# POSTECH-CVLab/SCNeRF

Hardware: AMD Instinct MI355X
Metric: rays/sec (64+128 samples/ray) train-step (higher is better)
Workload: dtype f32 (3 x fp16 MFMA products per product, fp32 accumulate); 1 GPU; configs[1]: 4096 rays x (64 coarse + 128 fine), coarse+fine NeRF (D=8, W=256), fwd+bwd of render_rays per GPU, perturb=1, raw_noise_std=1; precomputed rays of a fixed camera; rays_per_gpu=4096, parallelism=ray-parallel x1, no collective at N = 1

## Files before the change

include/scnerf_hip.h:

```cpp
#ifndef SCNERF_HIP_H
#define SCNERF_HIP_H

#include <stdint.h>

#ifdef __cplusplus
extern "C" {
#endif

#define SCNERF_ABI_VERSION 4

int scnerf_abi_version(void);


int scnerf_searchsorted(const float* a, const float* v, int64_t* out, int nrow, int nrow_a,
                        int nrow_v, int na, int nv, int side_left, void* stream);

int scnerf_sample_pdf(const float* bins, const float* weights, const float* u, int u_row_stride,
                      float* samples, int64_t* inds, float* cdf, int n, int nb, int ns,
                      void* stream);

int scnerf_render_randoms(unsigned long long seed, unsigned long long call, float* t_rand, long long n_t_rand,
                          float* u, long long n_u, float* noise_c, long long n_noise_c, float* noise_f,
                          long long n_noise_f, float raw_noise_std, void* stream);

// ... 18 lines not shown
long long scnerf_camera_bwd_workspace_floats(int n_slots);
int scnerf_camera_rays_bwd(const float* kps, const long long* cam_idx, int single_idx,
                           const float* extrinsic, int n_ext, const float* intr_init,
                           const float* intr_noise, float intr_scale, int multiplicative,
                           const float* extr_init, const float* extr_noise, float extr_scale,
                           int n_cams, const float* grid_o, float scale_o, const float* grid_d,
                           float scale_d, int gh, int gw, int H, int W, const float* g_o,
                           const float* g_d, float* d_intr_noise, float* d_extr_noise, float* d_grid_o,
                           float* d_grid_d, float* d_extrinsic, float* workspace, int n, void* stream);

int scnerf_camera_matrices_fwd(const float* intr_init, const float* intr_noise, float intr_scale, int multiplicative,
                               const float* extr_init, const float* extr_noise, float extr_scale, int n_cams,
                               float* K, float* E, void* stream);
int scnerf_camera_matrices_bwd(const float* intr_init, float intr_scale, int multiplicative, const float* extr_init,
                               const float* extr_noise, float extr_scale, int n_cams, const float* g_K,
                               const float* g_E, float* d_intr_noise, float* d_extr_noise, void* stream);

int scnerf_pinhole_rays(const float* kps, int kps_stride, const float* c2w, float focal, int H, int W,
                        float* rays_o, float* rays_d, int n, void* stream);

int scnerf_ndc_fwd(int H, int W, const float* focal_xy, float near, const float* rays_o,
                   const float* rays_d, float* ndc_o, float* ndc_d, int n, void* stream);
int scnerf_ndc_bwd(int H, int W, const float* focal_xy, float near, const float* rays_o,
                   const float* rays_d, const float* g_ndc_o, const float* g_ndc_d, float* g_rays_o,
                   float* g_rays_d, float* g_focal_xy, int n, void* stream);

int scnerf_pack_rays_fwd(int H, int W, const float* focal_xy, float ndc_near, const float* rays_o, const float* rays_d,
                         float near, float far, int cols, float* ray_batch, int n, void* stream);
int scnerf_pack_rays_bwd(int H, int W, const float* focal_xy, float ndc_near, const float* rays_o, const float* rays_d,
                         int cols, const float* g_ray_batch, float* g_rays_o, float* g_rays_d, float* g_focal_xy, int n,
                         void* stream);

int scnerf_upsample_grid_fwd(const float* grid, float scale, int gh, int gw, int H, int W, float* out,
                             void* stream);
int scnerf_upsample_grid_bwd(const float* g_out, float scale, int gh, int gw, int H, int W,
                             float* d_grid, void* stream);


int scnerf_composite_fwd(const float* raw, const float* z, const float* rays, int ray_stride,
                         const float* noise, int white_bkgd, float* rgb_map, float* disp_map,
                         float* acc_map, float* depth_map, float* weights, int n, int s,
                         void* stream);

int scnerf_composite_bwd(const float* raw, const float* z, const float* rays, int ray_stride,
                         const float* noise, int white_bkgd, const float* g_rgb,
                         const float* g_disp, const float* g_acc, const float* g_depth,
                         const float* g_raw_in, float* d_raw, float* d_rays_d, int n, int s,
                         void* stream);

int scnerf_ray_reduce(const float* d_pts, const float* d_views, const float* z,
                      const float* extra_d, float* d_rays, int ray_stride, int accumulate, int n,
                      int s, void* stream);


int scnerf_gather_f32(const float* src, const int* idx, float* dst, long long n, void* stream);

int scnerf_mlp_layout_info(int pt_dims, int* out, int n);

int scnerf_mlp_fwd(int pt_dims, const float* pts, const float* viewdirs, int vd_stride, int samples_per_ray,
                   const float* wpacked, float* raw, float* save, long long n_samples,
                   void* stream);

long long scnerf_mlp_save_floats(int pt_dims, long long n_samples);
long long scnerf_mlp_grad_floats(long long n_samples);

int scnerf_coarse_stage_fwd(const float* rays, int ray_stride, const float* t_vals, const float* t_rand, int lindisp,
                            const float* wpacked, float* save, const float* noise, int white_bkgd, float* z,
                            float* pts, float* raw, float* rgb_map, float* disp_map, float* acc_map,
                            float* depth_map, float* weights, int n_rays, int n_samples, void* stream);

int scnerf_mlp_bwd(int pt_dims, const float* d_raw, const float* pts, const float* viewdirs, int vd_stride,
                   int samples_per_ray, const float* wpacked_bwd, const float* save,
                   float* grads, float* d_pts, float* d_views, long long n_samples, void* stream);

long long scnerf_wgrad_workspace_floats(int n_load, int k_load, int n_chunks);
int scnerf_wgrad(const float* dz, int lda, int n_load, int n_out, int dz_tiled, const float* x,
                 int ldb, int k_load, int k_out, int x_tiled, long long n_samples, int n_chunks,
                 float* workspace, float* dW, int ldo, int col0, float* db, void* stream);

int scnerf_vecmat(const float* x_tiled256, const float* vec, int vec_stride, long long n_samples,
                  int n_chunks, float* workspace, float* dv, float* dvsum, void* stream);

int scnerf_nerf_param_count(int pt_dims);
int scnerf_wgrad_arithmetic(int mode);
long long scnerf_nerf_wgrad_workspace_floats(int n_chunks);
long long scnerf_wgrad_chunk_samples(long long n_samples, int n_chunks);
int scnerf_wgrad256_chunks(int n_chunks);
int scnerf_nerf_wgrad_h3(int pt_dims, const float* save, const float* grads, const float* d_raw,
                         long long n_samples, int n_chunks, float* workspace, float* flat_grad,
                         int accumulate, const float* amax_x, const float* amax_z, const float* scales,
                         void* ev_before, void* ev_after, void* stream);
int scnerf_wgrad256_half(const float* dz_tiled, const float* x_tiled, long long n_samples, int n_chunks,
                         float* workspace, float* dW, float* db, const float* amax_dz, const float* amax_x,
                         void* stream);
int scnerf_wgrad_half_narrow(const float* dz_tiled, int n_load, const float* x, int k_load, int k_out, int x_tiled,
                             long long n_samples, int n_chunks, float* workspace, float* dW, float* db,
                             const float* amax_dz, const float* amax_x, int n_coarse, long long coarse_chunk,
                             void* stream);
int scnerf_nerf_wgrad(int pt_dims, const float* save, const float* grads, const float* d_raw,
                      long long n_samples, int n_chunks, float* workspace, float* flat_grad,
                      int accumulate, void* stream);

long long scnerf_h3_scale_floats(void);
int scnerf_h3_pack(const float* flat_params, const int* jobs, const int* idx_fwd, const unsigned char* meta_fwd,
                   long long frags_fwd, const int* idx_bwd, const unsigned char* meta_bwd, long long frags_bwd,
                   short* stream_fwd, short* stream_bwd, float* scales, void* stream);
int scnerf_mlp_fwd_h3(int pt_dims, const float* pts, const float* viewdirs, int vd_stride, int samples_per_ray,
                      const float* wpacked, const short* stream_fwd, const float* scales, float* raw, float* save,
                      long long n_samples, float* chunk_amax, int n_chunks, long long chunk_samples, void* stream);
int scnerf_mlp_bwd_h3(int pt_dims, const float* d_raw, const float* pts, const float* viewdirs, int vd_stride,
                      int samples_per_ray, const float* wpacked_bwd, const short* stream_bwd, const float* scales,
                      const float* save, float* grads, float* d_pts, float* d_views, long long n_samples,
                      float* chunk_amax, int n_chunks, long long chunk_samples, void* stream);
int scnerf_coarse_stage_fwd_h3(const float* rays, int ray_stride, const float* t_vals, const float* t_rand,
                               int lindisp, const float* wpacked, const short* stream_fwd, const float* scales,
                               float* save, const float* noise, int white_bkgd, float* z, float* pts, float* raw,
                               float* rgb_map, float* disp_map, float* acc_map, float* depth_map, float* weights,
                               int n_rays, int n_samples, float* chunk_amax, int n_chunks, long long chunk_samples,
                               void* stream);
int scnerf_fine_stage_fwd_h3(const float* rays, int ray_stride, const float* z_c, const float* w_c, const float* u,
                             int u_row_stride, const float* wpacked, const short* stream_fwd, const float* scales,
                             float* save, const float* noise, int white_bkgd, float* z_f, float* pts_f, float* z_samples,
                             float* z_std, long long* inds, float* cdf, float* raw, float* rgb_map, float* disp_map,
                             float* acc_map, float* depth_map, float* weights, int n_rays, int n_coarse, int n_importance,
                             float* chunk_amax, int n_chunks, long long chunk_samples, void* stream);

int scnerf_mlp_fwd_h3_guarded(int pt_dims, const float* pts, const float* viewdirs, int vd_stride, int samples_per_ray,
                              const float* wpacked, const short* stream_fwd, const float* scales, float* raw, float* save,
                              long long n_samples, float* chunk_amax, int n_chunks, long long chunk_samples, int* guard_flags,
                              int* guard_any, float* guard_report, void* stream);
int scnerf_coarse_stage_fwd_h3_guarded(const float* rays, int ray_stride, const float* t_vals, const float* t_rand,
                                       int lindisp, const float* wpacked, const short* stream_fwd, const float* scales,
                                       float* save, const float* noise, int white_bkgd, float* z, float* pts, float* raw,
                                       float* rgb_map, float* disp_map, float* acc_map, float* depth_map, float* weights,
                                       int n_rays, int n_samples, float* chunk_amax, int n_chunks, long long chunk_samples,
                                       int* guard_flags, int* guard_any, float* guard_report, void* stream);
int scnerf_fine_stage_fwd_h3_guarded(const float* rays, int ray_stride, const float* z_c, const float* w_c, const float* u,
                                     int u_row_stride, const float* wpacked, const short* stream_fwd, const float* scales,
                                     float* save, const float* noise, int white_bkgd, float* z_f, float* pts_f,
                                     float* z_samples, float* z_std, long long* inds, float* cdf, float* raw, float* rgb_map,
                                     float* disp_map, float* acc_map, float* depth_map, float* weights, int n_rays,
                                     int n_coarse, int n_importance, float* chunk_amax, int n_chunks,
                                     long long chunk_samples, int* guard_flags, int* guard_any, float* guard_report,
                                     void* stream);
int scnerf_mlp_bwd_h3_guarded(int pt_dims, const float* d_raw, const float* pts, const float* viewdirs, int vd_stride,
                              int samples_per_ray, const float* wpacked_bwd, const short* stream_bwd, const float* scales,
                              const float* save, float* grads, float* d_pts, float* d_views, long long n_samples,
                              float* chunk_amax, int n_chunks, long long chunk_samples, int* guard_flags, int* guard_any,
                              float* guard_report, void* stream);
int scnerf_mlp_fwd_h3_lean(int pt_dims, const float* pts, const float* viewdirs, int vd_stride, int samples_per_ray,
                           const float* wpacked, const short* stream_fwd, const float* scales, float* raw, float* save,
                           long long n_samples, float* chunk_amax, int n_chunks, long long chunk_samples, int* guard_flags,
                           int* guard_any, float* guard_report, int lean, void* stream);
int scnerf_coarse_stage_fwd_h3_lean(const float* rays, int ray_stride, const float* t_vals, const float* t_rand,
                                    int lindisp, const float* wpacked, const short* stream_fwd, const float* scales,
                                    float* save, const float* noise, int white_bkgd, float* z, float* pts, float* raw,
                                    float* rgb_map, float* disp_map, float* acc_map, float* depth_map, float* weights,
                                    int n_rays, int n_samples, float* chunk_amax, int n_chunks, long long chunk_samples,
                                    int* guard_flags, int* guard_any, float* guard_report, int lean, void* stream);
int scnerf_fine_stage_fwd_h3_lean(const float* rays, int ray_stride, const float* z_c, const float* w_c, const float* u,
                                  int u_row_stride, const float* wpacked, const short* stream_fwd, const float* scales,
                                  float* save, const float* noise, int white_bkgd, float* z_f, float* pts_f,
                                  float* z_samples, float* z_std, long long* inds, float* cdf, float* raw, float* rgb_map,
                                  float* disp_map, float* acc_map, float* depth_map, float* weights, int n_rays,
                                  int n_coarse, int n_importance, float* chunk_amax, int n_chunks,
                                  long long chunk_samples, int* guard_flags, int* guard_any, float* guard_report, int lean,
                                  void* stream);
int scnerf_mlp_bwd_h3_lean(int pt_dims, const float* d_raw, const float* pts, const float* viewdirs, int vd_stride,
                           int samples_per_ray, const float* wpacked_bwd, const short* stream_bwd, const float* scales,
                           const float* save, float* grads, float* d_pts, float* d_views, long long n_samples,
                           float* chunk_amax, int n_chunks, long long chunk_samples, int* guard_flags, int* guard_any,
                           float* guard_report, int lean, void* stream);
int scnerf_nerf_wgrad_h3_lean(int pt_dims, const float* save, const float* grads, const float* d_raw,
                              long long n_samples, int n_chunks, float* workspace, float* flat_grad,
                              int accumulate, const float* amax_x, const float* amax_z, const float* scales,
                              const float* flat_params, void* ev_before, void* ev_after, void* stream);
int scnerf_wgrad_lean_finish(const float* M, const float* s, const float* flat_params, float* flat_grad, int accumulate,
                             void* stream);
int scnerf_wgrad_lean_finish_pd(int pt_dims, const float* M, const float* s, const float* flat_params, float* flat_grad,
                                int accumulate, void* stream);
int scnerf_mlp_fwd_gated(int pt_dims, const float* pts, const float* viewdirs, int vd_stride, int samples_per_ray,
                         const float* wpacked, float* raw, float* save, long long n_samples, const int* flags,
                         int max_workgroups, void* stream);
int scnerf_coarse_stage_fwd_gated(const float* rays, int ray_stride, const float* t_vals, const float* t_rand,
                                  int lindisp, const float* wpacked, float* save, const float* noise, int white_bkgd,
                                  float* z, float* pts, float* raw, float* rgb_map, float* disp_map, float* acc_map,
                                  float* depth_map, float* weights, int n_rays, int n_samples, const int* flags,
                                  int max_workgroups, void* stream);
int scnerf_mlp_bwd_gated(int pt_dims, const float* d_raw, const float* pts, const float* viewdirs, int vd_stride,
                         int samples_per_ray, const float* wpacked_bwd, const float* save, float* grads, float* d_pts,
                         float* d_views, long long n_samples, const int* flags, int max_workgroups, void* stream);

int scnerf_mlp_fwd_h3_fast(int pt_dims, const float* pts, const float* viewdirs, int vd_stride, int samples_per_ray,
                           const float* wpacked, const short* stream_fwd, const float* scales, float* raw,
                           long long n_samples, float* chunk_amax, int n_chunks, long long chunk_samples, void* stream);
int scnerf_coarse_stage_fwd_h3_fast(const float* rays, int ray_stride, const float* t_vals, const float* t_rand,
                                    int lindisp, const float* wpacked, const short* stream_fwd, const float* scales,
                                    const float* noise, int white_bkgd, float* z, float* pts, float* raw,
                                    float* rgb_map, float* disp_map, float* acc_map, float* depth_map, float* weights,
                                    int n_rays, int n_samples, float* chunk_amax, int n_chunks, long long chunk_samples,
                                    void* stream);


int scnerf_prd_loss_fwd(const float* kps0, const float* kps1, const float* rays0_o, const float* rays0_d,
                        const float* rays1_o, const float* rays1_d, const float* K, const float* E2,
                        float eps, float threshold, int negate_fx, int eval_mode, int m, float* sums6,
                        float* loss, float* n_match, void* stream);

int scnerf_prd_loss_bwd(const float* kps0, const float* kps1, const float* rays0_o, const float* rays0_d,
                        const float* rays1_o, const float* rays1_d, const float* K, const float* E2,
                        float eps, float threshold, int negate_fx, int m, const float* sums6,
                        const float* g_loss, float* g_rays0_o, float* g_rays0_d, float* g_rays1_o,
                        float* g_rays1_d, float* g_K, float* g_E2, float* workspace36, void* stream);

int scnerf_embed_fwd(const float* x, long long n, int d, const float* freqs, int n_freqs, int include_input,
                     float* out, void* stream);
int scnerf_embed_bwd(const float* x, const float* g_out, long long n, int d, const float* freqs, int n_freqs,
                     int include_input, float* g_x, void* stream);

int scnerf_prd_filter(const float* kps0, const float* kps1, const float* rays0_o, const float* rays0_d,
                      const float* rays1_o, const float* rays1_d, const float* K, const float* E2,
                      float eps, float threshold, int negate_fx, int m, unsigned char* keep, void* stream);


int scnerf_npp_intersect_fwd(const float* ray_o, const float* ray_d, float* far, int* outside_flag, int n,
                             void* stream);
int scnerf_npp_intersect_bwd(const float* ray_o, const float* ray_d, const float* g_far, float* g_ray_o,
                             float* g_ray_d, int n, void* stream);

int scnerf_npp_perturb_fwd(const float* z, const float* t_rand, float* out, int n, int s, void* stream);
int scnerf_npp_perturb_bwd(const float* g_out, const float* t_rand, float* g_z, int n, int s, void* stream);

int scnerf_npp_sample_pdf(const float* bins, const float* weights, const float* u, float* samples,
                          int* below_above, float* t, float* cdf, int n, int m, int ns, void* stream);
int scnerf_npp_sample_pdf_bwd(const float* g_samples, const int* below_above, const float* t, float* g_bins,
                              int n, int m, int ns, void* stream);

int scnerf_npp_points_fwd(const float* ray_o, const float* ray_d, const float* fg_z, const float* bg_z,
                          float* fg_pts, float* bg_pts, float* viewdirs, float* bg_depth_real, int n, int sf,
                          int sb, void* stream);
int scnerf_npp_points_bwd(const float* ray_o, const float* ray_d, const float* fg_z, const float* bg_z,
                          const float* d_fg_pts, const float* d_bg_pts, const float* d_views_fg,
                          const float* d_views_bg, const float* d_norm, const float* g_fg_z_in,
                          float* g_ray_o, float* g_ray_d, float* g_fg_z, int n, int sf, int sb, void* stream);

int scnerf_npp_composite_fwd(const float* raw_fg, const float* raw_bg, const float* fg_z, const float* fg_z_max,
                             const float* bg_z, const float* ray_d, float* rgb, float* fg_weights,
                             float* bg_weights, float* fg_rgb, float* fg_depth, float* bg_rgb, float* bg_depth,
                             float* bg_lambda, int n, int sf, int sb, void* stream);
int scnerf_npp_composite_bwd(const float* raw_fg, const float* raw_bg, const float* fg_z, const float* fg_z_max,
                             const float* bg_z, const float* ray_d, const float* g_rgb, const float* g_fg_weights,
                             const float* g_bg_weights, const float* g_fg_rgb, const float* g_fg_depth,
                             const float* g_bg_rgb, const float* g_bg_depth, const float* g_bg_lambda,
                             float* d_raw_fg, float* d_raw_bg, float* d_fg_z, float* d_fg_z_max, float* d_norm,
                             int n, int sf, int sb, void* stream);

int scnerf_npp_fg_lambda(const float* raw_fg, const float* fg_z, const float* fg_z_max, const float* ray_d,
                         float* bg_lambda, int n, int sf, void* stream);
int scnerf_npp_composite_fwd_skip(const float* raw_fg, const float* raw_bg_live, const float* fg_z,
                                  const float* fg_z_max, const float* bg_z, const float* ray_d, const int* slot_of,
                                  float* rgb, float* fg_weights, float* bg_weights, float* fg_rgb, float* fg_depth,
                                  float* bg_rgb, float* bg_depth, float* bg_lambda, int n, int n_live, int sf, int sb,
                                  void* stream);

int scnerf_npp_camera_rays_fwd(const long long* select, const float* dist2, int camera_idx,
                               const float* extrinsic, const float* intr_init, const float* intr_noise,
                               float intr_scale, int multiplicative, const float* extr_init,
                               const float* extr_noise, float extr_scale, int n_cams, const float* grid_o,
                               float scale_o, const float* grid_d, float scale_d, int gh, int gw, int H, int W,
                               float* rays_o, float* rays_d, int n, void* stream);
int scnerf_npp_camera_rays_bwd(const long long* select, const float* dist2, int camera_idx,
                               const float* extrinsic, const float* intr_init, const float* intr_noise,
                               float intr_scale, int multiplicative, const float* extr_init,
                               const float* extr_noise, float extr_scale, int n_cams, const float* grid_o,
                               float scale_o, const float* grid_d, float scale_d, int gh, int gw, int H, int W,
                               const float* g_o, const float* g_d, float* d_intr_noise, float* d_extr_noise,
                               float* d_grid_o, float* d_grid_d, float* d_extrinsic, float* d_dist2,
                               float* workspace, int n, void* stream);


int scnerf_adam_step(float* param, const float* grad, float* exp_avg, float* exp_avg_sq,
                     long long n, double lr, double beta1, double beta2, double eps,
                     double weight_decay, long long step, void* stream);
int scnerf_adam_step_range(float* param, const float* grad, float* exp_avg, float* exp_avg_sq,
                           long long n, double lr, double beta1, double beta2, double eps,
                           double weight_decay, long long decay_lo, long long decay_hi, long long step, void* stream);


long long scnerf_image_metrics_workspace_floats(int n, int c, int h, int w, int win);

int scnerf_image_metrics(const float* x, long long x_stride_n, long long x_stride_c, long long x_stride_h,
                         long long x_stride_w, const float* y, long long y_stride_n, long long y_stride_c,
                         long long y_stride_h, long long y_stride_w, int n, int c, int h, int w, const float* taps,
                         int win, float c1, float c2, float value_range, int clip_x, float* ssim_out, float* mse_out,
                         float* map_out, float* workspace, void* stream);


int scnerf_ray_batch(int mode, unsigned long long seed, unsigned long long step, const void* images, int image_u8,
                     int channels, int n_images, long long H, long long W, const int64_t* image_ids, int n_sel,
                     int image_pos, long long win_x0, long long win_y0, long long win_w, long long win_h, long long n,
                     int rank, int world, int white_bkgd, int64_t* coords, int64_t* select_inds, int64_t* image_idx,
                     float* target, void* stream);


int scnerf_ray_compact(const float* acc, float tau, int* live_idx, int* slot_of, int* n_live_dev, int* n_live_host,
                       long long n, void* stream);
// ... 73 lines not shown
```

scnerf_amd/_capi.py:

```python
from __future__ import annotations

import ctypes
import os
from ctypes import c_int, c_longlong, c_void_p, c_float, c_double

D = c_double

F = c_float

_HERE = os.path.dirname(os.path.abspath(__file__))
LIB_PATH = os.environ.get("SCNERF_HIP_LIB") or os.path.join(_HERE, "libscnerf_hip.so")

P = c_void_p
I = c_int
LL = c_longlong

PROTOTYPES = {
    "scnerf_abi_version": [],
    "scnerf_searchsorted": [P, P, P, I, I, I, I, I, I, P],
    "scnerf_sample_pdf": [P, P, P, I, P, P, P, I, I, I, P],
    "scnerf_render_randoms": [ctypes.c_ulonglong, ctypes.c_ulonglong, P, LL, P, LL, P, LL, P, LL, F, P],
    "scnerf_coarse_sample": [P, I, P, P, P, P, I, I, I, P],
    "scnerf_fine_sample": [P, I, P, P, P, I, P, P, P, P, P, P, I, I, I, P],
    "scnerf_camera_rays_fwd": [P, P, I, P, I, P, P, F, I, P, P, F, I, P, F, P, F, I, I, I, I, P, P, I, P],
    "scnerf_camera_rays_bwd": [P, P, I, P, I, P, P, F, I, P, P, F, I, P, F, P, F, I, I, I, I, P, P, P, P, P, P, P, P, I, P],
    "scnerf_camera_matrices_fwd": [P, P, F, I, P, P, F, I, P, P, P],
    "scnerf_camera_matrices_bwd": [P, F, I, P, P, F, I, P, P, P, P, P],
    "scnerf_pinhole_rays": [P, I, P, F, I, I, P, P, I, P],
    "scnerf_ndc_fwd": [I, I, P, F, P, P, P, P, I, P],
    "scnerf_ndc_bwd": [I, I, P, F, P, P, P, P, P, P, P, I, P],
    "scnerf_pack_rays_fwd": [I, I, P, F, P, P, F, F, I, P, I, P],
    "scnerf_pack_rays_bwd": [I, I, P, F, P, P, I, P, P, P, P, I, P],
    "scnerf_upsample_grid_fwd": [P, F, I, I, I, I, P, P],
    "scnerf_upsample_grid_bwd": [P, F, I, I, I, I, P, P],
    "scnerf_prd_loss_fwd": [P, P, P, P, P, P, P, P, F, F, I, I, I, P, P, P, P],
    "scnerf_prd_loss_bwd": [P, P, P, P, P, P, P, P, F, F, I, I, P, P, P, P, P, P, P, P, P, P],
    "scnerf_embed_fwd": [P, LL, I, P, I, I, P, P],
    "scnerf_embed_bwd": [P, P, LL, I, P, I, I, P, P],
    "scnerf_prd_filter": [P, P, P, P, P, P, P, P, F, F, I, I, P, P],
    "scnerf_npp_intersect_fwd": [P, P, P, P, I, P],
    "scnerf_npp_intersect_bwd": [P, P, P, P, P, I, P],
    "scnerf_npp_perturb_fwd": [P, P, P, I, I, P],
    "scnerf_npp_perturb_bwd": [P, P, P, I, I, P],
    "scnerf_npp_sample_pdf": [P, P, P, P, P, P, P, I, I, I, P],
    "scnerf_npp_sample_pdf_bwd": [P, P, P, P, I, I, I, P],
    "scnerf_npp_points_fwd": [P, P, P, P, P, P, P, P, I, I, I, P],
    "scnerf_npp_points_bwd": [P, P, P, P, P, P, P, P, P, P, P, P, P, I, I, I, P],
    "scnerf_npp_composite_fwd": [P, P, P, P, P, P, P, P, P, P, P, P, P, P, I, I, I, P],
    "scnerf_npp_composite_bwd": [P, P, P, P, P, P, P, P, P, P, P, P, P, P, P, P, P, P, P, I, I, I, P],
    "scnerf_npp_fg_lambda": [P, P, P, P, P, I, I, P],
    "scnerf_npp_composite_fwd_skip": [P, P, P, P, P, P, P, P, P, P, P, P, P, P, P, I, I, I, I, P],
    "scnerf_npp_camera_rays_fwd": [P, P, I, P, P, P, F, I, P, P, F, I, P, F, P, F, I, I, I, I, P, P, I, P],
    "scnerf_npp_camera_rays_bwd": [P, P, I, P, P, P, F, I, P, P, F, I, P, F, P, F, I, I, I, I, P, P, P, P, P, P, P,
                                   P, P, I, P],
    "scnerf_adam_step": [P, P, P, P, LL, D, D, D, D, D, LL, P],
    "scnerf_adam_step_range": [P, P, P, P, LL, D, D, D, D, D, LL, LL, LL, P],
    "scnerf_composite_fwd": [P, P, P, I, P, I, P, P, P, P, P, I, I, P],
    "scnerf_composite_bwd": [P, P, P, I, P, I, P, P, P, P, P, P, P, I, I, P],
    "scnerf_ray_reduce": [P, P, P, P, P, I, I, I, I, P],
    "scnerf_gather_f32": [P, P, P, LL, P],
    "scnerf_mlp_layout_info": [I, P, I],
    "scnerf_mlp_fwd": [I, P, P, I, I, P, P, P, LL, P],
    "scnerf_coarse_stage_fwd": [P, I, P, P, I, P, P, P, I, P, P, P, P, P, P, P, P, I, I, P],
    "scnerf_mlp_bwd": [I, P, P, P, I, I, P, P, P, P, P, LL, P],
    "scnerf_nerf_param_count": [I],
    "scnerf_nerf_wgrad": [I, P, P, P, LL, I, P, P, I, P],
    "scnerf_wgrad": [P, I, I, I, I, P, I, I, I, I, LL, I, P, P, I, I, P, P],
    "scnerf_vecmat": [P, P, I, LL, I, P, P, P, P],
    "scnerf_wgrad_arithmetic": [I],
    "scnerf_wgrad256_chunks": [I],
    "scnerf_h3_pack": [P, P, P, P, LL, P, P, LL, P, P, P, P],
    "scnerf_mlp_fwd_h3": [I, P, P, I, I, P, P, P, P, P, LL, P, I, LL, P],
    "scnerf_mlp_bwd_h3": [I, P, P, P, I, I, P, P, P, P, P, P, P, LL, P, I, LL, P],
    "scnerf_coarse_stage_fwd_h3": [P, I, P, P, I, P, P, P, P, P, I, P, P, P, P, P, P, P, P, I, I, P, I, LL, P],
    "scnerf_fine_stage_fwd_h3": [P, I, P, P, P, I, P, P, P, P, P, I, P, P, P, P, P, P, P, P, P, P, P, P, I, I, I, P, I, LL, P],
    "scnerf_mlp_fwd_h3_guarded": [I, P, P, I, I, P, P, P, P, P, LL, P, I, LL, P, P, P, P],
    "scnerf_mlp_bwd_h3_guarded": [I, P, P, P, I, I, P, P, P, P, P, P, P, LL, P, I, LL, P, P, P, P],
    "scnerf_coarse_stage_fwd_h3_guarded": [P, I, P, P, I, P, P, P, P, P, I, P, P, P, P, P, P, P, P, I, I, P, I, LL,
                                           P, P, P, P],
    "scnerf_fine_stage_fwd_h3_guarded": [P, I, P, P, P, I, P, P, P, P, P, I, P, P, P, P, P, P, P, P, P, P, P, P, I, I, I, P,
                                         I, LL, P, P, P, P],
    "scnerf_mlp_fwd_h3_fast": [I, P, P, I, I, P, P, P, P, LL, P, I, LL, P],
    "scnerf_coarse_stage_fwd_h3_fast": [P, I, P, P, I, P, P, P, P, I, P, P, P, P, P, P, P, P, I, I, P, I, LL, P],
    "scnerf_mlp_fwd_gated": [I, P, P, I, I, P, P, P, LL, P, I, P],
    "scnerf_coarse_stage_fwd_gated": [P, I, P, P, I, P, P, P, I, P, P, P, P, P, P, P, P, I, I, P, I, P],
    "scnerf_mlp_bwd_gated": [I, P, P, P, I, I, P, P, P, P, P, LL, P, I, P],
    "scnerf_nerf_wgrad_h3": [I, P, P, P, LL, I, P, P, I, P, P, P, P, P, P],
    "scnerf_wgrad256_half": [P, P, LL, I, P, P, P, P, P, P],
    "scnerf_wgrad_half_narrow": [P, I, P, I, I, I, LL, I, P, P, P, P, P, I, LL, P],
    "scnerf_mlp_fwd_h3_lean": [I, P, P, I, I, P, P, P, P, P, LL, P, I, LL, P, P, P, I, P],
    "scnerf_mlp_bwd_h3_lean": [I, P, P, P, I, I, P, P, P, P, P, P, P, LL, P, I, LL, P, P, P, I, P],
    "scnerf_coarse_stage_fwd_h3_lean": [P, I, P, P, I, P, P, P, P, P, I, P, P, P, P, P, P, P, P, I, I, P, I, LL,
                                        P, P, P, I, P],
    "scnerf_fine_stage_fwd_h3_lean": [P, I, P, P, P, I, P, P, P, P, P, I, P, P, P, P, P, P, P, P, P, P, P, P, I, I, I, P,
                                      I, LL, P, P, P, I, P],
    "scnerf_nerf_wgrad_h3_lean": [I, P, P, P, LL, I, P, P, I, P, P, P, P, P, P, P],
    "scnerf_wgrad_lean_finish": [P, P, P, P, I, P],
    "scnerf_wgrad_lean_finish_pd": [I, P, P, P, P, I, P],
    "scnerf_image_metrics": [P, LL, LL, LL, LL, P, LL, LL, LL, LL, I, I, I, I, P, I, F, F, F, I, P, P, P, P, P],
    "scnerf_ray_batch": [I, ctypes.c_ulonglong, ctypes.c_ulonglong, P, I, I, I, LL, LL, P, I, I, LL, LL, LL, LL, LL, I, I, I,
                         P, P, P, P, P],
    "scnerf_ray_compact": [P, F, P, P, P, P, LL, P],
    "scnerf_ray_rows_gather": [P, P, P, LL, I, LL, P],
    "scnerf_ray_expand": [P, LL, LL, I, I] + [P] * 8 + [P] * 4 + [P] * 8 + [P],
    "scnerf_live_compact": [P, LL, P, P, P, P, P, P, P],
    "scnerf_live_gather": [P, LL, LL, P, P, I, P, I, I, P, P, P, P],
    "scnerf_live_remap_maxima": [P, LL, P, I, LL, P, I, LL, I, P],
    "scnerf_live_scatter_rows": [P, P, P, LL, I, LL, P],
    "scnerf_mlp_bwd_h3_masks": [I, P, P, P, I, I, P, P, P, P, P, P, P, LL, P, I, LL, P, P, P, I, P],
    "scnerf_nerf_wgrad_h3_live": [I, P, LL, I, P, P, P, P, LL, I, P, P, I, P, P, P, P, P, P, P],
    "scnerf_occ_compact": [P, LL, P, I, I, P, I, F, F, F, F, F, F, P, P, P, P, P, P, P, P],
    "scnerf_occ_expand_raw": [P, P, P, LL, LL, P],
    "scnerf_occ_probe_points": [LL, LL, I, I, F, F, F, F, F, F, F, F, F, P, P],
    "scnerf_occ_accumulate": [P, F, LL, LL, I, I, P, P],
    "scnerf_occ_dilate": [P, P, I, P],
    "scnerf_occ_compact4": [P, LL, P, I, I, P, I, F, F, F, F, F, F, P, P, P, P, P, P, P, P],
    "scnerf_occ_probe_points_inverted": [LL, LL, I, I, F, F, F, F, F, F, F, F, F, P, P],
    "scnerf_seg_compact": [P, LL, I, I, I, P, P, I, P, I, F, F, F, F, F, F, P, P, P, P, P, P, P, P],
    "scnerf_seg_expand_raw": [P, P, P, LL, I, I, I, LL, P],
    "scnerf_seg_transmittance": [P, P, P, I, LL, I, I, I, I, I, D, P, P, P, P],
}


SIZE_FUNCS = {"scnerf_mlp_save_floats": [I, LL], "scnerf_mlp_grad_floats": [LL],
              "scnerf_wgrad_workspace_floats": [I, I, I],
              "scnerf_nerf_wgrad_workspace_floats": [I],
              "scnerf_h3_scale_floats": [],
              "scnerf_wgrad_chunk_samples": [LL, I],
              "scnerf_camera_bwd_workspace_floats": [I],
              "scnerf_live_compact_workspace_ints": [LL],
              "scnerf_occ_compact_workspace_ints": [LL],
              "scnerf_occ_compact4_workspace_ints": [LL],
              "scnerf_seg_compact_workspace_ints": [LL],
              "scnerf_image_metrics_workspace_floats": [I, I, I, I, I]}


def bind(lib: ctypes.CDLL) -> ctypes.CDLL:
    for name, args in PROTOTYPES.items():
        fn = getattr(lib, name)
        fn.argtypes = args
        fn.restype = c_int
    for name, args in SIZE_FUNCS.items():
        fn = getattr(lib, name)
        fn.argtypes = args
        fn.restype = c_longlong
    return lib


_lib = None


class ScnerfLibraryError(RuntimeError):
    pass


def load() -> ctypes.CDLL:
    global _lib
    if _lib is None:
        import torch
        if not os.path.isfile(LIB_PATH):
            raise ScnerfLibraryError(
                "libscnerf_hip.so is not built (%s). Run `python -m scnerf_amd.csrc.build` "
                "(or __graft_entry__.build()); scnerf_amd has no CPU fallback." % LIB_PATH)
        _lib = bind(ctypes.CDLL(LIB_PATH))
        if _lib.scnerf_abi_version() != 4:
            raise ScnerfLibraryError("ABI version mismatch")
    return _lib


def on_device(t) -> bool:
    return bool(t.is_cuda)


def current_stream():
    import torch
    return torch.cuda.current_stream().cuda_stream


def check(status: int, what: str):
    if status != 0:
        raise RuntimeError("%s failed with status %d" % (what, status))
```

scnerf_amd/csrc/mlp_fwd_h3.hip:

```cpp
#include <scn_wave.h>

#include "launch.h"
#include "mlp_fwd_h3_api.h"
#include "mlp_h3.h"
#include "scnerf_hip.h"

namespace {

using namespace scn;
using namespace scn::h3;

constexpr int kScaleBlocks = 16, kScaleCols = 512;
constexpr int kScalePartial = 4 + kScaleCols;

__global__ __launch_bounds__(256) void h3_scale_partial_kernel(const float* __restrict__ params, const int* __restrict__ jobs,
                                                               float* __restrict__ partial, float* __restrict__ table) {
    float* red = dynamic_lds<float>();
    float* cols_w = red + 16;
    const int l = blockIdx.x, blk = blockIdx.y, tid = threadIdx.x, lane = lane_id(), wave = wave_id();
    const float* wt = params + jobs[4 * l];
    const int rows = jobs[4 * l + 1], cols = jobs[4 * l + 2];
    const float* bs = params + jobs[4 * l + 3];
    const int per = (rows + kScaleBlocks - 1) / kScaleBlocks;
    const int r0 = blk * per, r1 = min(rows, r0 + per);
    if (l == kLayerRgb && blk == 0 && tid == 0) table[kLayerRgb * kScaleStride + kPoison] = 0.f;
    float mx = 0.f, rowsum = 0.f, bmax = 0.f, bad = 0.f;
    float colp[kScaleCols / 64];
#pragma unroll
    for (int k = 0; k < kScaleCols / 64; ++k) colp[k] = 0.f;
    for (int r = r0 + wave; r < r1; r += 4) {
        float s = 0.f;
#pragma unroll
        for (int k = 0; k < kScaleCols / 64; ++k) {
            const int c = lane + 64 * k;
            const float a = c < cols ? fabsf(wt[(long)r * cols + c]) : 0.f;
            s += a;
            mx = fmaxf(mx, a);
            colp[k] += a;
        }
        for (int o = 32; o > 0; o >>= 1) s += shfl_xor(s, o);
        rowsum = fmaxf(rowsum, s);
        bmax = fmaxf(bmax, fabsf(bs[r]));
        if (!(s < __builtin_huge_valf()) || !(fabsf(bs[r]) < __builtin_huge_valf())) bad = 1.f;
    }
    for (int o = 32; o > 0; o >>= 1) mx = fmaxf(mx, shfl_xor(mx, o));
#pragma unroll
    for (int k = 0; k < kScaleCols / 64; ++k) cols_w[wave * kScaleCols + lane + 64 * k] = colp[k];
    if (lane == 0) { red[wave * 4] = mx; red[wave * 4 + 1] = rowsum; red[wave * 4 + 2] = bmax; red[wave * 4 + 3] = bad; }
    block_sync();
    float* out = partial + ((long)l * kScaleBlocks + blk) * kScalePartial;
    if (tid < 4) out[tid] = fmaxf(fmaxf(red[tid], red[4 + tid]), fmaxf(red[8 + tid], red[12 + tid]));
    for (int c = tid; c < kScaleCols; c += 256)
        out[4 + c] = ((cols_w[c] + cols_w[kScaleCols + c]) + cols_w[2 * kScaleCols + c]) + cols_w[3 * kScaleCols + c];
}

__global__ __launch_bounds__(256) void h3_scale_finish_kernel(const float* __restrict__ partial, const int* __restrict__ jobs,
                                                              float* __restrict__ table) {
    float* red = dynamic_lds<float>();
    const int l = blockIdx.x, tid = threadIdx.x;
    const int cols = jobs[4 * l + 2];
    const float* p = partial + (long)l * kScaleBlocks * kScalePartial;
    float colsum = 0.f;
    for (int c = tid; c < cols; c += 256) {
        float s = 0.f;
        for (int b = 0; b < kScaleBlocks; ++b) s += p[b * kScalePartial + 4 + c];
        colsum = fmaxf(colsum, s);
    }
    red[tid] = colsum;
    block_sync();
    for (int s = 128; s > 0; s >>= 1) {
        if (tid < s) red[tid] = fmaxf(red[tid], red[tid + s]);
        block_sync();
    }
    if (tid == 0) {
        float mx = 0.f, rowsum = 0.f, bmax = 0.f, bad = 0.f;
        for (int b = 0; b < kScaleBlocks; ++b) {
            mx = fmaxf(mx, p[b * kScalePartial]);
            rowsum = fmaxf(rowsum, p[b * kScalePartial + 1]);
            bmax = fmaxf(bmax, p[b * kScalePartial + 2]);
            bad = fmaxf(bad, p[b * kScalePartial + 3]);
        }
        if (bad > 0.f) table[kLayerRgb * kScaleStride + kPoison] = __builtin_nanf("");
        const float sw = scn::h3::scale_for(mx);
        float* t = table + l * kScaleStride;
        t[kSw] = sw;
        t[kSwInv] = scn::h3::inv_pow2(sw);
        t[kBoundA] = rowsum * 1.0001f;
        t[kBoundB] = bmax;
        t[kBoundAT] = red[0] * 1.0001f;
        t[5] = mx; t[6] = 0.f;
        if (l != kLayerRgb) t[kPoison] = 0.f;
    }
}

__global__ __launch_bounds__(256) void h3_pack_kernel(const float* __restrict__ params, const int* __restrict__ idx,
                                                      const unsigned char* __restrict__ meta, const float* __restrict__ table,
                                                      short* __restrict__ out, long n) {
    const long i = (long)blockIdx.x * blockDim.x + threadIdx.x;
    if (i >= n) return;
    const int j = idx[i];
    const unsigned mt = meta[i >> 9];
    const float x = j >= 0 ? params[j] * table[(mt >> 1) * kScaleStride + kSw] : 0.f;
    const unsigned hb = f16_bits(x);
    out[i] = (short)((mt & 1u) ? f16_bits(x - f16_value(hb)) : hb);
}

}

extern "C" long long scnerf_h3_scale_floats(void) {
    return (long long)kScaleLayers * kScaleStride + (long long)kScaleLayers * kScaleBlocks * kScalePartial;
}

extern "C" int scnerf_h3_pack(const float* flat_params, const int* jobs, const int* idx_fwd, const unsigned char* meta_fwd,
                              long long frags_fwd, const int* idx_bwd, const unsigned char* meta_bwd, long long frags_bwd,
                              short* stream_fwd, short* stream_bwd, float* scales, void* stream) {
    SCN_RETURN_IF(!flat_params || !jobs || !scales, SCN_EINVAL);
    SCN_RETURN_IF((frags_fwd > 0 && (!idx_fwd || !meta_fwd || !stream_fwd)) || (frags_bwd > 0 && (!idx_bwd || !meta_bwd || !stream_bwd)), SCN_EINVAL);
    SCN_RETURN_IF(frags_fwd < 0 || frags_bwd < 0, SCN_EINVAL);
    hipStream_t st = (hipStream_t)stream;
    float* partial = scales + kScaleLayers * kScaleStride;
    hipLaunchKernelGGL(h3_scale_partial_kernel, dim3(kScaleLayers, kScaleBlocks), dim3(256), (16 + 4 * kScaleCols) * 4, st,
                       flat_params, jobs, partial, scales);
    hipLaunchKernelGGL(h3_scale_finish_kernel, dim3(kScaleLayers), dim3(256), 1024, st, partial, jobs, scales);
    if (frags_fwd > 0)
        hipLaunchKernelGGL(h3_pack_kernel, dim3(scn_ceil_div(frags_fwd * 512, 256)), dim3(256), 0, st, flat_params, idx_fwd,
                           meta_fwd, scales, stream_fwd, (long)(frags_fwd * 512));
    if (frags_bwd > 0)
        hipLaunchKernelGGL(h3_pack_kernel, dim3(scn_ceil_div(frags_bwd * 512, 256)), dim3(256), 0, st, flat_params, idx_bwd,
                           meta_bwd, scales, stream_bwd, (long)(frags_bwd * 512));
    return scn_launch_status();
}

extern "C" int scnerf_mlp_fwd_h3_lean(int pt_dims, const float* pts, const float* viewdirs, int vd_stride,
                                      int samples_per_ray, const float* wpacked, const short* stream_fwd,
                                      const float* scales, float* raw, float* save, long long n_samples, float* chunk_amax,
                                      int n_chunks, long long chunk_samples, int* guard_flags, int* guard_any,
                                      float* guard_report, int lean, void* stream) {
    SCN_RETURN_IF(!pts || !viewdirs || !wpacked || !stream_fwd || !scales || !raw, SCN_EINVAL);
    SCN_RETURN_IF(samples_per_ray < 1 || vd_stride < 3 || n_samples < 0 || (pt_dims != 3 && pt_dims != 4), SCN_EINVAL);
    SCN_RETURN_IF(n_samples >= (1LL << 31), SCN_ENOSUP);
    SCN_RETURN_IF(chunk_amax && (n_chunks < 1 || chunk_samples < 32 || chunk_samples % 32), SCN_EINVAL);
    SCN_RETURN_IF(!guard_flags != !guard_any || (guard_report && !guard_flags), SCN_EINVAL);
    if (n_samples == 0) return 0;
    hipStream_t st = (hipStream_t)stream;
    const scn::h3f::ChunkMaxima cm{chunk_amax, n_chunks, lean != 0, (long)chunk_samples, {guard_flags, guard_any, guard_report}};
    return pt_dims == 3 ? scn::h3f::fwd_h3_pd3(pts, viewdirs, vd_stride, samples_per_ray, wpacked, stream_fwd, scales, raw, save, n_samples, cm, st)
                        : scn::h3f::fwd_h3_pd4(pts, viewdirs, vd_stride, samples_per_ray, wpacked, stream_fwd, scales, raw, save, n_samples, cm, st);
}

extern "C" int scnerf_mlp_fwd_h3_guarded(int pt_dims, const float* pts, const float* viewdirs, int vd_stride,
                                         int samples_per_ray, const float* wpacked, const short* stream_fwd,
                                         const float* scales, float* raw, float* save, long long n_samples, float* chunk_amax,
                                         int n_chunks, long long chunk_samples, int* guard_flags, int* guard_any,
                                         float* guard_report, void* stream) {
    return scnerf_mlp_fwd_h3_lean(pt_dims, pts, viewdirs, vd_stride, samples_per_ray, wpacked, stream_fwd, scales, raw, save,
                                  n_samples, chunk_amax, n_chunks, chunk_samples, guard_flags, guard_any, guard_report, 0, stream);
}

extern "C" int scnerf_mlp_fwd_h3(int pt_dims, const float* pts, const float* viewdirs, int vd_stride, int samples_per_ray,
                                 const float* wpacked, const short* stream_fwd, const float* scales, float* raw, float* save,
                                 long long n_samples, float* chunk_amax, int n_chunks, long long chunk_samples, void* stream) {
    return scnerf_mlp_fwd_h3_guarded(pt_dims, pts, viewdirs, vd_stride, samples_per_ray, wpacked, stream_fwd, scales, raw, save,
                                     n_samples, chunk_amax, n_chunks, chunk_samples, nullptr, nullptr, nullptr, stream);
}

extern "C" int scnerf_coarse_stage_fwd_h3_lean(const float* rays, int ray_stride, const float* t_vals, const float* t_rand,
                                               int lindisp, const float* wpacked, const short* stream_fwd,
                                               const float* scales, float* save, const float* noise, int white_bkgd, float* z,
                                               float* pts, float* raw, float* rgb_map, float* disp_map, float* acc_map,
                                               float* depth_map, float* weights, int n_rays, int n_samples,
                                               float* chunk_amax, int n_chunks, long long chunk_samples, int* guard_flags,
                                               int* guard_any, float* guard_report, int lean, void* stream) {
    SCN_RETURN_IF(!rays || !t_vals || !wpacked || !stream_fwd || !scales || !z || !pts || !raw || !rgb_map || !disp_map || !acc_map, SCN_EINVAL);
    SCN_RETURN_IF(n_rays < 0 || ray_stride < 11, SCN_EINVAL);
    SCN_RETURN_IF(n_samples != scn::h3f::kCoarseSamples || n_rays >= (1 << 25), SCN_ENOSUP);
    SCN_RETURN_IF(chunk_amax && (n_chunks < 1 || chunk_samples < 32 || chunk_samples % 32), SCN_EINVAL);
    SCN_RETURN_IF(!guard_flags != !guard_any || (guard_report && !guard_flags), SCN_EINVAL);
    if (n_rays == 0) return 0;
    const scn::h3f::CoarseStage cs{rays, ray_stride, n_rays, t_vals, t_rand, lindisp, z, pts, noise, white_bkgd,
                                   rgb_map, disp_map, acc_map, depth_map, weights};
    const scn::h3f::ChunkMaxima cm{chunk_amax, n_chunks, lean != 0, (long)chunk_samples, {guard_flags, guard_any, guard_report}};
    return scn::h3f::fwd_h3_coarse(cs, rays, ray_stride, wpacked, stream_fwd, scales, raw, save, cm, (hipStream_t)stream);
}

extern "C" int scnerf_coarse_stage_fwd_h3_guarded(const float* rays, int ray_stride, const float* t_vals, const float* t_rand,
                                                  int lindisp, const float* wpacked, const short* stream_fwd,
                                                  const float* scales, float* save, const float* noise, int white_bkgd, float* z,
                                                  float* pts, float* raw, float* rgb_map, float* disp_map, float* acc_map,
                                                  float* depth_map, float* weights, int n_rays, int n_samples,
                                                  float* chunk_amax, int n_chunks, long long chunk_samples, int* guard_flags,
                                                  int* guard_any, float* guard_report, void* stream) {
    return scnerf_coarse_stage_fwd_h3_lean(rays, ray_stride, t_vals, t_rand, lindisp, wpacked, stream_fwd, scales, save, noise,
                                           white_bkgd, z, pts, raw, rgb_map, disp_map, acc_map, depth_map, weights, n_rays,
                                           n_samples, chunk_amax, n_chunks, chunk_samples, guard_flags, guard_any, guard_report,
                                           0, stream);
}

extern "C" int scnerf_coarse_stage_fwd_h3(const float* rays, int ray_stride, const float* t_vals, const float* t_rand,
                                          int lindisp, const float* wpacked, const short* stream_fwd, const float* scales,
                                          float* save, const float* noise, int white_bkgd, float* z, float* pts, float* raw,
                                          float* rgb_map, float* disp_map, float* acc_map, float* depth_map, float* weights,
                                          int n_rays, int n_samples, float* chunk_amax, int n_chunks, long long chunk_samples,
                                          void* stream) {
    return scnerf_coarse_stage_fwd_h3_guarded(rays, ray_stride, t_vals, t_rand, lindisp, wpacked, stream_fwd, scales, save, noise,
                                              white_bkgd, z, pts, raw, rgb_map, disp_map, acc_map, depth_map, weights, n_rays,
                                              n_samples, chunk_amax, n_chunks, chunk_samples, nullptr, nullptr, nullptr, stream);
}

extern "C" int scnerf_mlp_fwd_h3_fast(int pt_dims, const float* pts, const float* viewdirs, int vd_stride, int samples_per_ray,
                                      const float* wpacked, const short* stream_fwd, const float* scales, float* raw,
                                      long long n_samples, float* chunk_amax, int n_chunks, long long chunk_samples,
                                      void* stream) {
    SCN_RETURN_IF(!pts || !viewdirs || !wpacked || !stream_fwd || !scales || !raw, SCN_EINVAL);
    SCN_RETURN_IF(samples_per_ray < 1 || vd_stride < 3 || n_samples < 0 || (pt_dims != 3 && pt_dims != 4), SCN_EINVAL);
    SCN_RETURN_IF(n_samples >= (1LL << 31), SCN_ENOSUP);
    SCN_RETURN_IF(chunk_amax && (n_chunks < 1 || chunk_samples < 32 || chunk_samples % 32), SCN_EINVAL);
    if (n_samples == 0) return 0;
    hipStream_t st = (hipStream_t)stream;
    return pt_dims == 3 ? scn::h3f::fwd_h3_pd3_fast(pts, viewdirs, vd_stride, samples_per_ray, wpacked, stream_fwd, scales, raw, n_samples, st)
                        : scn::h3f::fwd_h3_pd4_fast(pts, viewdirs, vd_stride, samples_per_ray, wpacked, stream_fwd, scales, raw, n_samples, st);
}

extern "C" int scnerf_coarse_stage_fwd_h3_fast(const float* rays, int ray_stride, const float* t_vals, const float* t_rand,
                                               int lindisp, const float* wpacked, const short* stream_fwd, const float* scales,
                                               const float* noise, int white_bkgd, float* z, float* pts, float* raw,
                                               float* rgb_map, float* disp_map, float* acc_map, float* depth_map, float* weights,
                                               int n_rays, int n_samples, float* chunk_amax, int n_chunks,
                                               long long chunk_samples, void* stream) {
    SCN_RETURN_IF(!rays || !t_vals || !wpacked || !stream_fwd || !scales || !z || !pts || !raw || !rgb_map || !disp_map || !acc_map, SCN_EINVAL);
    SCN_RETURN_IF(n_rays < 0 || ray_stride < 11, SCN_EINVAL);
    SCN_RETURN_IF(n_samples != scn::h3f::kCoarseSamples || n_rays >= (1 << 25), SCN_ENOSUP);
    SCN_RETURN_IF(chunk_amax && (n_chunks < 1 || chunk_samples < 32 || chunk_samples % 32), SCN_EINVAL);
    if (n_rays == 0) return 0;
    const scn::h3f::CoarseStage cs{rays, ray_stride, n_rays, t_vals, t_rand, lindisp, z, pts, noise, white_bkgd,
                                   rgb_map, disp_map, acc_map, depth_map, weights};
    return scn::h3f::fwd_h3_coarse_fast(cs, rays, ray_stride, wpacked, stream_fwd, scales, raw, (hipStream_t)stream);
}

extern "C" int scnerf_fine_stage_fwd_h3_lean(const float* rays, int ray_stride, const float* z_c, const float* w_c,
                                             const float* u, int u_row_stride, const float* wpacked, const short* stream_fwd,
                                             const float* scales, float* save, const float* noise, int white_bkgd, float* z_f,
                                             float* pts_f, float* z_samples, float* z_std, long long* inds, float* cdf,
                                             float* raw, float* rgb_map, float* disp_map, float* acc_map, float* depth_map,
                                             float* weights, int n_rays, int n_coarse, int n_importance, float* chunk_amax,
                                             int n_chunks, long long chunk_samples, int* guard_flags, int* guard_any,
                                             float* guard_report, int lean, void* stream) {
    SCN_RETURN_IF(!rays || !z_c || !w_c || !u || !wpacked || !stream_fwd || !scales, SCN_EINVAL);
    SCN_RETURN_IF(!z_f || !pts_f || !z_samples || !z_std || !raw || !rgb_map || !disp_map || !acc_map, SCN_EINVAL);
    SCN_RETURN_IF(n_rays < 0 || ray_stride < 11 || (u_row_stride != 0 && u_row_stride != n_importance), SCN_EINVAL);
    SCN_RETURN_IF(n_coarse != scn::h3f::kCoarseSamples || (n_importance != 64 && n_importance != 128 && n_importance != 192), SCN_ENOSUP);
    SCN_RETURN_IF((long long)n_rays * (n_coarse + n_importance) >= (1LL << 31), SCN_ENOSUP);
    SCN_RETURN_IF(chunk_amax && (n_chunks < 1 || chunk_samples < 32 || chunk_samples % 32), SCN_EINVAL);
    SCN_RETURN_IF(!guard_flags != !guard_any || (guard_report && !guard_flags), SCN_EINVAL);
    if (n_rays == 0) return 0;
    const int tot = n_coarse + n_importance;
    const int rays_per_block = tot == 192 ? 2 : 1, tiles = tot * rays_per_block / 128;
    const scn::h3f::FineStage fs{rays, ray_stride, n_rays, z_c, w_c, u, u_row_stride, n_importance, z_f, pts_f, z_samples, z_std,
                                 reinterpret_cast<int64_t*>(inds), cdf, noise, white_bkgd, rgb_map, disp_map, acc_map,
                                 depth_map, weights, rays_per_block, tiles};
    const scn::h3f::ChunkMaxima cm{chunk_amax, n_chunks, lean != 0, (long)chunk_samples, {guard_flags, guard_any, guard_report}};
    return save ? scn::h3f::fwd_h3_fine_train(fs, wpacked, stream_fwd, scales, raw, save, cm, (hipStream_t)stream)
                : scn::h3f::fwd_h3_fine_infer(fs, wpacked, stream_fwd, scales, raw, cm, (hipStream_t)stream);
}

extern "C" int scnerf_fine_stage_fwd_h3_guarded(const float* rays, int ray_stride, const float* z_c, const float* w_c,
                                                const float* u, int u_row_stride, const float* wpacked, const short* stream_fwd,
                                                const float* scales, float* save, const float* noise, int white_bkgd, float* z_f,
                                                float* pts_f, float* z_samples, float* z_std, long long* inds, float* cdf,
                                                float* raw, float* rgb_map, float* disp_map, float* acc_map, float* depth_map,
                                                float* weights, int n_rays, int n_coarse, int n_importance, float* chunk_amax,
                                                int n_chunks, long long chunk_samples, int* guard_flags, int* guard_any,
                                                float* guard_report, void* stream) {
    return scnerf_fine_stage_fwd_h3_lean(rays, ray_stride, z_c, w_c, u, u_row_stride, wpacked, stream_fwd, scales, save, noise,
                                         white_bkgd, z_f, pts_f, z_samples, z_std, inds, cdf, raw, rgb_map, disp_map, acc_map,
                                         depth_map, weights, n_rays, n_coarse, n_importance, chunk_amax, n_chunks, chunk_samples,
                                         guard_flags, guard_any, guard_report, 0, stream);
}

extern "C" int scnerf_fine_stage_fwd_h3(const float* rays, int ray_stride, const float* z_c, const float* w_c, const float* u,
                                        int u_row_stride, const float* wpacked, const short* stream_fwd, const float* scales,
                                        float* save, const float* noise, int white_bkgd, float* z_f, float* pts_f,
                                        float* z_samples, float* z_std, long long* inds, float* cdf, float* raw, float* rgb_map,
                                        float* disp_map, float* acc_map, float* depth_map, float* weights, int n_rays,
                                        int n_coarse, int n_importance, float* chunk_amax, int n_chunks,
                                        long long chunk_samples, void* stream) {
    return scnerf_fine_stage_fwd_h3_guarded(rays, ray_stride, z_c, w_c, u, u_row_stride, wpacked, stream_fwd, scales, save, noise,
                                            white_bkgd, z_f, pts_f, z_samples, z_std, inds, cdf, raw, rgb_map, disp_map, acc_map,
                                            depth_map, weights, n_rays, n_coarse, n_importance, chunk_amax, n_chunks,
                                            chunk_samples, nullptr, nullptr, nullptr, stream);
}
```

scnerf_amd/csrc/mlp_fwd_h3_api.h:

```cpp
#pragma once
#include <cstdint>

#include <hip/hip_runtime.h>

#include "resident_guard.h"

namespace scn {
namespace h3f {

struct ChunkMaxima { float* amax; int n_chunks; int lean; long chunk; ResidentGuard guard; };

struct CoarseStage {
    const float* rays; int ray_stride; int n_rays;
    const float* t_vals; const float* t_rand; int lindisp;
    float* z; float* pts;
    const float* noise; int white_bkgd;
    float* rgb; float* disp; float* acc; float* depth; float* weights;
};
constexpr int kCoarseSamples = 64;

struct FineStage {
    const float* rays; int ray_stride; int n_rays;
    const float* z_c; const float* w_c;
    const float* u; int u_row_stride; int n_importance;
    float* z_f; float* pts_f; float* z_samples; float* z_std; int64_t* inds; float* cdf;
    const float* noise; int white_bkgd;
    float* rgb; float* disp; float* acc; float* depth; float* weights;
    int rays_per_block, tiles;
};

int fwd_h3_pd3(const float* pts, const float* viewdirs, int vd_stride, int samples_per_ray, const float* wpacked,
               const short* stream_fwd, const float* scales, float* raw, float* save, long long n_samples, ChunkMaxima cm,
               hipStream_t st);
int fwd_h3_pd4(const float* pts, const float* viewdirs, int vd_stride, int samples_per_ray, const float* wpacked,
               const short* stream_fwd, const float* scales, float* raw, float* save, long long n_samples, ChunkMaxima cm,
               hipStream_t st);
int fwd_h3_coarse(const CoarseStage& cs, const float* rays, int ray_stride, const float* wpacked, const short* stream_fwd,
                  const float* scales, float* raw, float* save, ChunkMaxima cm, hipStream_t st);
int fwd_h3_pd3_fast(const float* pts, const float* viewdirs, int vd_stride, int samples_per_ray, const float* wpacked,
                    const short* stream_fwd, const float* scales, float* raw, long long n_samples, hipStream_t st);
int fwd_h3_pd4_fast(const float* pts, const float* viewdirs, int vd_stride, int samples_per_ray, const float* wpacked,
                    const short* stream_fwd, const float* scales, float* raw, long long n_samples, hipStream_t st);
int fwd_h3_coarse_fast(const CoarseStage& cs, const float* rays, int ray_stride, const float* wpacked, const short* stream_fwd,
                       const float* scales, float* raw, hipStream_t st);
int fwd_h3_fine_train(const FineStage& fs, const float* wpacked, const short* stream_fwd, const float* scales, float* raw,
                      float* save, ChunkMaxima cm, hipStream_t st);
int fwd_h3_fine_infer(const FineStage& fs, const float* wpacked, const short* stream_fwd, const float* scales, float* raw,
                      ChunkMaxima cm, hipStream_t st);

}
}
```

scnerf_amd/csrc/mlp_fwd_h3_kernel.h:

```cpp
#pragma once
#include <scn_wave.h>

#include "launch.h"
#include "mlp_fwd_h3_api.h"
#include "mlp_h3.h"
#include "ray_sample.h"
#include "ray_stage.h"

namespace scn {
namespace h3f {

using namespace scn::mlp;
using namespace scn::h3;


template <int PD, int L, int NS, int LD>
struct PeInverse {
    unsigned off[LD];
    constexpr PeInverse() : off() {
        for (int c = 0; c < LD; ++c) off[c] = 0xffffffffu;
        for (int s = 0; s < NS; ++s)
            for (int h = 0; h < 2; ++h) {
                const int c = pe_col(L, s, h, PD);
                if (c >= 0) off[c] = (unsigned)((s / 4) * (kThreads * 16) + h * 512 + (s % 4) * 4);
            }
    }
};
template <int PD, int L, int NS, int LD>
__device__ __forceinline__ void store_pe_tile(const char* slots, float* __restrict__ section, long wave_tile, int wave, int lane) {
    if (lab::kNoPeStore) return;
    wave_lds_handoff();
    static constexpr PeInverse<PD, L, NS, LD> inverse{};
    constexpr int LPR = LD / 4;
    unsigned o[4];
#pragma unroll
    for (int i = 0; i < 4; ++i) o[i] = inverse.off[4 * (lane % LPR) + i];
    const global_bytes_rw block = uniform_global_rw(section + wave_tile * (32L * LD));
#pragma unroll
    for (int k = 0; k < LD / 8; ++k) {
        const int m = k * (64 / LPR) + lane / LPR;
        const char* row = slots + (wave * 64 + m) * 16;
        f32x4 v;
#pragma unroll
        for (int i = 0; i < 4; ++i) v[i] = o[i] == 0xffffffffu ? 0.f : *reinterpret_cast<const float*>(row + o[i]);
        store_stream_at(uniform_global_rw(block + k * 1024), pinned_here((unsigned)lane * 16u), v);
    }
}

struct NoDensity {};
struct Density {
    float sg;
    const float* alpha;
    f32x4 wq;
};
template <bool ON> struct MaskBits { unsigned bits0, bits1, words[4]; };
template <> struct MaskBits<false> {};
struct NoWindow {};
struct Window { unsigned window; };

template <bool TRAIN, int KIND, int PRODUCTS = 3>
struct FwdEpi : std::conditional_t<KIND == 1, Density, NoDensity>, MaskBits<TRAIN && KIND != 2>,
                std::conditional_t<TRAIN && KIND == 2, Window, NoWindow> {
    float os, s_next, am;
    const float* bias;
    global_bytes_rw save;
    unsigned lane16;
    f32x4 bq;
    float v[4];
    unsigned hp;

    __device__ __forceinline__ void prime() {}

    template <int P, int PIECE, int SUB, int NS>
    __device__ __forceinline__ void sub(f32x16 (&acc)[2], u32x4 (&oh)[NS], u32x4 (&ol)[NS]) {
        constexpr int x = PIECE >> 2, q = PIECE & 3, T = 2 * P + x;
        constexpr int sl = 2 * T + (q >> 1), c0 = 2 * (q & 1);
        static_assert(sl < NS, "operand buffer too small for this tile");
        if constexpr (lab::kNoEpilogue) {
            if constexpr (SUB == 1) {
                oh[sl][c0] = __float_as_uint(acc[x][4 * q]) & 0x3bff3bffu; oh[sl][c0 + 1] = __float_as_uint(acc[x][4 * q + 1]) & 0x3bff3bffu;
                if constexpr (PRODUCTS == 3) {
                    ol[sl][c0] = __float_as_uint(acc[x][4 * q + 2]) & 0x3bff3bffu; ol[sl][c0 + 1] = __float_as_uint(acc[x][4 * q + 3]) & 0x3bff3bffu;
                }
            }
        } else if constexpr (SUB == 0) {
            bq = *reinterpret_cast<const f32x4*>(bias + (4 * T + q) * 8);
            if constexpr (KIND == 1) this->wq = *reinterpret_cast<const f32x4*>(this->alpha + (4 * T + q) * 8);
            if constexpr (TRAIN && KIND != 2 && PIECE == 0) { this->bits0 = 0u; this->bits1 = 0u; }
        } else if constexpr (SUB <= 4) {
            constexpr int e = SUB - 1;
            const float z = __builtin_fmaf(acc[x][4 * q + e], os, bq[e]);
            v[e] = KIND == 2 ? z : relu_raw(z);
            if constexpr (TRAIN && KIND != 2) {
                if constexpr (x == 0) this->bits0 = shift_in_positive(this->bits0, v[e]);
                else this->bits1 = shift_in_positive(this->bits1, v[e]);
            }
        } else if constexpr (SUB == 5) {
            if constexpr (KIND == 2) { am = max3_abs(am, v[0], v[1]); am = max3_abs(am, v[2], v[3]); }
            else { am = max3(am, v[0], v[1]); am = max3(am, v[2], v[3]); }
        } else if constexpr (SUB == 6) {
            hp = pack_f16_scaled(v[0], v[1], s_next);
        } else if constexpr (SUB == 7) {
            oh[sl][c0] = hp;
            if constexpr (PRODUCTS == 3) ol[sl][c0] = pack_f16(residual_f16<0>(v[0], s_next, hp), residual_f16<1>(v[1], s_next, hp));
        } else if constexpr (SUB == 8) {
            hp = pack_f16_scaled(v[2], v[3], s_next);
        } else if constexpr (SUB == 9) {
            oh[sl][c0 + 1] = hp;
            if constexpr (PRODUCTS == 3) ol[sl][c0 + 1] = pack_f16(residual_f16<0>(v[2], s_next, hp), residual_f16<1>(v[3], s_next, hp));
        } else if constexpr (SUB == 10) {
            if constexpr (TRAIN && !lab::kNoStore) {
                if constexpr (KIND == 2)
                    store_written_through_window(uniform_global_rw(save + (4 * T + q) * 1024), pinned_here(lane16), f32x4{v[0], v[1], v[2], v[3]}, this->window);
                else
                    store_written_through_at(uniform_global_rw(save + (4 * T + q) * 1024), pinned_here(lane16), f32x4{v[0], v[1], v[2], v[3]});
            }
        } else {
            if constexpr (KIND == 1) {
#pragma unroll
                for (int e = 0; e < 4; ++e) this->sg = __builtin_fmaf(this->wq[e], v[e], this->sg);
            }
            if constexpr (TRAIN && KIND != 2 && PIECE == 7) this->words[P] = (this->bits0 << 16) | this->bits1;
        }
    }
};



constexpr int kTabFeat = 8 * 256, kTabViews = kTabFeat + 256, kTabRgb = kTabViews + 128, kTabAlpha = kTabRgb + 32,
              kTabAlphaB = kTabAlpha + 256;

enum : int { kPoints = 0, kCoarse = 1, kFine = 2 };
constexpr int kFineMaxSamples = 384;

template <int PD, int STAGE = kPoints>
__host__ __device__ constexpr unsigned fwd_lds_bytes() {
    return (unsigned)(kStreamLds + kTableFloats * 4 + Var<PD>::kES * kThreads * 4 + (STAGE == kFine ? kFineMaxSamples * 20 : 0));
}

struct FwdKernelArgs {
    const float* pts; const float* viewdirs; int vd_stride; int samples_per_ray; const float* wpk; const short* wh3;
    const float* sc; float* raw; float* save; long P; CoarseStage cs; FineStage fs; ChunkMaxima cm;
};
static_assert(sizeof(FwdKernelArgs) == 72 + sizeof(CoarseStage) + sizeof(FineStage) + sizeof(ChunkMaxima), "argument block layout");

template <int PD, bool TRAIN, int STAGE, int PRODUCTS = 3>
__global__ __launch_bounds__(kThreads, 1) void mlp_fwd_h3_kernel(
    const float* __restrict__ pts, const float* __restrict__ viewdirs, int vd_stride, int samples_per_ray,
    const float* __restrict__ wpk, const short* __restrict__ wh3, const float* __restrict__ sc,
    float* __restrict__ raw, float* __restrict__ save_arg, long P, CoarseStage cs, FineStage fs, ChunkMaxima cm) {
    using V = Var<PD>;
    constexpr int ES = V::kES, NE = ES / 8;
    constexpr bool COARSE = STAGE == kCoarse, FINE = STAGE == kFine, ONE = PRODUCTS == 1;
    static_assert(!ONE || (!TRAIN && !FINE), "one product: forward-only, sample-list forward and coarse stage");
    claim_whole_register_file();
    auto low_of = [](const u32x4& lo, const u32x4& hi) { if constexpr (ONE) return hi; else return lo; };
    float* const save = TRAIN ? save_arg : nullptr;
    const long Ppad_kernel = padded_samples(P);

    Wave w;
    w.lds = dynamic_lds<char>();
    float* const tables = reinterpret_cast<float*>(w.lds + kStreamLds);
    float* const zbuf = reinterpret_cast<float*>(w.lds + kStreamLds + kTableFloats * 4 + ES * kThreads * 4);
    f32x4* const rawbuf = reinterpret_cast<f32x4*>(zbuf + kFineMaxSamples);
    for (int i = threadIdx.x; i < V::kFwdTotal - V::kFwdBias; i += kThreads) tables[i] = wpk[V::kFwdBias + i];
    const int tiles = FINE ? uniform(fs.tiles) : 1;
    if constexpr (FINE) {
        static_assert(PD == 3, "the fine stage samples 3-D points");
        const int wv = uniform(wave_id());
        const int slot = wv % fs.rays_per_block;
        long ray = (long)blockIdx.x * fs.rays_per_block + slot;
        const bool mine = wv < fs.rays_per_block && ray < fs.n_rays;
        if (ray >= fs.n_rays) ray = fs.n_rays - 1;
        const int tot = kCoarseSamples + fs.n_importance;
        float* scratch = reinterpret_cast<float*>(w.lds + kStreamLds + kTableFloats * 4) + wv * ray::fine_sample_lds_floats(kCoarseSamples, fs.n_importance);
        const float* sorted = ray::fine_sample_ray(
            fs.rays + ray * fs.ray_stride, fs.z_c + ray * kCoarseSamples, fs.w_c + ray * kCoarseSamples,
            fs.u + ray * fs.u_row_stride, kCoarseSamples, fs.n_importance, scratch, lane_id(), mine, fs.z_f + ray * tot,
            fs.pts_f + ray * tot * 3, fs.z_samples + ray * fs.n_importance, fs.z_std + ray,
            fs.inds ? fs.inds + ray * fs.n_importance : nullptr, fs.cdf ? fs.cdf + ray * (kCoarseSamples - 1) : nullptr);
        if (wv < fs.rays_per_block)
            for (int e = lane_id(); e < tot; e += kWave) zbuf[slot * tot + e] = sorted[e];
        block_sync();
    }
    static_for<FINE ? 3 : 1>([&](auto tile_tag) __attribute__((always_inline)) {
    constexpr int tile = decltype(tile_tag)::value;
    if (tile < tiles && (!FINE || ((long)blockIdx.x * tiles + tile) * kSamplesPerBlock < P)) {
    if (tile > 0) block_sync();
    const long Ppad = FINE ? fresh_uniform(Ppad_kernel) : Ppad_kernel;
    const unsigned tid = FINE ? pinned_here(threadIdx.x) : threadIdx.x;
    w.tid16 = tid * 16u;
    f32x4* const park = reinterpret_cast<f32x4*>(w.lds + kStreamLds + kTableFloats * 4) + tid;
    const long wave_tile = ((long)blockIdx.x * tiles + tile) * 4 + uniform(wave_id());
    struct Lane { int lane, m, h; long p, pc; bool live; };
    auto lane_now = [&]() {
        Lane L;
        L.lane = (int)pinned_here((unsigned)lane_id());
        L.m = L.lane & 31;
        L.h = L.lane >> 5;
        L.p = wave_tile * kSamplesPerWave + L.m;
        L.live = L.p < P;
        L.pc = L.live ? L.p : P - 1;
        return L;
    };
    const Lane L0 = lane_now();
    const int lane = L0.lane, m = L0.m, h = (int)(pinned_here((unsigned)lane_id()) >> 5);
    const long p = L0.p, pc = L0.pc;
    const bool live = L0.live;
    (void)m;

    w.lane16 = (unsigned)lane * 16u;
    stream_prime(w.ws, wh3, w.lds, w.tid16);

    float px, py, pz, pw = 0.f;
    auto coarse_depth_at = [&](long q) {
        const float* r = cs.rays + (q >> 6) * cs.ray_stride;
        return ray::coarse_z(r[6], r[7], cs.t_vals, (int)(q & 63), kCoarseSamples, cs.lindisp, cs.t_rand != nullptr,
                             cs.t_rand ? cs.t_rand[q] : 0.f);
    };
    if constexpr (COARSE) {
        static_assert(PD == 3, "the coarse stage samples 3-D points");
        const float* r = cs.rays + (pc >> 6) * cs.ray_stride;
        const float z = coarse_depth_at(pc);
        px = r[0] + r[3] * z;
        py = r[1] + r[4] * z;
        pz = r[2] + r[5] * z;
        if (live && h == 0) {
            cs.z[p] = z;
            cs.pts[p * 3 + 0] = px; cs.pts[p * 3 + 1] = py; cs.pts[p * 3 + 2] = pz;
        }
    } else if constexpr (FINE) {
        const FwdKernelArgs mirror{pts, viewdirs, vd_stride, samples_per_ray, wpk, wh3, sc, raw, save_arg, P, cs, fs, cm};
        const auto* late = late_args(mirror);
        const float* r = late->fs.rays + (long)((unsigned)pc / (unsigned)samples_per_ray) * late->fs.ray_stride;
        const float z = zbuf[(int)(pc - (long)blockIdx.x * tiles * kSamplesPerBlock)];
        px = r[0] + r[3] * z;
        py = r[1] + r[4] * z;
        pz = r[2] + r[5] * z;
    } else {
        px = pts[pc * PD + 0]; py = pts[pc * PD + 1]; pz = pts[pc * PD + 2];
        if constexpr (PD == 4) pw = pts[pc * PD + (PD - 1)];
    }
    const float m_e = fmaxf(fmaxf(1.f, fabsf(px)), fmaxf(fmaxf(fabsf(py), fabsf(pz)), fabsf(pw)));
    u32x4 eh[NE], el[NE];
    {
        float e[ES];
        if constexpr (lab::kNoPe) {
#pragma unroll
            for (int i = 0; i < ES; ++i) e[i] = px * (float)i + py;
        } else {
            pe_slots<PD, 10, ES>(px, py, pz, pw, h, e);
        }
#pragma unroll
        for (int g = 0; g < ES / 4; ++g) park[g * kThreads] = f32x4{e[4 * g], e[4 * g + 1], e[4 * g + 2], e[4 * g + 3]};
        if (save) store_pe_tile<PD, 10, ES, V::kEW>(w.lds + kStreamLds + kTableFloats * 4, save + (long)kSaveEpts * Ppad, wave_tile,
                                                    uniform(wave_id()), lane);
        const float s_e = scale_for(m_e);
#pragma unroll
        for (int u = 0; u < NE; ++u) {
            if constexpr (ONE) cut8_high(e + 8 * u, s_e, eh[u]);
            else cut8(e + 8 * u, s_e, eh[u], el[u]);
        }
    }
    block_sync();
    ring_prime(w);

    u32x4 bh[2][16], bl[2][16];
    f32x16 acc[2][2];
    const float* const tab_h = tables + 4 * h;
    auto section = [&](int offset, int width) {
        return uniform_global_rw(save + (long)offset * Ppad + wave_tile * (32L * width));
    };
    auto mask_block = [&](int sect) {
        unsigned* base = reinterpret_cast<unsigned*>(save + (long)V::kSavePerSample * Ppad);
        return uniform_global_rw(base + ((long)sect * (Ppad / 32) + wave_tile) * 256);
    };
    auto scale_of = [&](int layer, int what) { return sc[layer * kScaleStride + what]; };
    auto amax_of = [&](float a) { return fmaxf(a, shfl_xor(a, 32)); };
    const int chunk_of_tile = (TRAIN && cm.amax) ? uniform((int)((unsigned)(wave_tile * kSamplesPerWave) / (unsigned)cm.chunk)) : 0;
    auto note_chunk_max = [&](int job, float v) __attribute__((always_inline)) {
        if constexpr (TRAIN) {
            if (cm.amax == nullptr) return;
            v = fmaxf(v, shfl_xor(v, 16)); v = fmaxf(v, shfl_xor(v, 8)); v = fmaxf(v, shfl_xor(v, 4));
            v = fmaxf(v, shfl_xor(v, 2)); v = fmaxf(v, shfl_xor(v, 1));
            if (lane_id() == 0) atomic_max_nonneg(cm.amax + (long)job * cm.n_chunks + chunk_of_tile, v);
        }
    };

    auto guard = [&](int guard_layer, float am, float s) __attribute__((always_inline)) {
        if constexpr (!ONE) {
            const FwdKernelArgs mirror{pts, viewdirs, vd_stride, samples_per_ray, wpk, wh3, sc, raw, save_arg, P, cs, fs, cm};
            const auto* late = late_args(mirror);
            const ResidentGuard g{late->cm.guard.flags, late->cm.guard.any, late->cm.guard.report};
            guard_check(g, guard_layer, am, s, lane_now().live, wave_tile);
        }
    };

    using Relu = FwdEpi<TRAIN, 0, PRODUCTS>;
    auto make_relu = [&](int l, float s_in) {
        Relu e;
        e.os = inv_pow2(s_in) * scale_of(l, kSwInv);
        e.s_next = 1.f;
        e.am = 0.f;
        e.bias = tab_h + 256 * l;
        e.save = TRAIN ? section(kSaveAct + 256 * l, 256) : nullptr;
        e.lane16 = w.lane16;
        e.prime();
        return e;
    };
    auto store_mask = [&](auto& epi, int sect) {
        if constexpr (TRAIN) store_at(mask_block(sect), w.lane16, u32x4{epi.words[0], epi.words[1], epi.words[2], epi.words[3]});
    };

    Relu prev = make_relu(0, scale_for(m_e));
    prev.s_next = scale_for(__builtin_fmaf(scale_of(0, kBoundA), m_e, scale_of(0, kBoundB)));
    {
        auto operand = [&](auto s_tag, u32x4& xh, u32x4& xl) {
            constexpr int s = decltype(s_tag)::value;
            xh = eh[s]; xl = low_of(el[s], xh);
        };
        static_for<4>([&](auto p_tag) {
            constexpr int PP = decltype(p_tag)::value;
            tile_pair<NE * PP, NE, PRODUCTS>(w, acc[PP & 1], operand, NoFill{});
            if constexpr (PP < 3) epi_all<Relu, PP>(prev, acc[PP & 1], bh[0], bl[0]);
        });
    }

    auto trunk_layer = [&](auto x_tag, auto nef_tag, auto u0_tag, auto& pend, auto& cur, int pend_mask_sect, int layer,
                           float am_floor, float bound_floor) __attribute__((always_inline)) {
        constexpr int X = decltype(x_tag)::value, NEF = decltype(nef_tag)::value, U0 = decltype(u0_tag)::value;
        constexpr int NK = NEF + 16;
        auto operand = [&](auto s_tag, u32x4& xh, u32x4& xl) {
            constexpr int s = decltype(s_tag)::value;
            if constexpr (s < NEF) { xh = eh[s]; xl = low_of(el[s], xh); }
            else { xh = bh[X][s - NEF]; xl = low_of(bl[X][s - NEF], xh); }
        };
        using Pend = std::remove_reference_t<decltype(pend)>;
        using Cur = std::remove_reference_t<decltype(cur)>;
        tile_pair<U0, NK, PRODUCTS>(w, acc[0], operand, [&](auto sg_tag) {
            epi_slot<Pend, 3, decltype(sg_tag)::value, NEF >= 4 ? 12 : 9>(pend, acc[1], bh[X], bl[X]);
        });
        if constexpr (std::is_base_of_v<MaskBits<true>, Pend>) store_mask(pend, pend_mask_sect);
        const float am_in = amax_of(pend.am);
        note_chunk_max(layer == kLayerFeat ? 7 : layer - 1, am_in);
        guard(layer == kLayerFeat ? 7 : layer - 1, am_in, pend.s_next);
        const float am = fmaxf(am_in, am_floor);
        cur.s_next = scale_for(fmaxf(__builtin_fmaf(scale_of(layer, kBoundA), am, scale_of(layer, kBoundB)), bound_floor));
        tile_pair<U0 + NK, NK, PRODUCTS>(w, acc[1], operand, [&](auto sg_tag) {
            epi_slot<Cur, 0, decltype(sg_tag)::value, 12>(cur, acc[0], bh[X ^ 1], bl[X ^ 1]);
        });
        tile_pair<U0 + 2 * NK, NK, PRODUCTS>(w, acc[0], operand, [&](auto sg_tag) {
            epi_slot<Cur, 1, decltype(sg_tag)::value, 12>(cur, acc[1], bh[X ^ 1], bl[X ^ 1]);
        });
        tile_pair<U0 + 3 * NK, NK, PRODUCTS>(w, acc[1], operand, [&](auto sg_tag) {
            epi_slot<Cur, 2, decltype(sg_tag)::value, 12>(cur, acc[0], bh[X ^ 1], bl[X ^ 1]);
        });
    };

#pragma unroll 1
    for (int it = 0; it < 3; ++it) {
        const int l = 2 * it + 1;
        Relu cur = make_relu(l, prev.s_next);
        if (it < 2) {
            trunk_layer(I<0>{}, I<0>{}, I<0>{}, prev, cur, l - 1, l, 0.f, 0.f);
        } else {
            float e[ES];
#pragma unroll
            for (int g = 0; g < ES / 4; ++g) {
                const f32x4 v = park[g * kThreads];
                e[4 * g] = v[0]; e[4 * g + 1] = v[1]; e[4 * g + 2] = v[2]; e[4 * g + 3] = v[3];
            }
#pragma unroll
            for (int u = 0; u < NE; ++u) {
                if constexpr (ONE) cut8_high(e + 8 * u, prev.s_next, eh[u]);
                else cut8(e + 8 * u, prev.s_next, eh[u], el[u]);
            }
            trunk_layer(I<0>{}, I<NE>{}, I<0>{}, prev, cur, l - 1, l, m_e, 0.f);
        }
        prev = cur;
        Relu cur2 = make_relu(l + 1, prev.s_next);
        trunk_layer(I<1>{}, I<0>{}, I<0>{}, prev, cur2, l, l + 1, 0.f, l + 1 == 4 ? m_e : 0.f);
        prev = cur2;
    }

    float vx, vy, vz;
    {
        const Lane L = lane_now();
        const long ray = (long)((unsigned)L.pc / (unsigned)samples_per_ray);
        vx = viewdirs[ray * vd_stride + 0]; vy = viewdirs[ray * vd_stride + 1]; vz = viewdirs[ray * vd_stride + 2];
    }
    const float m_ev = fmaxf(fmaxf(1.f, fabsf(vx)), fmaxf(fabsf(vy), fabsf(vz)));
    FwdEpi<TRAIN, 1, PRODUCTS> epi7;
    {
        const Relu t = make_relu(7, prev.s_next);
        epi7.os = t.os; epi7.s_next = 1.f; epi7.am = 0.f; epi7.sg = 0.f; epi7.bias = t.bias;
        epi7.alpha = tab_h + kTabAlpha; epi7.save = t.save; epi7.lane16 = t.lane16;
        epi7.prime();
    }
    trunk_layer(I<0>{}, I<0>{}, I<0>{}, prev, epi7, 6, 7, 0.f, 0.f);
    FwdEpi<TRAIN, 2, PRODUCTS> epif;
    epif.os = inv_pow2(epi7.s_next) * scale_of(kLayerFeat, kSwInv);
    epif.s_next = 1.f; epif.am = 0.f;
    epif.bias = tab_h + kTabFeat;
    epif.save = TRAIN ? section(kSaveFeat, 256) : nullptr;
    epif.lane16 = w.lane16;
    if constexpr (TRAIN) {
        const FwdKernelArgs mirror{pts, viewdirs, vd_stride, samples_per_ray, wpk, wh3, sc, raw, save_arg, P, cs, fs, cm};
        epif.window = late_args(mirror)->cm.lean ? kStoreWindowShut : kStoreWindowOpen;
    }
    epif.prime();
    trunk_layer(I<1>{}, I<0>{}, I<0>{}, epi7, epif, 7, kLayerFeat, 0.f, m_ev);

    u32x4 vh[2], vl[2];
    {
        float ev[16];
        pe_slots<3, 4, 16>(vx, vy, vz, 0.f, h, ev);
        if (save) {
            f32x4* const vpark = reinterpret_cast<f32x4*>(w.lds + kStreamLds + kTableFloats * 4) + pinned_here(threadIdx.x);
#pragma unroll
            for (int g = 0; g < 4; ++g) vpark[g * kThreads] = f32x4{ev[4 * g], ev[4 * g + 1], ev[4 * g + 2], ev[4 * g + 3]};
            store_pe_tile<3, 4, 16, 32>(w.lds + kStreamLds + kTableFloats * 4, save + (long)kSaveEviews * Ppad, wave_tile,
                                        uniform(wave_id()), (int)pinned_here((unsigned)lane_id()));
        }
        if constexpr (ONE) {
            cut8_high(ev, epif.s_next, vh[0]);
            cut8_high(ev + 8, epif.s_next, vh[1]);
        } else {
            cut8(ev, epif.s_next, vh[0], vl[0]);
            cut8(ev + 8, epif.s_next, vh[1], vl[1]);
        }
    }
    Relu epiv;
    epiv.os = inv_pow2(epif.s_next) * scale_of(kLayerViews, kSwInv);
    epiv.s_next = 1.f; epiv.am = 0.f;
    epiv.bias = tab_h + kTabViews;
    epiv.save = TRAIN ? section(kSaveHv, 128) : nullptr;
    epiv.lane16 = w.lane16;
    epiv.prime();
    if constexpr (TRAIN) { epiv.words[2] = 0u; epiv.words[3] = 0u; }
    {
        auto operand = [&](auto s_tag, u32x4& xh, u32x4& xl) {
            constexpr int s = decltype(s_tag)::value;
            if constexpr (s < 16) { xh = bh[0][s]; xl = low_of(bl[0][s], xh); }
            else { xh = vh[s - 16]; xl = low_of(vl[s - 16], xh); }
        };
        tile_pair<0, 18, PRODUCTS>(w, acc[0], operand, [&](auto sg_tag) {
            epi_slot<FwdEpi<TRAIN, 2, PRODUCTS>, 3, decltype(sg_tag)::value, 9>(epif, acc[1], bh[0], bl[0]);
        });
        const float am_f = amax_of(epif.am);
        guard(kLayerFeat, am_f, epif.s_next);
        const float am = fmaxf(am_f, m_ev);
        epiv.s_next = scale_for(__builtin_fmaf(scale_of(kLayerViews, kBoundA), am, scale_of(kLayerViews, kBoundB)));
        tile_pair<18, 18, PRODUCTS>(w, acc[1], operand, [&](auto sg_tag) {
            epi_slot<Relu, 0, decltype(sg_tag)::value, 12>(epiv, acc[0], bh[1], bl[1]);
        });
        epi_all<Relu, 1>(epiv, acc[1], bh[1], bl[1]);
        store_mask(epiv, 8);
        guard(kLayerViews, amax_of(epiv.am), epiv.s_next);
    }

    f32x16 accc[2];
    tile_single<36, 4, PRODUCTS>(w, accc, [&](auto s_tag, u32x4& xh, u32x4& xl) {
        constexpr int s = decltype(s_tag)::value;
        xh = bh[1][s]; xl = low_of(bl[1][s], xh);
    }, NoFill{});
    const float os_rgb = __builtin_fmaf(inv_pow2(epiv.s_next), scale_of(kLayerRgb, kSwInv), scale_of(kLayerRgb, kPoison));
    const float sigma = epi7.sg + shfl_xor(epi7.sg, 32) + tables[kTabAlphaB];
    const f32x4 brgb = *reinterpret_cast<const f32x4*>(tables + kTabRgb);
    const f32x4 o = {__builtin_fmaf(accc[0][0] + accc[1][0], os_rgb, brgb[0]), __builtin_fmaf(accc[0][1] + accc[1][1], os_rgb, brgb[1]),
                     __builtin_fmaf(accc[0][2] + accc[1][2], os_rgb, brgb[2]), sigma};
    const Lane LE = lane_now();
    if (LE.live && LE.h == 0) *reinterpret_cast<f32x4*>(raw + LE.p * 4) = o;
    if constexpr (FINE) {
        if (LE.h == 0) rawbuf[tile * kSamplesPerBlock + wave_id() * kSamplesPerWave + LE.m] = o;
    }
    if constexpr (COARSE) {
        float* sraw = reinterpret_cast<float*>(w.lds + kStreamLds + kTableFloats * 4);
        float* sz = sraw + kSamplesPerBlock * 4;
        const int local = wave_id() * kSamplesPerWave + LE.m;
        if (LE.h == 0) {
            *reinterpret_cast<f32x4*>(sraw + local * 4) = o;
            sz[local] = coarse_depth_at(LE.pc);
        }
        block_sync();
        if (wave_id() < kSamplesPerBlock / kCoarseSamples) {
            const int slot = wave_id();
            long ray = (long)blockIdx.x * (kSamplesPerBlock / kCoarseSamples) + slot;
            const bool ray_live = ray < cs.n_rays;
            if (!ray_live) ray = cs.n_rays - 1;
            const float norm = ray::ray_norm(cs.rays + ray * cs.ray_stride + 3);
            auto fetch = [&](int i, f32x4* rw, float* zi) {
                *rw = *reinterpret_cast<const f32x4*>(sraw + (slot * kCoarseSamples + i) * 4);
                *zi = sz[slot * kCoarseSamples + i];
            };
            ray::composite_ray(fetch, kCoarseSamples, norm, cs.noise ? cs.noise + ray * kCoarseSamples : nullptr,
                               cs.white_bkgd, ray_live, LE.lane, cs.rgb + ray * 3, cs.disp + ray, cs.acc + ray,
                               cs.depth ? cs.depth + ray : nullptr, cs.weights ? cs.weights + ray * kCoarseSamples : nullptr);
        }
    }
    }});
    if constexpr (FINE) {
        block_sync();
        const FwdKernelArgs mirror{pts, viewdirs, vd_stride, samples_per_ray, wpk, wh3, sc, raw, save_arg, P, cs, fs, cm};
        const auto* late = late_args(mirror);
        const int rays_per_block = late->fs.rays_per_block;
        if (wave_id() < rays_per_block) {
            const int slot = wave_id(), tot = kCoarseSamples + late->fs.n_importance;
            const int n_rays = late->fs.n_rays;
            long ray = (long)blockIdx.x * rays_per_block + slot;
            const bool ray_live = ray < n_rays;
            if (!ray_live) ray = n_rays - 1;
            const float norm = ray::ray_norm(late->fs.rays + ray * late->fs.ray_stride + 3);
            auto fetch = [&](int i, f32x4* rw, float* zi) {
                *rw = rawbuf[slot * tot + i];
                *zi = zbuf[slot * tot + i];
            };
            const float* noise = late->fs.noise;
            float* depth = late->fs.depth;
            float* weights = late->fs.weights;
            ray::composite_ray(fetch, tot, norm, noise ? noise + ray * tot : nullptr, late->fs.white_bkgd, ray_live, lane_id(),
                               late->fs.rgb + ray * 3, late->fs.disp + ray, late->fs.acc + ray, depth ? depth + ray : nullptr,
                               weights ? weights + ray * tot : nullptr);
        }
    }
}


template <int PD, bool TRAIN, int PRODUCTS = 3>
inline int launch_fwd_h3(const float* pts, const float* viewdirs, int vd_stride, int samples_per_ray, const float* wpacked,
                         const short* wh3, const float* scales, float* raw, float* save, long long n_samples, ChunkMaxima cm,
                         hipStream_t st) {
    constexpr unsigned lds = fwd_lds_bytes<PD>();
    SCN_LDS_OPT_IN((mlp_fwd_h3_kernel<PD, TRAIN, kPoints, PRODUCTS>), lds);
    hipLaunchKernelGGL((mlp_fwd_h3_kernel<PD, TRAIN, kPoints, PRODUCTS>), dim3(scn_ceil_div(n_samples, kSamplesPerBlock)), dim3(kThreads),
                       lds, st, pts, viewdirs, vd_stride, samples_per_ray, wpacked, wh3, scales, raw, save, (long)n_samples,
                       CoarseStage{}, FineStage{}, cm);
    return scn_launch_status();
}


template <bool TRAIN, int PRODUCTS = 3>
inline int launch_coarse_h3(const CoarseStage& cs, const float* rays, int ray_stride, const float* wpacked, const short* stream_fwd,
                            const float* scales, float* raw, float* save, ChunkMaxima cm, hipStream_t st) {
    constexpr unsigned lds = fwd_lds_bytes<3>();
    const long P = (long)cs.n_rays * kCoarseSamples;
    SCN_LDS_OPT_IN((mlp_fwd_h3_kernel<3, TRAIN, kCoarse, PRODUCTS>), lds);
    hipLaunchKernelGGL((mlp_fwd_h3_kernel<3, TRAIN, kCoarse, PRODUCTS>), dim3(scn_ceil_div(P, kSamplesPerBlock)), dim3(kThreads), lds, st,
                       (const float*)nullptr, rays + 8, ray_stride, kCoarseSamples, wpacked, stream_fwd, scales, raw, save, P, cs,
                       FineStage{}, cm);
    return scn_launch_status();
}


template <bool TRAIN>
inline int launch_fine_h3(const FineStage& fs, const float* wpacked, const short* stream_fwd, const float* scales, float* raw,
                          float* save, ChunkMaxima cm, hipStream_t st) {
    constexpr unsigned lds = fwd_lds_bytes<3, kFine>();
    const int tot = kCoarseSamples + fs.n_importance;
    const long P = (long)fs.n_rays * tot;
    SCN_LDS_OPT_IN((mlp_fwd_h3_kernel<3, TRAIN, kFine>), lds);
    hipLaunchKernelGGL((mlp_fwd_h3_kernel<3, TRAIN, kFine>), dim3(scn_ceil_div(fs.n_rays, fs.rays_per_block)), dim3(kThreads), lds,
                       st, (const float*)nullptr, fs.rays + 8, fs.ray_stride, tot, wpacked, stream_fwd, scales, raw, save, P,
                       CoarseStage{}, fs, cm);
    return scn_launch_status();
}

}
}
```

scnerf_amd/csrc/mlp_h3.h:

```cpp
#pragma once
#include <type_traits>
#include <utility>

#include <scn_lab.h>
#include <scn_wave.h>

#include "mlp_common.h"
#include "resident_guard.h"

namespace scn {
namespace h3 {

using namespace scn::mlp;

constexpr int kChunkBytes = 32768;
constexpr int kStreamLds = 3 * kChunkBytes;
constexpr int kTableFloats = 2816;
constexpr int kScaleStride = 8;
enum : int { kSw = 0, kSwInv = 1, kBoundA = 2, kBoundB = 3, kBoundAT = 4, kPoison = 7 };
enum : int { kLayerFeat = 8, kLayerViews = 9, kLayerRgb = 10, kLayerAlpha = 11, kScaleLayers = 12 };

typedef unsigned u32x4 __attribute__((ext_vector_type(4)));
template <int N> using I = std::integral_constant<int, N>;

template <class F, int... Is>
__device__ __forceinline__ void static_for_impl(F&& f, std::integer_sequence<int, Is...>) {
    (f(I<Is>{}), ...);
}
template <int N, class F>
__device__ __forceinline__ void static_for(F&& f) {
    static_for_impl(f, std::make_integer_sequence<int, N>{});
}

__device__ __forceinline__ float scale_for(float bound) {
    const unsigned e = (__float_as_uint(bound) >> 23) & 0xffu;
    return __uint_as_float((266u - (e < 13u ? 13u : e)) << 23);
}
__device__ __forceinline__ float inv_pow2(float s) { return __uint_as_float(0x7f000000u - __float_as_uint(s)); }

constexpr unsigned kStoreWindowOpen = 0x7fffffffu, kStoreWindowShut = 0u;
#if defined(SCNERF_SIMT_EMU_BUILD)
inline void store_written_through_window(global_bytes_rw base, unsigned lane_off, f32x4 v, unsigned window) {
    if (window != kStoreWindowShut) store_written_through_at(base, lane_off, v);
}
#else
__device__ __forceinline__ void store_written_through_window(global_bytes_rw base, unsigned lane_off, f32x4 v, unsigned window) {
    const __amdgpu_buffer_rsrc_t rsrc = __builtin_amdgcn_make_buffer_rsrc((void*)base, 0, (int)window, 0x00020000);
    __builtin_amdgcn_raw_buffer_store_b128(__builtin_bit_cast(scn_u32x4, v), rsrc, (int)lane_off, 0, 1 | 2 | 16);
}
#endif

__device__ __forceinline__ void guard_check(const ResidentGuard& g, int guard_layer, float am, float s, bool live, long wave_tile) {
    if (g.flags == nullptr) return;
    const int m = (int)((__float_as_uint(am) >> 23) & 0xffu) + (int)((__float_as_uint(s) >> 23) & 0xffu) - 254;
    const bool on = live && lane_id() < 32 && am > 0.f;
    const unsigned long long under = ballot(on && m < kGuardLo), over = ballot(on && m >= kGuardHi);
    if ((under | over) != 0ull && lane_id() == 0) {
        g.flags[wave_tile >> 2] = 1;
        *g.any = 1;
        if (g.report) {
            float* counts = g.report + kGuardLayers * kGuardSlots + 2 * guard_layer;
            if (under) atomic_add(counts, (float)popcount64(under));
            if (over) atomic_add(counts + 1, (float)popcount64(over));
        }
    }
    if (g.report) {
        float v = on ? (float)(kGuardBias - m) : 0.f;
        v = fmaxf(v, shfl_xor(v, 16)); v = fmaxf(v, shfl_xor(v, 8)); v = fmaxf(v, shfl_xor(v, 4));
        v = fmaxf(v, shfl_xor(v, 2)); v = fmaxf(v, shfl_xor(v, 1));
        if (lane_id() == 0 && v > 0.f)
            atomic_max_nonneg(g.report + guard_layer * kGuardSlots + (int)(wave_tile & (kGuardSlots - 1)), v);
    }
}

__device__ __forceinline__ void cut8(const float* x, float s, u32x4& h, u32x4& l) {
#pragma unroll
    for (int c = 0; c < 4; ++c) {
        const unsigned hp = pack_f16_scaled(x[2 * c], x[2 * c + 1], s);
        h[c] = hp;
        l[c] = pack_f16(residual_f16<0>(x[2 * c], s, hp), residual_f16<1>(x[2 * c + 1], s, hp));
    }
}

__device__ __forceinline__ void cut8_high(const float* x, float s, u32x4& h) {
#pragma unroll
    for (int c = 0; c < 4; ++c) h[c] = pack_f16_scaled(x[2 * c], x[2 * c + 1], s);
}

struct Stream {
    global_bytes g;
    unsigned cur;
    f32x4 stage[8];
    __device__ __forceinline__ unsigned next() const { return cur == 2u * kChunkBytes ? 0u : cur + kChunkBytes; }
};

__device__ __forceinline__ void stream_prime(Stream& ws, const void* stream, char* lds, unsigned tid16) {
    ws.g = uniform_global(stream);
#pragma unroll
    for (int i = 0; i < 8; ++i) ws.stage[i] = load_f32x4(ws.g + i * 4096, tid16);
#pragma unroll
    for (int i = 0; i < 8; ++i) *reinterpret_cast<f32x4*>(lds + i * 4096 + tid16) = ws.stage[i];
    ws.g = uniform_global(ws.g + kChunkBytes);
#pragma unroll
    for (int i = 0; i < 8; ++i) ws.stage[i] = load_f32x4(ws.g + i * 4096, tid16);
    ws.g = uniform_global(ws.g + kChunkBytes);
    ws.cur = 0u;
    if constexpr (lab::kNoStream) {
#pragma unroll
        for (int b = 1; b < 3; ++b)
#pragma unroll
            for (int i = 0; i < 8; ++i) *reinterpret_cast<f32x4*>(lds + b * kChunkBytes + i * 4096 + tid16) = ws.stage[i];
    }
}

template <int KAPPA>
__device__ __forceinline__ void stream_slot(Stream& ws, char* lds, unsigned tid16) {
    if constexpr (!lab::kNoStream && KAPPA < 24 && KAPPA % 3 == 0)
        *reinterpret_cast<f32x4*>(lds + ws.next() + (KAPPA / 3) * 4096 + tid16) = ws.stage[KAPPA / 3];
    if constexpr (!lab::kNoBarrier && KAPPA == 30) block_sync();
    constexpr int LOAD_PIECE = lab::kNoStream ? -1
                               : lab::kLateLoads ? ((KAPPA >= 24 && KAPPA % 3 == 0) ? (KAPPA - 24) / 3 : -1)
                                                 : ((KAPPA < 24 && KAPPA % 3 == 1) ? KAPPA / 3 : -1);
    if constexpr (LOAD_PIECE >= 0)
        ws.stage[LOAD_PIECE] = load_f32x4(uniform_global(ws.g + LOAD_PIECE * 4096), pinned_here(tid16));
    if constexpr (KAPPA == 47) {
        ws.cur = ws.next();
        ws.g = uniform_global(ws.g + kChunkBytes);
    }
}

__device__ __forceinline__ s16x8 as_frag(u32x4 v) { return __builtin_bit_cast(s16x8, v); }

struct NoFill {
    template <int S> __device__ __forceinline__ void operator()(I<S>) const {}
};

struct Wave {
    char* lds;
    unsigned tid16, lane16;
    Stream ws;
    s16x8 ring[2][4];
};

__device__ __forceinline__ void ring_prime(Wave& w) {
#pragma unroll
    for (int j = 0; j < 4; ++j) w.ring[0][j] = *reinterpret_cast<const s16x8*>(w.lds + j * 1024 + w.lane16);
}

template <int U, bool PAIR, bool FIRST, int PRODUCTS = 3, class Fill>
__device__ __forceinline__ void unit(Wave& w, u32x4 xhA, u32x4 xlA, u32x4 xhB, u32x4 xlB, f32x16 (&acc)[2], Fill&& fill) {
    static_assert(PRODUCTS == 3 || PRODUCTS == 1, "three fp16 products per product, or the high one alone");
    constexpr int PH = U & 7, RP = U & 1;
    static_for<6>([&](auto j_tag) {
        constexpr int j = decltype(j_tag)::value;
        if constexpr (PRODUCTS == 1) {
            stream_slot<PH * 6 + j>(w.ws, w.lds, w.tid16);
            fill(j_tag);
            if constexpr (j < 3) {
                constexpr int NPH = (PH + 1) & 7;
                const unsigned buf = PH == 7 ? w.ws.next() : w.ws.cur;
                w.ring[RP ^ 1][j] = *reinterpret_cast<const s16x8*>(w.lds + buf + (NPH * 4 + j) * 1024 + w.lane16);
            }
            sched_fence();
            if constexpr (j == 0 || j == 3) {
                constexpr int x = j == 3, fr = PAIR ? x : 2 * x;
                const u32x4 b = (!PAIR && x) ? xhB : xhA;
                if constexpr (FIRST) {
                    const f32x16 zero = {0.f, 0.f, 0.f, 0.f, 0.f, 0.f, 0.f, 0.f, 0.f, 0.f, 0.f, 0.f, 0.f, 0.f, 0.f, 0.f};
                    acc[x] = mfma_32x32x16_f16(w.ring[RP][fr], as_frag(b), zero);
                } else {
                    acc[x] = mfma_32x32x16_f16(w.ring[RP][fr], as_frag(b), acc[x]);
                }
            }
// ... 92 lines not shown
```

scnerf_amd/functional.py:

```python
from __future__ import annotations

from dataclasses import dataclass
from typing import Optional

import torch

from . import mlp_layout as ML
from . import ops

Tensor = torch.Tensor


@dataclass
class RenderConfig:
    n_samples: int
    n_importance: int
    lindisp: bool
    white_bkgd: bool
    track: bool = True


_host_cache = {}


def host_linspace(n: int, device) -> Tensor:
    key = (n, str(device))
    if key not in _host_cache:
        _host_cache[key] = torch.linspace(0.0, 1.0, steps=n, dtype=torch.float32, device="cpu").to(device)
    return _host_cache[key]


def _c(t: Optional[Tensor]) -> Optional[Tensor]:
    if t is None:
        return None
    return t.contiguous().float()


class RenderRaysFunction(torch.autograd.Function):

    @staticmethod
    def forward(ctx, ray_batch, cfg, t_rand, u, noise_c, noise_f, net_c, net_f, *params):
        ctx.set_materialize_grads(False)
        rays = _c(ray_batch)
        if rays.shape[1] < 11:
            raise NotImplementedError("the fused network needs view directions (ray_batch [N, 11])")
        n = rays.shape[0]
        dev = rays.device
        sc, sf = cfg.n_samples, cfg.n_importance
        train = cfg.track and any(ctx.needs_input_grad)
        viewdirs = rays[:, 8:11]

        net_c.require_standard()
        flat_c = net_c.flat_parameters()
        save_c = ops.save_workspace(n * sc, dev) if train else None
        wf_c, pl_c = ops.network_packs(net_c, flat_c, train, n)
        resident = isinstance(pl_c, ops.ResidentWeights)
        mx_c = ops.ChunkMaxima(n * sc, dev) if (train and resident) else None
        lean = ops.lean_decision(("render", "all"), mx_c)
        fast = resident and pl_c.fast
        guards = ops.guard_records(dev, [("coarse", n * sc)] + ([("fine", n * (sc + sf))] if sf > 0 else []), fast=fast) \
            if (resident and n > 0) else {}
        gd_c = guards.get("coarse")
        grid = ops.inference_occupancy() if (not train and n > 0 and noise_c is None and noise_f is None) else None
        stop = ops.inference_early_stop() if (not train and n > 0 and noise_c is None and noise_f is None) else None
        if grid is not None:
            grid.check(net_c, net_f)
            if grid.bits.device != dev:
                raise ValueError("the occupancy grid lives on %s, the rays on %s" % (grid.bits.device, dev))
        if grid is not None or (stop is not None and sf == 0):
            z_c, pts_c = ops.coarse_sample(rays, host_linspace(sc, dev), _c(t_rand), cfg.lindisp)
            raw_c = RenderRaysFunction._stage_network(pts_c, viewdirs, sc, wf_c, pl_c, gd_c, grid,
                                                      stop + (z_c, rays) if (stop is not None and sf == 0) else None).view(n, sc, 4)
            rgb_c, disp_c, acc_c, w_c, depth_c = ops.composite_fwd(raw_c, z_c, rays, None, cfg.white_bkgd)
        elif sc == ops.COARSE_STAGE_SAMPLES and n > 0:
            z_c, pts_c, raw_c, rgb_c, disp_c, acc_c, w_c, depth_c = ops.coarse_stage_fwd(
                rays, host_linspace(sc, dev), _c(t_rand), cfg.lindisp, wf_c, save_c, _c(noise_c), cfg.white_bkgd,
                planes=pl_c, maxima=mx_c, guard=gd_c, lean=lean)
        else:
            z_c, pts_c = ops.coarse_sample(rays, host_linspace(sc, dev), _c(t_rand), cfg.lindisp)
            raw_c = ops.mlp_fwd(pts_c, viewdirs, sc, wf_c, save_c, planes=pl_c, maxima=mx_c, guard=gd_c, lean=lean).view(n, sc, 4)
            rgb_c, disp_c, acc_c, w_c, depth_c = ops.composite_fwd(raw_c, z_c, rays, _c(noise_c), cfg.white_bkgd)

        ctx.cfg, ctx.train, ctx.n = cfg, train, n
        ctx.net_c, ctx.net_f = net_c, net_f
        ctx.n_params_c = len(net_c.ordered_parameters())
        ctx.coarse = (z_c, pts_c, raw_c, _c(noise_c), save_c, mx_c)
        ctx.lean = lean
        ctx.live = {"coarse": ops.live_decision(n * sc, mx_c), "fine": False}
        ctx.flat_c = flat_c.detach().clone() if lean else None
        ctx.flat_f = None
        ctx.pl_c = pl_c
        ctx.guards = guards
        ctx.rays = rays
        ctx.wb_c = ops.pack_weights(flat_c, "bwd") if train else None
        ctx.fine = None
        if sf == 0:
            out = (rgb_c, disp_c, acc_c, depth_c, raw_c, None, None, None, None, None, z_c, None)
            ctx.mark_non_differentiable(z_c)
            return out

        fine_net = net_f if net_f is not None else net_c
        u_dev = _c(u) if u is not None else host_linspace(sf, dev)
        tot = sc + sf
        fine_net.require_standard()
        flat_f = fine_net.flat_parameters()
        save_f = ops.save_workspace(n * tot, dev) if train else None
        wf_f, pl_f = (wf_c, pl_c) if fine_net is net_c else ops.network_packs(fine_net, flat_f, train, n)
        mx_f = ops.ChunkMaxima(n * tot, dev) if (train and resident) else None
        gd_f = guards.get("fine")
        if not train and sf > 0 and ops.inference_skip_empty() is not None and n > 0:
            out = RenderRaysFunction._fine_stage_on_live_rays(
                ops.inference_skip_empty(), rays, z_c, w_c, u_dev, _c(noise_f), cfg.white_bkgd, wf_f, pl_f, gd_f,
                (rgb_c, disp_c, acc_c, depth_c), sc, sf, grid=grid, stop=stop)
            ctx.mark_non_differentiable(*out[5:])
            return out[:5] + (rgb_c, disp_c, acc_c, depth_c) + out[5:]
        if grid is not None or stop is not None:
            z_f, pts_f, z_s, z_std, _, _ = ops.fine_sample(rays, z_c, w_c, u_dev)
            raw_f = RenderRaysFunction._stage_network(pts_f, viewdirs, tot, wf_f, pl_f, gd_f, grid,
                                                      stop + (z_f, rays) if stop is not None else None).view(n, tot, 4)
            rgb_f, disp_f, acc_f, _, depth_f = ops.composite_fwd(raw_f, z_f, rays, None, cfg.white_bkgd, want_weights=False)
        elif ops.fused_fine_stage() and gd_f is None and not fast and resident and sc == ops.COARSE_STAGE_SAMPLES and sf in ops.FINE_STAGE_IMPORTANCE and n > 0:
            z_f, pts_f, z_s, z_std, _, _, raw_f, rgb_f, disp_f, acc_f, depth_f, _ = ops.fine_stage_fwd(
                rays, z_c, w_c, u_dev, wf_f, save_f, _c(noise_f), cfg.white_bkgd, pl_f, maxima=mx_f, lean=lean)
        else:
            z_f, pts_f, z_s, z_std, _, _ = ops.fine_sample(rays, z_c, w_c, u_dev)
            raw_f = ops.mlp_fwd(pts_f, viewdirs, tot, wf_f, save_f, planes=pl_f, maxima=mx_f, guard=gd_f, lean=lean).view(n, tot, 4)
            rgb_f, disp_f, acc_f, _, depth_f = ops.composite_fwd(raw_f, z_f, rays, _c(noise_f), cfg.white_bkgd,
                                                                 want_weights=False)
        ctx.fine = (z_f, pts_f, raw_f, _c(noise_f), save_f, mx_f)
        ctx.live["fine"] = ops.live_decision(n * tot, mx_f)
        ctx.flat_f = (ctx.flat_c if fine_net is net_c else flat_f.detach().clone()) if lean else None
        ctx.pl_f = pl_f
        ctx.wb_f = (ctx.wb_c if fine_net is net_c else ops.pack_weights(flat_f, "bwd")) if train else None
        ctx.mark_non_differentiable(z_std, z_f, z_s)
        return (rgb_f, disp_f, acc_f, depth_f, raw_f, rgb_c, disp_c, acc_c, depth_c, z_std, z_f, z_s)

    @staticmethod
    def _stage_network(pts, viewdirs, samples_per_ray, wf, pl, gd, grid=None, stop=None):
        if stop is None:
            if grid is None:
                return ops.mlp_fwd(pts, viewdirs, samples_per_ray, wf, None, planes=pl, guard=gd)
            _, slot_of, pts_l, vd_l, n_live = ops.occ_compact(pts, viewdirs, samples_per_ray, grid)
            raw_l = ops.mlp_fwd(pts_l, vd_l, 1, wf, None, planes=pl, guard=gd) if n_live > 0 else None
            return ops.occ_expand_raw(raw_l, slot_of, n_live)
        eps, K, z, rays = stop
        S = samples_per_ray
        n = z.shape[0]
        b = ops.segment_bounds(S, K)
        raw = torch.empty((n * S, 4), dtype=torch.float32, device=pts.device)
        state = ops.StopState(n, pts.device)
        ran, n_rays = 0, n
        for k in range(K):
            first, length = b[k], b[k + 1] - b[k]
            opening = k == 0
            _, slot_of, pts_l, vd_l, n_live, n_rays = ops.seg_compact(
                pts, viewdirs, S, first, length, None if opening else state.alive, grid, read=not (opening and grid is None))
            raw_l = None
            if n_live > 0:
                name = "%s/%d" % (gd.name, k) if gd is not None else None
                gd_k = ops.guard_records(pts.device, [(name, n_live)])[name] if gd is not None else None
                raw_l = ops.mlp_fwd(pts_l, vd_l, 1, wf, None, planes=pl, guard=gd_k)
            ops.seg_expand_raw(raw_l, slot_of, raw, S, first, length, n_live)
            ran += n_live
            if k < K - 1:
                ops.seg_transmittance(raw, z, rays, first, length, k, K, eps, state)
        ops.early_stop_count(n, S, ran, n_rays, state.stop_segment)
        return raw

    @staticmethod
    def _fine_stage_on_live_rays(tau, rays, z_c, w_c, u, noise_f, white_bkgd, wf_f, pl_f, gd_f, coarse, sc, sf, grid=None,
                                 stop=None):
        tot = sc + sf
        live_idx, slot_of, n_live = ops.ray_compact(coarse[2], tau)
        live = None
        if n_live > 0:
            rays_l, z_l, w_l = (ops.ray_rows_gather(t, live_idx, n_live) for t in (rays, z_c, w_c))
            u_l = ops.ray_rows_gather(u, live_idx, n_live) if u.dim() == 2 else u
            noise_l = ops.ray_rows_gather(noise_f, live_idx, n_live) if noise_f is not None else None
            z_f, pts_f, z_s, z_std, _, _ = ops.fine_sample(rays_l, z_l, w_l, u_l)
            raw_f = RenderRaysFunction._stage_network(pts_f, rays_l[:, 8:11], tot, wf_f, pl_f, gd_f, grid,
                                                      stop + (z_f, rays_l) if stop is not None else None)
            raw_f = raw_f.view(n_live, tot, 4)
            rgb_f, disp_f, acc_f, _, depth_f = ops.composite_fwd(raw_f, z_f, rays_l, noise_l, white_bkgd, want_weights=False)
            live = (rgb_f, disp_f, acc_f, depth_f, z_std, raw_f, z_f, z_s)
        rgb, disp, acc, depth, z_std, raw, z_vals, z_samples = ops.ray_expand(slot_of, n_live, live, coarse, tot, sf)
        return rgb, disp, acc, depth, raw, z_std, z_vals, z_samples

    @staticmethod
    def _stage_composite_bwd(stage, rays, white_bkgd, g_rgb, g_disp, g_acc, g_depth, g_raw, want, live):
        z, _, raw, noise, _, _ = stage
        d_raw, d_rd = ops.composite_bwd(raw, z, rays, noise, white_bkgd, _c(g_rgb), _c(g_disp), _c(g_acc),
                                        _c(g_depth), _c(g_raw), want_d_rays_d=want)
        return d_raw, d_rd, ops.live_compact(d_raw) if live else None

    @staticmethod
    def _stage_dgrad(stage, first, rays, spr, wbk, d_rays, accumulate, planes=None, guard=None, lean=False, flat_params=None,
                     guard_fwd=None):
        z, pts, raw, noise, save, maxima = stage
        d_raw, d_rd, L = first
        want = d_rays is not None
        P = z.shape[0] * spr
        if L is not None and L.n > 0 and ops.live_guard_tripped(guard_fwd):
            L = None
        if L is not None and L.n > ops.LIVE_MAX_SHARE * P:
            L = None
        if L is not None and L.n > 0:
            masks, pts_l, vd_l = ops.live_gather(L, save, pts, rays[:, 8:11], spr)
            maxima_l = ops.live_maxima(L, maxima)
            guard_l = ops.live_guard_record(guard, L.n) if guard is not None else None
            grads, d_pts, d_views = ops.mlp_bwd_live(L, masks, pts_l, vd_l, wbk, planes, maxima_l, input_grad=want, lean=lean,
                                                     guard=guard_l)
            if guard_l is not None and guard_l.rerun and ops.live_guard_tripped(guard_l):
                L = None
            else:
                if guard_l is not None:
                    ops.live_guard_keep(guard_l)
                maxima = maxima_l
                if want:
                    d_pts, d_views = ops.live_scatter_rows(L, d_pts), ops.live_scatter_rows(L, d_views)
        if L is None:
            grads, d_pts, d_views = ops.mlp_bwd(d_raw, pts, rays[:, 8:11], spr, wbk, save, planes=planes, maxima=maxima,
                                                input_grad=want, guard=guard, lean=lean)
        elif L.n == 0:
            grads = maxima = None
            d_pts, d_views = (torch.zeros((P, 3), dtype=torch.float32, device=rays.device) for _ in range(2)) if want else (None, None)
        if want:
            ops.ray_reduce(d_pts, d_views, z, d_rd, d_rays, accumulate)
        return save, grads, d_raw, P, maxima, lean, flat_params, L

    @staticmethod
    def _stage_wgrad(pending, into=None):
        save, grads, d_raw, P, maxima, lean, flat_params, L = pending
        if L is not None:
            if L.n == 0:
                return None if into is not None else torch.zeros(ML.N_PARAMS, dtype=torch.float32, device=d_raw.device)
            out = ops.nerf_wgrad_live(L, save, grads, d_raw, maxima, flat_grad=into, accumulate=into is not None, lean=lean,
                                      flat_params=flat_params)
            return None if into is not None else out
        if into is not None:
            ops.nerf_wgrad(save, grads, d_raw, P, flat_grad=into, accumulate=True, maxima=maxima, lean=lean,
                           flat_params=flat_params)
            return None
        return ops.nerf_wgrad(save, grads, d_raw, P, maxima=maxima, lean=lean, flat_params=flat_params)

    @staticmethod
    def backward(ctx, g_rgb, g_disp, g_acc, g_depth, g_raw, g_rgb0, g_disp0, g_acc0, g_depth0, *_unused):
        if not ctx.train:
            raise RuntimeError("render_rays was evaluated without gradient tracking")
        cfg, rays, n = ctx.cfg, ctx.rays, ctx.n
        sc, sf = cfg.n_samples, cfg.n_importance
        d_rays = torch.zeros_like(rays) if ctx.needs_input_grad[0] else None
        fg_c = fg_f = None
        wrote = False
        n_pc = ctx.n_params_c
        need = ctx.needs_input_grad[8:]
        into_c = ctx.net_c.attached_flat_grad() if all(need[:n_pc]) else None
        into_f = into_c if ctx.net_f is None else (ctx.net_f.attached_flat_grad() if all(need[n_pc:]) else None)
        pend_f = pend_c = first_f = first_c = None
        want = d_rays is not None
        if sf > 0:
            if any(g is not None for g in (g_rgb, g_disp, g_acc, g_depth, g_raw)):
                first_f = RenderRaysFunction._stage_composite_bwd(ctx.fine, rays, cfg.white_bkgd, g_rgb, g_disp, g_acc, g_depth,
                                                                  g_raw, want, ctx.live["fine"])
            coarse_g = (g_rgb0, g_disp0, g_acc0, g_depth0, None)
        else:
            coarse_g = (g_rgb, g_disp, g_acc, g_depth, g_raw)
        if any(g is not None for g in coarse_g):
            first_c = RenderRaysFunction._stage_composite_bwd(ctx.coarse, rays, cfg.white_bkgd, *coarse_g, want,
                                                              ctx.live["coarse"])
        compactions = [f[2] for f in (first_f, first_c) if f is not None and f[2] is not None]
        if compactions:
            ops.live_counts(*compactions)
        if first_f is not None:
            pend_f = RenderRaysFunction._stage_dgrad(ctx.fine, first_f, rays, sc + sf, ctx.wb_f, d_rays, wrote,
                                                     planes=ctx.pl_f, guard=ctx.guards.get("fine_bwd"), lean=ctx.lean,
                                                     flat_params=ctx.flat_f, guard_fwd=ctx.guards.get("fine"))
            wrote = True
        if first_c is not None:
            pend_c = RenderRaysFunction._stage_dgrad(ctx.coarse, first_c, rays, sc, ctx.wb_c, d_rays, wrote, planes=ctx.pl_c,
# ... 48 lines not shown
```

scnerf_amd/mlp_layout.py:

```python
from __future__ import annotations

from dataclasses import dataclass
from typing import Dict, List, Tuple

import numpy as np

W = 256
D = 8
SKIP = 4
L_PTS = 10
L_VIEWS = 4
IN_VIEWS = 3 + 6 * L_VIEWS
E_VIEWS_SLOTS = 16


def feat_of(t, r, h):
    return 32 * t + (r & 3) + 8 * (r >> 2) + 4 * h


def row_to_rh(i):
    return (i & 3) + 4 * (i >> 3), (i >> 2) & 1


def pe_col(L: int, s: int, h: int, pd: int = 3) -> int:
# ... 206 lines not shown
                return base + row * ld + col if (col >= 0 and row >= 0) else -1
            return src

        def ident(limit, off=0):
            return lambda t, i: (off + 32 * t + i) if (32 * t + i) < limit else -1

        def pe_rows(L, t_base, off=0, pdim=3):
            def f(t, i):
                r, h = row_to_rh(i)
                c = pe_col(L, 16 * (t - t_base) + r, h, pdim)
                return off + c if c >= 0 else -1
            return f

        for p in self.bwd_parts:
            if p.name == "RGBT":
                s = dense_t("rgb_linear.weight", W // 2, ident(W // 2),
                            lambda st, h: (2 * st + h) if (2 * st + h) < 3 else -1)
            elif p.name == "VTF":
                s = dense_t("views_linears.0.weight", W + IN_VIEWS, ident(W), _feat_step)
            elif p.name == "VTE":
                s = dense_t("views_linears.0.weight", W + IN_VIEWS, pe_rows(L_VIEWS, 0, off=W), _feat_step)
            elif p.name == "FT":
                s = dense_t("feature_linear.weight", W, ident(W), _feat_step)
            elif p.name == "L5TH":
                s = dense_t("pts_linears.5.weight", W + IN, ident(W, off=IN), _feat_step)
            elif p.name == "L5TE":
                s = dense_t("pts_linears.5.weight", W + IN, pe_rows(L_PTS, 0, pdim=pd), _feat_step)
            elif p.name == "L0T":
                s = dense_t("pts_linears.0.weight", IN, pe_rows(L_PTS, 0, pdim=pd), _feat_step)
            else:
                l = int(p.name[1])
                s = dense_t("pts_linears.%d.weight" % l, W, ident(W), _feat_step)
            out.append(_part_index(p, s))
        out.append(lane_vector_table(po["alpha_linear.weight"], W, 8))
        idx = np.concatenate(out)
        assert idx.shape[0] == self.bwd_total
        return idx


_layouts: Dict[int, Layout] = {}


def layout(pd: int = 3) -> Layout:
    if pd not in _layouts:
        _layouts[pd] = Layout(pd)
    return _layouts[pd]


def padded_samples(P: int) -> int:
    return (P + 127) // 128 * 128


def grad_floats(P: int) -> int:
    return GRAD_FLOATS_PER_SAMPLE * padded_samples(P)


def untile(block, width: int, P: int):
    Pp = block.shape[0] // width
    a = block.reshape(Pp // 32, width // 32, 4, 2, 32, 4)
    a = a.transpose(0, 4, 1, 2, 3, 5).reshape(Pp, width)
    return a[:P]


def section_offsets(sections, P):
    Pp = padded_samples(P)
    off, out = 0, {}
    for name, w in sections:
        out[name] = off
        off += w * Pp
    return out, off


_STD = layout(3)
IN_PTS = _STD.in_pts
E_PTS_SLOTS = _STD.e_slots
PARAM_SHAPES = _STD.param_shapes
PARAM_OFFSETS = _STD.param_offsets
N_PARAMS = _STD.n_params
FWD_PARTS, BWD_PARTS = _STD.fwd_parts, _STD.bwd_parts
FWD_STREAM, BWD_STREAM = _STD.fwd_stream, _STD.bwd_stream
FWD_BIAS, FWD_BIAS_F, FWD_BIAS_V, FWD_BIAS_RGB = _STD.fwd_bias, _STD.fwd_bias_f, _STD.fwd_bias_v, _STD.fwd_bias_rgb
FWD_ALPHA_W, FWD_ALPHA_B, FWD_TOTAL = _STD.fwd_alpha_w, _STD.fwd_alpha_b, _STD.fwd_total
BWD_ALPHA_W, BWD_TOTAL = _STD.bwd_alpha_w, _STD.bwd_total
SAVE_SECTIONS = _STD.save_sections
SAVE_FLOATS_PER_SAMPLE = _STD.save_floats_per_sample


def forward_index() -> np.ndarray:
    return _STD.forward_index()


def backward_index() -> np.ndarray:
    return _STD.backward_index()


def save_floats(P: int) -> int:
    return _STD.save_floats(P)


H3_CHUNK_FRAGS = 32
H3_LAYER_FEAT, H3_LAYER_VIEWS, H3_LAYER_RGB, H3_LAYER_ALPHA = 8, 9, 10, 11
H3_SCALE_STRIDE = 8
H3_N_LAYERS = 12


def h3_feature_of(sl, g, e):
    return 32 * (sl >> 1) + 16 * (sl & 1) + 8 * (e >> 2) + 4 * g + (e & 3)


class H3Plan:

    def __init__(self):
        self.idx: List[np.ndarray] = []
        self.meta: List[int] = []
        self.part_units: List[Tuple[str, int]] = []

    def _frag(self, elem, T, slab, plane, layer):
        lane = np.arange(64)
        n, g = lane & 31, lane >> 5
        f = np.full((64, 8), -1, np.int32)
        for e in range(8):
            for ln in range(64):
                f[ln, e] = elem(32 * T + int(n[ln]), slab, int(g[ln]), e)
        self.idx.append(f)
        self.meta.append(plane | (layer << 1))

    def pair_part(self, name, n_tiles, slabs, elem, layer):
        assert n_tiles % 2 == 0
        for P in range(n_tiles // 2):
            for sl in slabs:
                for plane in (0, 1):
                    for T in (2 * P, 2 * P + 1):
                        self._frag(elem, T, sl, plane, layer)
        self.part_units.append((name, (n_tiles // 2) * len(slabs)))

    def single_part(self, name, T, slabs, elem, layer):
        assert len(slabs) % 2 == 0
        for sl in slabs:
            for plane in (0, 1):
                self._frag(elem, T, sl, plane, layer)
        self.part_units.append((name, len(slabs) // 2))

    def finish(self):
        n = len(self.idx)
        pad = (-n) % H3_CHUNK_FRAGS
        total = n + pad + 2 * H3_CHUNK_FRAGS
        idx = np.full((total, 64, 8), -1, np.int32)
        idx[:n] = np.stack(self.idx)
        meta = np.zeros(total, np.uint8)
        meta[:n] = np.array(self.meta, np.uint8)
        return idx.reshape(-1), meta, n


def _h3_forward(lay: "Layout") -> H3Plan:
    po, IN, pd = lay.param_offsets, lay.in_pts, lay.pd
    plan = H3Plan()
    enc = [("e", u) for u in range(lay.e_slots // 8)]
    trunk = [("t", sl) for sl in range(16)]

    def kcol(slab, g, e, L, pdim, off_enc, off_feat):
        kind, s = slab
        if kind == "e":
            c = pe_col(L, 8 * s + e, g, pdim)
            return off_enc + c if c >= 0 else -1
        return off_feat + h3_feature_of(s, g, e)

    def dense(wname, ld, n_valid, L=L_PTS, pdim=pd, off_enc=0, off_feat=0):
        base = po[wname]

        def elem(o, slab, g, e):
            c = kcol(slab, g, e, L, pdim, off_enc, off_feat)
            return base + o * ld + c if (o < n_valid and c >= 0) else -1
        return elem

    plan.pair_part("L0", 8, enc, dense("pts_linears.0.weight", IN, W), 0)
    for l in range(1, 8):
        if l == 5:
            plan.pair_part("L5", 8, enc + trunk, dense("pts_linears.5.weight", W + IN, W, off_feat=IN), 5)
        else:
            plan.pair_part("L%d" % l, 8, trunk, dense("pts_linears.%d.weight" % l, W, W), l)
    plan.pair_part("LF", 8, trunk, dense("feature_linear.weight", W, W), H3_LAYER_FEAT)
    venc = [("e", u) for u in range(E_VIEWS_SLOTS // 8)]
    plan.pair_part("V", 4, trunk + venc,
                   dense("views_linears.0.weight", W + IN_VIEWS, W // 2, L=L_VIEWS, pdim=3, off_enc=W), H3_LAYER_VIEWS)
    plan.single_part("RGB", 0, [("t", sl) for sl in range(8)], dense("rgb_linear.weight", W // 2, 3), H3_LAYER_RGB)
    return plan


def _h3_backward(lay: "Layout") -> H3Plan:
    po, IN, pd = lay.param_offsets, lay.in_pts, lay.pd
    plan = H3Plan()
    trunk = list(range(16))

    def ident(limit, off=0):
        return lambda o: (off + o) if o < limit else -1

    def pe_rows(L, off=0, pdim=3, n_slots=None):
        def f(o):
            t, i = divmod(o, 32)
            r, h = row_to_rh(i)
            s = 16 * t + r
            if n_slots is not None and s >= n_slots:
                return -1
            c = pe_col(L, s, h, pdim)
            return off + c if c >= 0 else -1
        return f

    def dense_t(wname, ld, ocol, n_rows):
        base = po[wname]

        def elem(o, sl, g, e):
            col = ocol(o)
            row = h3_feature_of(sl, g, e)
            return base + row * ld + col if (col >= 0 and row < n_rows) else -1
        return elem

    def rgbt(o, sl, g, e):
        return po["rgb_linear.weight"] + e * (W // 2) + o if (g == 0 and e < 3 and o < W // 2) else -1

    plan.pair_part("RGBT", 4, [0], rgbt, H3_LAYER_RGB)
    hv = list(range(8))
    plan.single_part("VTE", 0, hv, dense_t("views_linears.0.weight", W + IN_VIEWS,
                                            pe_rows(L_VIEWS, off=W, n_slots=E_VIEWS_SLOTS), W // 2), H3_LAYER_VIEWS)
    plan.pair_part("VTF", 8, hv, dense_t("views_linears.0.weight", W + IN_VIEWS, ident(W), W // 2), H3_LAYER_VIEWS)
    plan.pair_part("FT", 8, trunk, dense_t("feature_linear.weight", W, ident(W), W), H3_LAYER_FEAT)
    e_tiles = 2 if pd == 3 else 4
    for l in range(7, 0, -1):
        if l == 5:
            plan.pair_part("L5TE", e_tiles, trunk,
                           dense_t("pts_linears.5.weight", W + IN, pe_rows(L_PTS, pdim=pd, n_slots=lay.e_slots), W), 5)
            plan.pair_part("L5TH", 8, trunk, dense_t("pts_linears.5.weight", W + IN, ident(W, off=IN), W), 5)
        else:
            plan.pair_part("L%dT" % l, 8, trunk, dense_t("pts_linears.%d.weight" % l, W, ident(W), W), l)
    plan.pair_part("L0T", e_tiles, trunk,
                   dense_t("pts_linears.0.weight", IN, pe_rows(L_PTS, pdim=pd, n_slots=lay.e_slots), W), 0)
    return plan


_h3_cache: Dict[Tuple[int, str], tuple] = {}


def h3_plan(pd: int, kind: str):
    key = (pd, kind)
    if key not in _h3_cache:
        plan = _h3_forward(layout(pd)) if kind == "fwd" else _h3_backward(layout(pd))
        idx, meta, n = plan.finish()
        _h3_cache[key] = (idx, meta, n, plan.part_units)
    return _h3_cache[key]


def h3_scale_jobs(pd: int) -> np.ndarray:
    lay = layout(pd)
    po = lay.param_offsets
    names = ["pts_linears.%d" % l for l in range(8)] + ["feature_linear", "views_linears.0", "rgb_linear", "alpha_linear"]
    shapes = dict(lay.param_shapes)
    jobs = []
    for n in names:
        rows, cols = shapes[n + ".weight"]
        jobs.append([po[n + ".weight"], rows, cols, po[n + ".bias"]])
    return np.array(jobs, np.int32)
```

scnerf_amd/ops.py:

```python
from __future__ import annotations

import os
from typing import Optional

import numpy as np
import torch

from . import _capi
from . import mlp_layout as ML

Tensor = torch.Tensor


class _Profile:

    def __init__(self):
        self.enabled = False
        self.records = {}

    def reset(self, enabled=False):
        self.records = {}
        self.enabled = enabled

    class _Region:
# ... 734 lines not shown
    _EARLY_STOP_LAST[0] = stop_segment


RESIDENT_GUARDS = ("off", "fallback", "report", "strict")
_RESIDENT_GUARD = _Switch(RESIDENT_GUARDS, "SCNERF_RESIDENT_GUARD", "off",
                          "resident_guard is one of " + ", ".join(RESIDENT_GUARDS))


def resident_guard(mode: Optional[str] = None) -> str:
    return _RESIDENT_GUARD(mode)


class ResidentRangeError(RuntimeError):
    """A resident pass cut a layer output at a scale outside the range where the arithmetic is fp32 grade."""


GUARD_LAYERS = tuple("layer_%d" % l for l in range(8)) + ("feature", "views")
GUARD_SLOTS, GUARD_BIAS, GUARD_RANGE = 64, 256, (-3, 13)
GUARD_REPORT_FLOATS = len(GUARD_LAYERS) * (GUARD_SLOTS + 2)
_GUARD_LAST = {}


class GuardRecord:
    __slots__ = ("name", "blocks", "flags", "any", "report", "mode")

    def __init__(self, name, blocks, flags, any_, report, mode):
        self.name, self.blocks, self.flags, self.any, self.report, self.mode = name, blocks, flags, any_, report, mode

    @property
    def rerun(self) -> bool:
        return self.mode in ("fallback", "report")

    def args(self):
        return _p(self.flags) if self.blocks else _p(self.any), _p(self.any), _p(self.report)

    def margins(self) -> dict:
        out = {"reran_blocks": int((self.flags != 0).sum()) if self.rerun else 0, "blocks": self.blocks}
        if self.report is not None:
            rep = self.report.cpu()
            nl = len(GUARD_LAYERS)
            best = rep[:nl * GUARD_SLOTS].view(nl, GUARD_SLOTS).max(1)[0]
            counts = rep[nl * GUARD_SLOTS:].view(nl, 2)
            for i, name in enumerate(GUARD_LAYERS):
                out[name] = {"min_log2": GUARD_BIAS - int(best[i]) if best[i] > 0 else None,
                             "under": int(counts[i, 0]), "over": int(counts[i, 1])}
        return out

    def raise_if_tripped(self):
        if int(self.any.item()) == 0:
            return
        m = self.margins()
        lo, hi = GUARD_RANGE
        bad = [(n, m[n]) for n in GUARD_LAYERS if m[n]["under"] or m[n]["over"]]
        raise ResidentRangeError("resident pass %r: %s outside [%d, %d) (%d of %d blocks)" % (
            self.name, ", ".join("%s at min_log2 %s (%d under, %d over)" % (n, r["min_log2"], r["under"], r["over"]) for n, r in bad),
            lo, hi, int((self.flags != 0).sum()), m["blocks"]))


def guard_records(device, passes, fast: bool = False) -> dict:
    mode = _RESIDENT_GUARD.value
    if fast:
        for name, _ in passes:
            _GUARD_LAST.pop(name, None)
            _GUARD_LAST.pop(name + "_bwd", None)
        return {}
    if mode == "off":
        return {}
    rep = GUARD_REPORT_FLOATS if mode in ("report", "strict") else 0
    layout, total = [], 0
    for name, P in passes:
        nb = (int(P) + 127) // 128
        layout.append((name, nb, total))
        total += nb + 2 + 2 * rep
    buf = torch.zeros(total, dtype=torch.float32, device=device)
    ints = buf.view(torch.int32)
    out = {}
    for name, nb, o in layout:
        flags = ints[o:o + nb]
        r = o + nb + 2
        out[name] = GuardRecord(name, nb, flags, ints[o + nb:o + nb + 1], buf[r:r + rep] if rep else None, mode)
        out[name + "_bwd"] = GuardRecord(name + "_bwd", nb, flags, ints[o + nb + 1:o + nb + 2],
                                         buf[r + rep:r + 2 * rep] if rep else None, mode)
    return out


def resident_margins() -> dict:
    return {name: rec.margins() for name, rec in _GUARD_LAST.items()}


def _guard_args(guard: Optional[GuardRecord]):
    return guard.args() if guard is not None else (None, None, None)


def _guard_after(guard: Optional[GuardRecord], rerun):
    if guard is None:
        return
    _GUARD_LAST[guard.name] = guard
    if guard.mode == "strict":
        guard.raise_if_tripped()
    elif guard.rerun and guard.blocks:
        rerun(_p(guard.flags), 0)


def pack_for_arithmetic(flat_params: Tensor, train: bool, pd: int = 3, remap=None):
    if _MLP_ARITHMETIC.value == "resident":
        return pack_resident(flat_params, pd, remap=remap)
    return None


_PACK_CACHE = _Switch((False, True), "SCNERF_PACK_CACHE", parse=lambda preset: preset != "0")
PACK_CACHE_STATS = {"hits": 0, "packs": 0}


def weight_pack_cache(on: Optional[bool] = None) -> bool:
    return _PACK_CACHE(_on_off(on))


def forget_packs(net) -> None:
    if hasattr(net, "_infer_packs"):
        net._infer_packs = None


def inference_packs(net, flat_params: Tensor, pd: int = 3, remap=None):
    def build():
        PACK_CACHE_STATS["packs"] += 1
        planes = pack_for_arithmetic(flat_params, False, pd, remap=remap)
        if isinstance(planes, ResidentWeights):
            planes.fast = _INFERENCE_ARITHMETIC.value == "fast"
        return (pack_weights(flat_params, "fwd", pd=pd, remap=remap), planes)
    if not _PACK_CACHE.value:
        return build()
    key = (flat_params.data_ptr(), flat_params._version, tuple(p._version for p in net.parameters()), _MLP_ARITHMETIC.value,
           _INFERENCE_ARITHMETIC.value, pd, torch.cuda.current_stream(flat_params.device).cuda_stream if flat_params.is_cuda else 0)
    hit = getattr(net, "_infer_packs", None)
    if hit is not None and hit[0] == key:
        PACK_CACHE_STATS["hits"] += 1
        return hit[1]
    packs = build()
    object.__setattr__(net, "_infer_packs", (key, packs))
    return packs


def network_packs(net, flat_params: Tensor, train: bool, n: int, pd: int = 3, remap=None):
    if train or n == 0:
        wpacked = pack_weights(flat_params, "fwd", pd=pd, remap=remap)
        return wpacked, (pack_for_arithmetic(flat_params, train, pd, remap=remap) if n > 0 else None)
    return inference_packs(net, flat_params, pd, remap=remap)


_canon_cache = {}


class ResidentWeights:
    __slots__ = ("fwd", "bwd", "scales", "pd", "fast")

    def __init__(self, fwd, bwd, scales, pd):
        self.fwd, self.bwd, self.scales, self.pd = fwd, bwd, scales, pd
        self.fast = False


class ChunkMaxima:
    __slots__ = ("x", "z", "chunks", "chunk_samples", "scales")

    def __init__(self, P: int, device):
        self.chunks = int(_capi.load().scnerf_wgrad256_chunks(wgrad_chunks(P)))
        self.chunk_samples = int(_capi.load().scnerf_wgrad_chunk_samples(int(P), self.chunks))
        both = torch.zeros((2, 12, self.chunks), dtype=torch.float32, device=device)
        self.x, self.z = both[0], both[1]
        self.scales = None


_h3_tables = {}


def _h3_device_tables(pd: int, device):
    key = (pd, str(device))
    if key not in _h3_tables:
        t = {"jobs": torch.from_numpy(np.ascontiguousarray(ML.h3_scale_jobs(pd))).to(device)}
        for kind in ("fwd", "bwd"):
            idx, meta, _, _ = ML.h3_plan(pd, kind)
            t[kind] = (torch.from_numpy(idx).to(device), torch.from_numpy(meta).to(device), int(meta.shape[0]))
        _h3_tables[key] = t
    return _h3_tables[key]


def pack_resident(flat_params: Tensor, pd: int = 3, out: Optional[ResidentWeights] = None, remap=None) -> ResidentWeights:
    _f(flat_params, "flat_params")
    lay = ML.layout(pd)
    if flat_params.numel() != lay.n_params:
        raise ValueError("expected %d parameters, got %d" % (lay.n_params, flat_params.numel()))
    lib = _capi.load()
    dev = flat_params.device
    if remap is not None:
        key = (remap[0], str(dev))
        if key not in _canon_cache:
            _canon_cache[key] = torch.from_numpy(np.asarray(remap[1], dtype=np.int32)).to(dev)
        idx = _canon_cache[key]
        canon = torch.empty(lay.n_params, dtype=torch.float32, device=dev)
        _capi.check(lib.scnerf_gather_f32(_p(flat_params), _p(idx), _p(canon), idx.numel(), _stream()), "scnerf_gather_f32")
        flat_params = canon
    t = _h3_device_tables(pd, dev)
    if out is None:
        out = ResidentWeights(torch.empty(t["fwd"][2] * 512, dtype=torch.int16, device=dev),
                              torch.empty(t["bwd"][2] * 512, dtype=torch.int16, device=dev),
                              torch.empty(lib.scnerf_h3_scale_floats(), dtype=torch.float32, device=dev), pd)
    st = lib.scnerf_h3_pack(_p(flat_params), _p(t["jobs"]), _p(t["fwd"][0]), _p(t["fwd"][1]), t["fwd"][2],
                            _p(t["bwd"][0]), _p(t["bwd"][1]), t["bwd"][2], _p(out.fwd), _p(out.bwd), _p(out.scales), _stream())
    _capi.check(st, "scnerf_h3_pack")
    return out


def _vd(viewdirs: Tensor):
    if viewdirs.dtype != torch.float32 or not _capi.on_device(viewdirs) or viewdirs.dim() != 2 or viewdirs.shape[1] != 3:
        raise TypeError("viewdirs must be a CUDA fp32 [n,3] tensor")
    if viewdirs.stride(1) != 1:
        raise ValueError("viewdirs rows must be dense")
    return viewdirs.data_ptr(), int(viewdirs.stride(0)) if viewdirs.shape[0] > 1 else 3


def _network_args(pts: Tensor, viewdirs: Tensor, packed: Tensor, kind: str, pd: int, save: Optional[Tensor]):
    name = "wpacked" if kind == "fwd" else "wpacked_bwd"
    _f(pts, "pts"), _f(packed, name)
    if kind == "bwd":
        _f(save, "save")
    vptr, vstride = _vd(viewdirs)
    lay = ML.layout(pd)
    P = pts.numel() // pd
    if packed.numel() != (lay.fwd_total if kind == "fwd" else lay.bwd_total):
        raise ValueError(name + " has the wrong size")
    if kind == "fwd" and save is not None:
        _f(save, "save")
        if save.numel() < lay.save_floats(P):
            raise ValueError("activation workspace too small")
    return vptr, vstride, lay, P


def _ray_outputs(n: int, s: int, device, want_weights: bool = True):
    rgb = torch.empty((n, 3), dtype=torch.float32, device=device)
    disp, acc, depth = (torch.empty((n,), dtype=torch.float32, device=device) for _ in range(3))
    return rgb, disp, acc, depth, torch.empty((n, s), dtype=torch.float32, device=device) if want_weights else None


_MAC_PER_SAMPLE = {3: 593408, 4: 593408 + 2 * 256 * 21}


def mlp_fwd(pts: Tensor, viewdirs: Tensor, samples_per_ray: int, wpacked: Tensor,
            save: Optional[Tensor] = None, pd: int = 3, planes: Optional[Tensor] = None,
            maxima: Optional["ChunkMaxima"] = None, guard: Optional[GuardRecord] = None, lean: bool = False) -> Tensor:
    if isinstance(planes, ResidentWeights):
        if planes.pd != pd:
            raise ValueError("resident weights of another network variant")
        return mlp_fwd_resident(pts, viewdirs, samples_per_ray, wpacked, planes, save, maxima, guard, lean=lean)
    vptr, vstride, _, P = _network_args(pts, viewdirs, wpacked, "fwd", pd, save)
    raw = torch.empty((P, 4), dtype=torch.float32, device=pts.device)
    tag = "" if pd == 3 else "/pd4"
    if planes is not None:
        raise TypeError("planes must be a ResidentWeights or None")
    if lean:
        raise ValueError("the lean workspace belongs to the resident arithmetic")
    with PROFILE.region("mlp_fwd_kernel%s/P=%d/%s" % (tag, P, "train" if save is not None else "infer"),
                        2 * _MAC_PER_SAMPLE[pd] * P):
        st = _capi.load().scnerf_mlp_fwd(pd, _p(pts), vptr, vstride, int(samples_per_ray), _p(wpacked), _p(raw),
                                         _p(save), P, _stream())
    _capi.check(st, "scnerf_mlp_fwd")
    return raw


def mlp_fwd_resident(pts: Tensor, viewdirs: Tensor, samples_per_ray: int, wpacked: Tensor, rw: ResidentWeights,
                     save: Optional[Tensor] = None, maxima: Optional[ChunkMaxima] = None,
                     guard: Optional[GuardRecord] = None, lean: bool = False) -> Tensor:
    pd = rw.pd
    vptr, vstride, _, P = _network_args(pts, viewdirs, wpacked, "fwd", pd, save)
    raw = torch.empty((P, 4), dtype=torch.float32, device=pts.device)
    _check_lean(lean, pd, save, maxima, rw)
    if rw.fast:
        if save is not None or guard is not None:
            raise ValueError("the one-product arithmetic is forward-only and takes no guard record")
        with PROFILE.region("mlp_fwd_h3_kernel%s/P=%d/infer fast" % ("" if pd == 3 else "/pd4", P), 2 * _MAC_PER_SAMPLE[pd] * P):
            st = _capi.load().scnerf_mlp_fwd_h3_fast(pd, _p(pts), vptr, vstride, int(samples_per_ray), _p(wpacked), _p(rw.fwd),
                                                     _p(rw.scales), _p(raw), P, None, 0, 0, _stream())
        _capi.check(st, "scnerf_mlp_fwd_h3_fast")
        return raw
    with PROFILE.region("mlp_fwd_h3_kernel%s/P=%d/%s" % ("" if pd == 3 else "/pd4", P, "train" if save is not None else "infer"),
                        2 * _MAC_PER_SAMPLE[pd] * P):
        mx = maxima if save is not None else None
        st = _capi.load().scnerf_mlp_fwd_h3_lean(
            pd, _p(pts), vptr, vstride, int(samples_per_ray), _p(wpacked), _p(rw.fwd), _p(rw.scales), _p(raw), _p(save), P,
            _p(mx.x) if mx else None, mx.chunks if mx else 0, mx.chunk_samples if mx else 0, *_guard_args(guard), int(lean),
            _stream())
    _capi.check(st, "scnerf_mlp_fwd_h3")

    def rerun(flags, wgs):
        _capi.check(_capi.load().scnerf_mlp_fwd_gated(pd, _p(pts), vptr, vstride, int(samples_per_ray), _p(wpacked), _p(raw),
                                                      _p(save), P, flags, wgs, _stream()), "scnerf_mlp_fwd_gated")
    _guard_after(guard, rerun)
    return raw


def _check_lean(lean, pd, save, maxima, rw):
    if lean and (pd not in (3, 4) or save is None or maxima is None or rw.fast):
        raise ValueError("the lean workspace needs a training pass on three-product packs with chunk maxima")


COARSE_STAGE_SAMPLES = 64


def coarse_stage_fwd(rays: Tensor, t_vals: Tensor, t_rand: Optional[Tensor], lindisp: bool, wpacked: Tensor,
                     save: Optional[Tensor], noise: Optional[Tensor], white_bkgd: bool, planes: Optional[Tensor] = None,
                     maxima: Optional["ChunkMaxima"] = None, guard: Optional[GuardRecord] = None, lean: bool = False):
    _f(rays, "rays"), _f(t_vals, "t_vals"), _f(wpacked, "wpacked")
    for name, t_ in (("t_rand", t_rand), ("noise", noise), ("save", save)):
        if t_ is not None:
            _f(t_, name)
    n, s = rays.shape[0], t_vals.shape[0]
    if s != COARSE_STAGE_SAMPLES or rays.shape[1] < 11:
        raise ValueError("the fused coarse stage takes 64 samples per ray and an 11-column ray batch")
    lay = ML.layout(3)
    if wpacked.numel() != lay.fwd_total:
        raise ValueError("wpacked has the wrong size")
    if save is not None and save.numel() < lay.save_floats(n * s):
        raise ValueError("activation workspace too small")
    dev = rays.device
    z = torch.empty((n, s), dtype=torch.float32, device=dev)
    pts = torch.empty((n, s, 3), dtype=torch.float32, device=dev)
    raw = torch.empty((n, s, 4), dtype=torch.float32, device=dev)
    rgb, disp, acc, depth, w = _ray_outputs(n, s, dev)
    P = n * s
    if isinstance(planes, ResidentWeights):
        if planes.pd != 3:
            raise ValueError("the coarse stage samples 3-D points")
        _check_lean(lean, 3, save, maxima, planes)
        if planes.fast:
            if save is not None or guard is not None:
                raise ValueError("the one-product arithmetic is forward-only and takes no guard record")
            with PROFILE.region("mlp_fwd_h3_kernel<coarse stage>/P=%d/infer fast" % P, 2 * _MAC_PER_SAMPLE[3] * P):
                st = _capi.load().scnerf_coarse_stage_fwd_h3_fast(
                    _p(rays), rays.shape[1], _p(t_vals), _p(t_rand), int(bool(lindisp)), _p(wpacked), _p(planes.fwd),
                    _p(planes.scales), _p(noise), int(bool(white_bkgd)), _p(z), _p(pts), _p(raw), _p(rgb), _p(disp), _p(acc),
                    _p(depth), _p(w), n, s, None, 0, 0, _stream())
            _capi.check(st, "scnerf_coarse_stage_fwd_h3_fast")
            return z, pts, raw, rgb, disp, acc, w, depth
        with PROFILE.region("mlp_fwd_h3_kernel<coarse stage>/P=%d/%s" % (P, "train" if save is not None else "infer"),
                            2 * _MAC_PER_SAMPLE[3] * P):
            st = _capi.load().scnerf_coarse_stage_fwd_h3_lean(
                _p(rays), rays.shape[1], _p(t_vals), _p(t_rand), int(bool(lindisp)), _p(wpacked), _p(planes.fwd),
                _p(planes.scales), _p(save), _p(noise), int(bool(white_bkgd)), _p(z), _p(pts), _p(raw), _p(rgb), _p(disp),
                _p(acc), _p(depth), _p(w), n, s, _p(maxima.x) if (maxima and save is not None) else None,
                maxima.chunks if maxima else 0, maxima.chunk_samples if maxima else 0, *_guard_args(guard), int(lean),
                _stream())
        _capi.check(st, "scnerf_coarse_stage_fwd_h3")

        def rerun(flags, wgs):
            _capi.check(_capi.load().scnerf_coarse_stage_fwd_gated(
                _p(rays), rays.shape[1], _p(t_vals), _p(t_rand), int(bool(lindisp)), _p(wpacked), _p(save), _p(noise),
                int(bool(white_bkgd)), _p(z), _p(pts), _p(raw), _p(rgb), _p(disp), _p(acc), _p(depth), _p(w), n, s, flags, wgs,
                _stream()), "scnerf_coarse_stage_fwd_gated")
        _guard_after(guard, rerun)
        return z, pts, raw, rgb, disp, acc, w, depth
    if planes is not None:
        raise TypeError("planes must be a ResidentWeights or None")
    if lean:
        raise ValueError("the lean workspace belongs to the resident arithmetic")
    with PROFILE.region("mlp_fwd_kernel/P=%d/%s" % (P, "train" if save is not None else "infer"), 2 * _MAC_PER_SAMPLE[3] * P):
        st = _capi.load().scnerf_coarse_stage_fwd(_p(rays), rays.shape[1], _p(t_vals), _p(t_rand), int(bool(lindisp)),
                                                  _p(wpacked), _p(save), _p(noise), int(bool(white_bkgd)), _p(z), _p(pts),
                                                  _p(raw), _p(rgb), _p(disp), _p(acc), _p(depth), _p(w), n, s, _stream())
    _capi.check(st, "scnerf_coarse_stage_fwd")
    return z, pts, raw, rgb, disp, acc, w, depth


FINE_STAGE_IMPORTANCE = (64, 128, 192)
_FUSED_FINE_STAGE = _Switch((False, True), "SCNERF_FUSED_FINE_STAGE", parse=lambda preset: preset not in (None, "", "0"))


def fused_fine_stage(on: Optional[bool] = None) -> bool:
    return _FUSED_FINE_STAGE(_on_off(on))


_LEAN_SCOPES = ("off", "render", "all")


def _lean_scope_from_env(value: Optional[str]) -> str:
    if value is None:
        return "render"
    if value in ("", "0"):
        return "off"
    return "all" if value == "all" else "render"


_LEAN_WORKSPACE = _Switch(_LEAN_SCOPES, "SCNERF_LEAN_WORKSPACE", set_error="lean workspace scope must be one of %s" % (_LEAN_SCOPES,),
                          parse=_lean_scope_from_env)


def lean_workspace_scope(scope: Optional[str] = None) -> str:
    return _LEAN_WORKSPACE(scope)


def lean_workspace(on: Optional[bool] = None) -> bool:
    if on is not None:
        _LEAN_WORKSPACE.value = "render" if on else "off"
    return _LEAN_WORKSPACE.value != "off"


def lean_decision(scopes, *maxima) -> bool:
    return bool(_LEAN_WORKSPACE.value in scopes and all(m is not None for m in maxima) and wgrad_arithmetic() == "half")


def fine_stage_fwd(rays: Tensor, z_c: Tensor, w_c: Tensor, u: Tensor, wpacked: Tensor, save: Optional[Tensor],
                   noise: Optional[Tensor], white_bkgd: bool, planes: "ResidentWeights", maxima: Optional["ChunkMaxima"] = None,
                   want_inds=False, want_cdf=False, want_weights=False, lean: bool = False):
    _f(rays, "rays"), _f(z_c, "z_c"), _f(w_c, "w_c"), _f(u, "u"), _f(wpacked, "wpacked")
    for name, t_ in (("noise", noise), ("save", save)):
        if t_ is not None:
            _f(t_, name)
    if not isinstance(planes, ResidentWeights) or planes.pd != 3:
        raise TypeError("the fused fine stage runs on the resident arithmetic (3-D points)")
    if planes.fast:
        raise ValueError("the fused fine stage has no one-product instantiation: fine_sample, mlp_fwd, composite_fwd")
    n, sc = z_c.shape
    sf = u.shape[-1]
    if sc != COARSE_STAGE_SAMPLES or sf not in FINE_STAGE_IMPORTANCE or rays.shape[1] < 11:
        raise ValueError("the fused fine stage takes 64 coarse samples, N_importance in %s and an 11-column ray batch" % (FINE_STAGE_IMPORTANCE,))
    tot = sc + sf
    stride = sf if u.dim() == 2 else 0
    lay = ML.layout(3)
    if wpacked.numel() != lay.fwd_total:
        raise ValueError("wpacked has the wrong size")
    if save is not None and save.numel() < lay.save_floats(n * tot):
        raise ValueError("activation workspace too small")
    dev = rays.device
    z_f = torch.empty((n, tot), dtype=torch.float32, device=dev)
    pts_f = torch.empty((n, tot, 3), dtype=torch.float32, device=dev)
    z_s = torch.empty((n, sf), dtype=torch.float32, device=dev)
    z_std = torch.empty((n,), dtype=torch.float32, device=dev)
    inds = torch.empty((n, sf), dtype=torch.int64, device=dev) if want_inds else None
    cdf = torch.empty((n, sc - 1), dtype=torch.float32, device=dev) if want_cdf else None
    raw = torch.empty((n, tot, 4), dtype=torch.float32, device=dev)
    rgb, disp, acc, depth, w = _ray_outputs(n, tot, dev, want_weights)
    P = n * tot
    mx = maxima if save is not None else None
    _check_lean(lean, 3, save, maxima, planes)
    with PROFILE.region("mlp_fwd_h3_kernel<fine stage>/P=%d/%s" % (P, "train" if save is not None else "infer"),
                        2 * _MAC_PER_SAMPLE[3] * P):
        st = _capi.load().scnerf_fine_stage_fwd_h3_lean(
            _p(rays), rays.shape[1], _p(z_c), _p(w_c), _p(u), stride, _p(wpacked), _p(planes.fwd), _p(planes.scales), _p(save),
            _p(noise), int(bool(white_bkgd)), _p(z_f), _p(pts_f), _p(z_s), _p(z_std), _p(inds), _p(cdf), _p(raw), _p(rgb),
            _p(disp), _p(acc), _p(depth), _p(w), n, sc, sf, _p(mx.x) if mx else None, mx.chunks if mx else 0,
            mx.chunk_samples if mx else 0, *_guard_args(None), int(lean), _stream())
    _capi.check(st, "scnerf_fine_stage_fwd_h3")
    return z_f, pts_f, z_s, z_std, inds, cdf, raw, rgb, disp, acc, depth, w


def save_workspace(P: int, device, pd: int = 3) -> Tensor:
    return torch.empty(ML.layout(pd).save_floats(P), dtype=torch.float32, device=device)


def mlp_bwd(d_raw: Tensor, pts: Tensor, viewdirs: Tensor, samples_per_ray: int, wpacked_bwd: Tensor,
            save: Tensor, pd: int = 3, planes: Optional[Tensor] = None, maxima: Optional["ChunkMaxima"] = None,
            input_grad: bool = True, guard: Optional[GuardRecord] = None, lean: bool = False):
    if isinstance(planes, ResidentWeights):
        if planes.pd != pd:
            raise ValueError("resident weights of another network variant")
        return mlp_bwd_resident(d_raw, pts, viewdirs, samples_per_ray, wpacked_bwd, planes, save, maxima, input_grad, guard,
                                lean=lean)
    if lean:
        raise ValueError("the lean workspace belongs to the resident arithmetic")
    _f(d_raw, "d_raw")
    vptr, vstride, _, P = _network_args(pts, viewdirs, wpacked_bwd, "bwd", pd, save)
    dev = pts.device
    grads = torch.empty(ML.grad_floats(P), dtype=torch.float32, device=dev)
    d_pts = torch.empty((P, pd), dtype=torch.float32, device=dev)
    d_views = torch.empty((P, 3), dtype=torch.float32, device=dev)
    if planes is not None:
        raise TypeError("planes must be a ResidentWeights or None")
    with PROFILE.region("mlp_bwd_kernel%s/P=%d" % ("" if pd == 3 else "/pd4", P), 2 * _MAC_PER_SAMPLE[pd] * P):
        st = _capi.load().scnerf_mlp_bwd(pd, _p(d_raw), _p(pts), vptr, vstride, int(samples_per_ray),
                                         _p(wpacked_bwd), _p(save), _p(grads), _p(d_pts), _p(d_views), P, _stream())
    _capi.check(st, "scnerf_mlp_bwd")
    return grads, d_pts, d_views


def mlp_bwd_resident(d_raw: Tensor, pts: Tensor, viewdirs: Tensor, samples_per_ray: int, wpacked_bwd: Tensor,
                     rw: ResidentWeights, save: Tensor, maxima: Optional[ChunkMaxima] = None, input_grad: bool = True,
                     guard: Optional[GuardRecord] = None, lean: bool = False):
    _f(d_raw, "d_raw")
    pd = rw.pd
    vptr, vstride, _, P = _network_args(pts, viewdirs, wpacked_bwd, "bwd", pd, save)
    _check_lean(lean, pd, save, maxima, rw)
    dev = pts.device
    grads = torch.empty(ML.grad_floats(P), dtype=torch.float32, device=dev)
    d_pts = torch.empty((P, pd), dtype=torch.float32, device=dev) if input_grad else None
    d_views = torch.empty((P, 3), dtype=torch.float32, device=dev) if input_grad else None
    with PROFILE.region("mlp_bwd_h3_kernel%s/P=%d" % ("" if pd == 3 else "/pd4", P), 2 * _MAC_PER_SAMPLE[pd] * P):
        if maxima is not None:
            maxima.scales = rw.scales
        st = _capi.load().scnerf_mlp_bwd_h3_lean(
            pd, _p(d_raw), _p(pts), vptr, vstride, int(samples_per_ray), _p(wpacked_bwd), _p(rw.bwd), _p(rw.scales), _p(save),
            _p(grads), _p(d_pts), _p(d_views), P, _p(maxima.z) if maxima else None, maxima.chunks if maxima else 0,
            maxima.chunk_samples if maxima else 0, *_guard_args(guard), int(lean), _stream())
    _capi.check(st, "scnerf_mlp_bwd_h3")

    def rerun(flags, wgs):
        dp = d_pts if input_grad else torch.empty((P, pd), dtype=torch.float32, device=dev)
        dv = d_views if input_grad else torch.empty((P, 3), dtype=torch.float32, device=dev)
        _capi.check(_capi.load().scnerf_mlp_bwd_gated(pd, _p(d_raw), _p(pts), vptr, vstride, int(samples_per_ray),
                                                      _p(wpacked_bwd), _p(save), _p(grads), _p(dp), _p(dv), P, flags, wgs,
                                                      _stream()), "scnerf_mlp_bwd_gated")
    _guard_after(guard, rerun)
    return grads, d_pts, d_views


def wgrad_chunks(P: int) -> int:
    return int(max(1, min(256, P // 256)))

# ... 553 lines not shown
```

Before: 403,800 rays/s.

## Fold feature_linear into views layer for lean coarse forward passes

Adds a fold kernel that precomputes W_views[:, :256]·W_feat and the matching folded bias in double precision. It also adds forward kernel variants that skip the feature_linear layer and feed layer 7's output straight into the folded views layer. This removes one 256x256 GEMM per sample in the lean training forward. The cost is a separate folded weight pack, plus extra validation and numeric differences from folding the weights. The path is gated by a SCNERF_FOLD_FEATURE switch that is off by default and by a minimum sample count.

```diff
diff --git a/include/scnerf_hip.h b/include/scnerf_hip.h
--- a/include/scnerf_hip.h
+++ b/include/scnerf_hip.h
@@ -194,6 +194,8 @@
                            const float* wpacked, const short* stream_fwd, const float* scales, float* raw, float* save,
                            long long n_samples, float* chunk_amax, int n_chunks, long long chunk_samples, int* guard_flags,
                            int* guard_any, float* guard_report, int lean, void* stream);
+int scnerf_h3_fold(float* ext_params, long long w_views, long long b_views, long long w_feat, long long b_feat,
+                   long long w_out, long long b_out, float* scales, void* stream);
 int scnerf_coarse_stage_fwd_h3_lean(const float* rays, int ray_stride, const float* t_vals, const float* t_rand,
                                     int lindisp, const float* wpacked, const short* stream_fwd, const float* scales,
                                     float* save, const float* noise, int white_bkgd, float* z, float* pts, float* raw,
diff --git a/scnerf_amd/_capi.py b/scnerf_amd/_capi.py
--- a/scnerf_amd/_capi.py
+++ b/scnerf_amd/_capi.py
@@ -95,6 +95,7 @@
     "scnerf_fine_stage_fwd_h3_lean": [P, I, P, P, P, I, P, P, P, P, P, I, P, P, P, P, P, P, P, P, P, P, P, P, I, I, I, P,
                                       I, LL, P, P, P, I, P],
     "scnerf_nerf_wgrad_h3_lean": [I, P, P, P, LL, I, P, P, I, P, P, P, P, P, P, P],
+    "scnerf_h3_fold": [P, LL, LL, LL, LL, LL, LL, P, P],
     "scnerf_wgrad_lean_finish": [P, P, P, P, I, P],
     "scnerf_wgrad_lean_finish_pd": [I, P, P, P, P, I, P],
     "scnerf_image_metrics": [P, LL, LL, LL, LL, P, LL, LL, LL, LL, I, I, I, I, P, I, F, F, F, I, P, P, P, P, P],
diff --git a/scnerf_amd/csrc/mlp_fwd_h3.hip b/scnerf_amd/csrc/mlp_fwd_h3.hip
--- a/scnerf_amd/csrc/mlp_fwd_h3.hip
+++ b/scnerf_amd/csrc/mlp_fwd_h3.hip
@@ -10,8 +10,6 @@
 using namespace scn;
 using namespace scn::h3;
 
-constexpr int kScaleBlocks = 16, kScaleCols = 512;
-constexpr int kScalePartial = 4 + kScaleCols;
 
 __global__ __launch_bounds__(256) void h3_scale_partial_kernel(const float* __restrict__ params, const int* __restrict__ jobs,
                                                                float* __restrict__ partial, float* __restrict__ table) {
@@ -105,10 +103,47 @@
     out[i] = (short)((mt & 1u) ? f16_bits(x - f16_value(hb)) : hb);
 }
 
-}
-
-extern "C" long long scnerf_h3_scale_floats(void) {
-    return (long long)kScaleLayers * kScaleStride + (long long)kScaleLayers * kScaleBlocks * kScalePartial;
+constexpr int kFoldRows = 128, kFoldCols = 256 + 27, kFoldInner = 256;
+
+__global__ __launch_bounds__(256) void h3_fold_kernel(float* __restrict__ ext, long w_views, long b_views, long w_feat,
+                                                      long b_feat, long w_out, long b_out, float* __restrict__ scales) {
+    const int i = blockIdx.x * blockDim.x + threadIdx.x;
+    if (i >= kFoldRows * (kFoldCols + 1)) return;
+    const float* wv = ext + w_views;
+    if (i < kFoldRows * kFoldCols) {
+        const int o = i / kFoldCols, c = i % kFoldCols;
+        float r = wv[(long)o * kFoldCols + c];
+        if (c < kFoldInner) {
+            const float* wf = ext + w_feat;
+            double s = 0.0;
+            for (int k = 0; k < kFoldInner; ++k) s += (double)wv[(long)o * kFoldCols + k] * (double)wf[(long)k * kFoldInner + c];
+            r = (float)s;
+        }
+        ext[w_out + i] = r;
+    } else {
+        const int o = i - kFoldRows * kFoldCols;
+        const float* bf = ext + b_feat;
+        double s = (double)ext[b_views + o];
+        for (int k = 0; k < kFoldInner; ++k) s += (double)wv[(long)o * kFoldCols + k] * (double)bf[k];
+        const float r = (float)s;
+        ext[b_out + o] = r;
+        scales[kScaleFoldBias + o] = r;
+    }
+}
+
+}
+
+extern "C" long long scnerf_h3_scale_floats(void) { return (long long)kScaleFloats; }
+
+extern "C" int scnerf_h3_fold(float* ext_params, long long w_views, long long b_views, long long w_feat, long long b_feat,
+                              long long w_out, long long b_out, float* scales, void* stream) {
+    SCN_RETURN_IF(!ext_params || !scales, SCN_EINVAL);
+    SCN_RETURN_IF(w_views < 0 || b_views < 0 || w_feat < 0 || b_feat < 0 || w_out < 0 || b_out < 0, SCN_EINVAL);
+    SCN_RETURN_IF(w_out < w_views + (long long)kFoldRows * kFoldCols || w_out < w_feat + (long long)kFoldInner * kFoldInner, SCN_EINVAL);
+    SCN_RETURN_IF(w_out < b_views + kFoldRows || w_out < b_feat + kFoldInner || b_out < w_out + (long long)kFoldRows * kFoldCols, SCN_EINVAL);
+    hipLaunchKernelGGL(h3_fold_kernel, dim3(scn_ceil_div(kFoldRows * (kFoldCols + 1), 256)), dim3(256), 0, (hipStream_t)stream,
+                       ext_params, (long)w_views, (long)b_views, (long)w_feat, (long)b_feat, (long)w_out, (long)b_out, scales);
+    return scn_launch_status();
 }
 
 extern "C" int scnerf_h3_pack(const float* flat_params, const int* jobs, const int* idx_fwd, const unsigned char* meta_fwd,
@@ -141,9 +176,12 @@
     SCN_RETURN_IF(n_samples >= (1LL << 31), SCN_ENOSUP);
     SCN_RETURN_IF(chunk_amax && (n_chunks < 1 || chunk_samples < 32 || chunk_samples % 32), SCN_EINVAL);
     SCN_RETURN_IF(!guard_flags != !guard_any || (guard_report && !guard_flags), SCN_EINVAL);
+    SCN_RETURN_IF(lean < 0 || lean > 3 || ((lean & 2) && (!(lean & 1) || pt_dims != 3 || !save)), SCN_EINVAL);
     if (n_samples == 0) return 0;
     hipStream_t st = (hipStream_t)stream;
-    const scn::h3f::ChunkMaxima cm{chunk_amax, n_chunks, lean != 0, (long)chunk_samples, {guard_flags, guard_any, guard_report}};
+    const scn::h3f::ChunkMaxima cm{chunk_amax, n_chunks, lean & 1, (long)chunk_samples, {guard_flags, guard_any, guard_report}};
+    if (lean & 2)
+        return scn::h3f::fwd_h3_pd3_fold(pts, viewdirs, vd_stride, samples_per_ray, wpacked, stream_fwd, scales, raw, save, n_samples, cm, st);
     return pt_dims == 3 ? scn::h3f::fwd_h3_pd3(pts, viewdirs, vd_stride, samples_per_ray, wpacked, stream_fwd, scales, raw, save, n_samples, cm, st)
                         : scn::h3f::fwd_h3_pd4(pts, viewdirs, vd_stride, samples_per_ray, wpacked, stream_fwd, scales, raw, save, n_samples, cm, st);
 }
@@ -176,10 +214,12 @@
     SCN_RETURN_IF(n_samples != scn::h3f::kCoarseSamples || n_rays >= (1 << 25), SCN_ENOSUP);
     SCN_RETURN_IF(chunk_amax && (n_chunks < 1 || chunk_samples < 32 || chunk_samples % 32), SCN_EINVAL);
     SCN_RETURN_IF(!guard_flags != !guard_any || (guard_report && !guard_flags), SCN_EINVAL);
+    SCN_RETURN_IF(lean < 0 || lean > 3 || ((lean & 2) && (!(lean & 1) || !save)), SCN_EINVAL);
     if (n_rays == 0) return 0;
     const scn::h3f::CoarseStage cs{rays, ray_stride, n_rays, t_vals, t_rand, lindisp, z, pts, noise, white_bkgd,
                                    rgb_map, disp_map, acc_map, depth_map, weights};
-    const scn::h3f::ChunkMaxima cm{chunk_amax, n_chunks, lean != 0, (long)chunk_samples, {guard_flags, guard_any, guard_report}};
+    const scn::h3f::ChunkMaxima cm{chunk_amax, n_chunks, lean & 1, (long)chunk_samples, {guard_flags, guard_any, guard_report}};
+    if (lean & 2) return scn::h3f::fwd_h3_coarse_fold(cs, rays, ray_stride, wpacked, stream_fwd, scales, raw, save, cm, (hipStream_t)stream);
     return scn::h3f::fwd_h3_coarse(cs, rays, ray_stride, wpacked, stream_fwd, scales, raw, save, cm, (hipStream_t)stream);
 }
 
diff --git a/scnerf_amd/csrc/mlp_fwd_h3_api.h b/scnerf_amd/csrc/mlp_fwd_h3_api.h
--- a/scnerf_amd/csrc/mlp_fwd_h3_api.h
+++ b/scnerf_amd/csrc/mlp_fwd_h3_api.h
@@ -37,6 +37,11 @@
                hipStream_t st);
 int fwd_h3_coarse(const CoarseStage& cs, const float* rays, int ray_stride, const float* wpacked, const short* stream_fwd,
                   const float* scales, float* raw, float* save, ChunkMaxima cm, hipStream_t st);
+int fwd_h3_pd3_fold(const float* pts, const float* viewdirs, int vd_stride, int samples_per_ray, const float* wpacked,
+                    const short* stream_fwd, const float* scales, float* raw, float* save, long long n_samples, ChunkMaxima cm,
+                    hipStream_t st);
+int fwd_h3_coarse_fold(const CoarseStage& cs, const float* rays, int ray_stride, const float* wpacked, const short* stream_fwd,
+                       const float* scales, float* raw, float* save, ChunkMaxima cm, hipStream_t st);
 int fwd_h3_pd3_fast(const float* pts, const float* viewdirs, int vd_stride, int samples_per_ray, const float* wpacked,
                     const short* stream_fwd, const float* scales, float* raw, long long n_samples, hipStream_t st);
 int fwd_h3_pd4_fast(const float* pts, const float* viewdirs, int vd_stride, int samples_per_ray, const float* wpacked,
diff --git a/scnerf_amd/csrc/mlp_fwd_h3_coarse_fold.hip b/scnerf_amd/csrc/mlp_fwd_h3_coarse_fold.hip
--- /dev/null
+++ b/scnerf_amd/csrc/mlp_fwd_h3_coarse_fold.hip
@@ -0,0 +1,12 @@
+#include "mlp_fwd_h3_kernel.h"
+
+namespace scn {
+namespace h3f {
+
+int fwd_h3_coarse_fold(const CoarseStage& cs, const float* rays, int ray_stride, const float* wpacked, const short* stream_fwd,
+                       const float* scales, float* raw, float* save, ChunkMaxima cm, hipStream_t st) {
+    return launch_coarse_h3<true, 3, true>(cs, rays, ray_stride, wpacked, stream_fwd, scales, raw, save, cm, st);
+}
+
+}
+}
diff --git a/scnerf_amd/csrc/mlp_fwd_h3_kernel.h b/scnerf_amd/csrc/mlp_fwd_h3_kernel.h
--- a/scnerf_amd/csrc/mlp_fwd_h3_kernel.h
+++ b/scnerf_amd/csrc/mlp_fwd_h3_kernel.h
@@ -144,8 +144,8 @@
 };
 static_assert(sizeof(FwdKernelArgs) == 72 + sizeof(CoarseStage) + sizeof(FineStage) + sizeof(ChunkMaxima), "argument block layout");
 
-template <int PD, bool TRAIN, int STAGE, int PRODUCTS = 3>
-__global__ __launch_bounds__(kThreads, 1) void mlp_fwd_h3_kernel(
+template <int PD, bool TRAIN, int STAGE, int PRODUCTS, bool FOLD>
+__device__ __forceinline__ void mlp_fwd_h3_body(
     const float* __restrict__ pts, const float* __restrict__ viewdirs, int vd_stride, int samples_per_ray,
     const float* __restrict__ wpk, const short* __restrict__ wh3, const float* __restrict__ sc,
     float* __restrict__ raw, float* __restrict__ save_arg, long P, CoarseStage cs, FineStage fs, ChunkMaxima cm) {
@@ -153,6 +153,7 @@
     constexpr int ES = V::kES, NE = ES / 8;
     constexpr bool COARSE = STAGE == kCoarse, FINE = STAGE == kFine, ONE = PRODUCTS == 1;
     static_assert(!ONE || (!TRAIN && !FINE), "one product: forward-only, sample-list forward and coarse stage");
+    static_assert(!FOLD || (TRAIN && PD == 3 && !FINE && !ONE), "folded: the lean training passes of the standard network");
     claim_whole_register_file();
     auto low_of = [](const u32x4& lo, const u32x4& hi) { if constexpr (ONE) return hi; else return lo; };
     float* const save = TRAIN ? save_arg : nullptr;
@@ -163,7 +164,8 @@
     float* const tables = reinterpret_cast<float*>(w.lds + kStreamLds);
     float* const zbuf = reinterpret_cast<float*>(w.lds + kStreamLds + kTableFloats * 4 + ES * kThreads * 4);
     f32x4* const rawbuf = reinterpret_cast<f32x4*>(zbuf + kFineMaxSamples);
-    for (int i = threadIdx.x; i < V::kFwdTotal - V::kFwdBias; i += kThreads) tables[i] = wpk[V::kFwdBias + i];
+    for (int i = threadIdx.x; i < V::kFwdTotal - V::kFwdBias; i += kThreads)
+        tables[i] = (FOLD && i >= kTabViews && i < kTabViews + 128) ? sc[kScaleFoldBias + i - kTabViews] : wpk[V::kFwdBias + i];
     const int tiles = FINE ? uniform(fs.tiles) : 1;
     if constexpr (FINE) {
         static_assert(PD == 3, "the fine stage samples 3-D points");
@@ -397,20 +399,26 @@
         epi7.alpha = tab_h + kTabAlpha; epi7.save = t.save; epi7.lane16 = t.lane16;
         epi7.prime();
     }
-    trunk_layer(I<0>{}, I<0>{}, I<0>{}, prev, epi7, 6, 7, 0.f, 0.f);
-    FwdEpi<TRAIN, 2, PRODUCTS> epif;
-    epif.os = inv_pow2(epi7.s_next) * scale_of(kLayerFeat, kSwInv);
-    epif.s_next = 1.f; epif.am = 0.f;
-    epif.bias = tab_h + kTabFeat;
-    epif.save = TRAIN ? section(kSaveFeat, 256) : nullptr;
-    epif.lane16 = w.lane16;
-    if constexpr (TRAIN) {
-        const FwdKernelArgs mirror{pts, viewdirs, vd_stride, samples_per_ray, wpk, wh3, sc, raw, save_arg, P, cs, fs, cm};
-        epif.window = late_args(mirror)->cm.lean ? kStoreWindowShut : kStoreWindowOpen;
-    }
-    epif.prime();
-    trunk_layer(I<1>{}, I<0>{}, I<0>{}, epi7, epif, 7, kLayerFeat, 0.f, m_ev);
-
+    trunk_layer(I<0>{}, I<0>{}, I<0>{}, prev, epi7, 6, 7, 0.f, FOLD ? m_ev : 0.f);
+    using Feat = FwdEpi<TRAIN, 2, PRODUCTS>;
+    [[maybe_unused]] Feat epif;
+    if constexpr (!FOLD) {
+        epif.os = inv_pow2(epi7.s_next) * scale_of(kLayerFeat, kSwInv);
+        epif.s_next = 1.f; epif.am = 0.f;
+        epif.bias = tab_h + kTabFeat;
+        epif.save = TRAIN ? section(kSaveFeat, 256) : nullptr;
+        epif.lane16 = w.lane16;
+        if constexpr (TRAIN) {
+            const FwdKernelArgs mirror{pts, viewdirs, vd_stride, samples_per_ray, wpk, wh3, sc, raw, save_arg, P, cs, fs, cm};
+            epif.window = late_args(mirror)->cm.lean ? kStoreWindowShut : kStoreWindowOpen;
+        }
+        epif.prime();
+        trunk_layer(I<1>{}, I<0>{}, I<0>{}, epi7, epif, 7, kLayerFeat, 0.f, m_ev);
+    }
+
+    constexpr int XV = FOLD ? 1 : 0;
+    float s_vin;
+    if constexpr (FOLD) s_vin = epi7.s_next; else s_vin = epif.s_next;
     u32x4 vh[2], vl[2];
     {
         float ev[16];
@@ -423,15 +431,15 @@
                                         uniform(wave_id()), (int)pinned_here((unsigned)lane_id()));
         }
         if constexpr (ONE) {
-            cut8_high(ev, epif.s_next, vh[0]);
-            cut8_high(ev + 8, epif.s_next, vh[1]);
+            cut8_high(ev, s_vin, vh[0]);
+            cut8_high(ev + 8, s_vin, vh[1]);
         } else {
-            cut8(ev, epif.s_next, vh[0], vl[0]);
-            cut8(ev + 8, epif.s_next, vh[1], vl[1]);
+            cut8(ev, s_vin, vh[0], vl[0]);
+            cut8(ev + 8, s_vin, vh[1], vl[1]);
         }
     }
     Relu epiv;
-    epiv.os = inv_pow2(epif.s_next) * scale_of(kLayerViews, kSwInv);
+    epiv.os = inv_pow2(s_vin) * scale_of(kLayerViews, kSwInv);
     epiv.s_next = 1.f; epiv.am = 0.f;
     epiv.bias = tab_h + kTabViews;
     epiv.save = TRAIN ? section(kSaveHv, 128) : nullptr;
@@ -441,20 +449,29 @@
     {
         auto operand = [&](auto s_tag, u32x4& xh, u32x4& xl) {
             constexpr int s = decltype(s_tag)::value;
-            if constexpr (s < 16) { xh = bh[0][s]; xl = low_of(bl[0][s], xh); }
+            if constexpr (s < 16) { xh = bh[XV][s]; xl = low_of(bl[XV][s], xh); }
             else { xh = vh[s - 16]; xl = low_of(vl[s - 16], xh); }
         };
         tile_pair<0, 18, PRODUCTS>(w, acc[0], operand, [&](auto sg_tag) {
-            epi_slot<FwdEpi<TRAIN, 2, PRODUCTS>, 3, decltype(sg_tag)::value, 9>(epif, acc[1], bh[0], bl[0]);
+            if constexpr (FOLD) epi_slot<FwdEpi<TRAIN, 1, PRODUCTS>, 3, decltype(sg_tag)::value, 9>(epi7, acc[1], bh[XV], bl[XV]);
+            else epi_slot<Feat, 3, decltype(sg_tag)::value, 9>(epif, acc[1], bh[XV], bl[XV]);
         });
-        const float am_f = amax_of(epif.am);
-        guard(kLayerFeat, am_f, epif.s_next);
-        const float am = fmaxf(am_f, m_ev);
+        float am_in;
+        if constexpr (FOLD) {
+            store_mask(epi7, 7);
+            am_in = amax_of(epi7.am);
+            note_chunk_max(7, am_in);
+            guard(7, am_in, epi7.s_next);
+        } else {
+            am_in = amax_of(epif.am);
+            guard(kLayerFeat, am_in, epif.s_next);
+        }
+        const float am = fmaxf(am_in, m_ev);
         epiv.s_next = scale_for(__builtin_fmaf(scale_of(kLayerViews, kBoundA), am, scale_of(kLayerViews, kBoundB)));
         tile_pair<18, 18, PRODUCTS>(w, acc[1], operand, [&](auto sg_tag) {
-            epi_slot<Relu, 0, decltype(sg_tag)::value, 12>(epiv, acc[0], bh[1], bl[1]);
+            epi_slot<Relu, 0, decltype(sg_tag)::value, 12>(epiv, acc[0], bh[XV ^ 1], bl[XV ^ 1]);
         });
-        epi_all<Relu, 1>(epiv, acc[1], bh[1], bl[1]);
+        epi_all<Relu, 1>(epiv, acc[1], bh[XV ^ 1], bl[XV ^ 1]);
         store_mask(epiv, 8);
         guard(kLayerViews, amax_of(epiv.am), epiv.s_next);
     }
@@ -462,7 +479,7 @@
     f32x16 accc[2];
     tile_single<36, 4, PRODUCTS>(w, accc, [&](auto s_tag, u32x4& xh, u32x4& xl) {
         constexpr int s = decltype(s_tag)::value;
-        xh = bh[1][s]; xl = low_of(bl[1][s], xh);
+        xh = bh[XV ^ 1][s]; xl = low_of(bl[XV ^ 1][s], xh);
     }, NoFill{});
     const float os_rgb = __builtin_fmaf(inv_pow2(epiv.s_next), scale_of(kLayerRgb, kSwInv), scale_of(kLayerRgb, kPoison));
     const float sigma = epi7.sg + shfl_xor(epi7.sg, 32) + tables[kTabAlphaB];
@@ -526,28 +543,60 @@
 }
 
 
-template <int PD, bool TRAIN, int PRODUCTS = 3>
+template <int PD, bool TRAIN, int STAGE, int PRODUCTS = 3>
+__global__ __launch_bounds__(kThreads, 1) void mlp_fwd_h3_kernel(
+    const float* __restrict__ pts, const float* __restrict__ viewdirs, int vd_stride, int samples_per_ray,
+    const float* __restrict__ wpk, const short* __restrict__ wh3, const float* __restrict__ sc,
+    float* __restrict__ raw, float* __restrict__ save_arg, long P, CoarseStage cs, FineStage fs, ChunkMaxima cm) {
+    mlp_fwd_h3_body<PD, TRAIN, STAGE, PRODUCTS, false>(pts, viewdirs, vd_stride, samples_per_ray, wpk, wh3, sc, raw, save_arg, P, cs, fs, cm);
+}
+
+template <int STAGE>
+__global__ __launch_bounds__(kThreads, 1) void mlp_fwd_h3_kernel_fold(
+    const float* __restrict__ pts, const float* __restrict__ viewdirs, int vd_stride, int samples_per_ray,
+    const float* __restrict__ wpk, const short* __restrict__ wh3, const float* __restrict__ sc,
+    float* __restrict__ raw, float* __restrict__ save_arg, long P, CoarseStage cs, FineStage fs, ChunkMaxima cm) {
+    mlp_fwd_h3_body<3, true, STAGE, 3, true>(pts, viewdirs, vd_stride, samples_per_ray, wpk, wh3, sc, raw, save_arg, P, cs, fs, cm);
+}
+
+template <int PD, bool TRAIN, int PRODUCTS = 3, bool FOLD = false>
 inline int launch_fwd_h3(const float* pts, const float* viewdirs, int vd_stride, int samples_per_ray, const float* wpacked,
                          const short* wh3, const float* scales, float* raw, float* save, long long n_samples, ChunkMaxima cm,
                          hipStream_t st) {
     constexpr unsigned lds = fwd_lds_bytes<PD>();
-    SCN_LDS_OPT_IN((mlp_fwd_h3_kernel<PD, TRAIN, kPoints, PRODUCTS>), lds);
-    hipLaunchKernelGGL((mlp_fwd_h3_kernel<PD, TRAIN, kPoints, PRODUCTS>), dim3(scn_ceil_div(n_samples, kSamplesPerBlock)), dim3(kThreads),
-                       lds, st, pts, viewdirs, vd_stride, samples_per_ray, wpacked, wh3, scales, raw, save, (long)n_samples,
-                       CoarseStage{}, FineStage{}, cm);
+    if constexpr (FOLD) {
+        static_assert(PD == 3 && TRAIN && PRODUCTS == 3, "folded: the lean training pass of the standard network");
+        SCN_LDS_OPT_IN((mlp_fwd_h3_kernel_fold<kPoints>), lds);
+        hipLaunchKernelGGL((mlp_fwd_h3_kernel_fold<kPoints>), dim3(scn_ceil_div(n_samples, kSamplesPerBlock)), dim3(kThreads),
+                           lds, st, pts, viewdirs, vd_stride, samples_per_ray, wpacked, wh3, scales, raw, save, (long)n_samples,
+                           CoarseStage{}, FineStage{}, cm);
+    } else {
+        SCN_LDS_OPT_IN((mlp_fwd_h3_kernel<PD, TRAIN, kPoints, PRODUCTS>), lds);
+        hipLaunchKernelGGL((mlp_fwd_h3_kernel<PD, TRAIN, kPoints, PRODUCTS>), dim3(scn_ceil_div(n_samples, kSamplesPerBlock)), dim3(kThreads),
+                           lds, st, pts, viewdirs, vd_stride, samples_per_ray, wpacked, wh3, scales, raw, save, (long)n_samples,
+                           CoarseStage{}, FineStage{}, cm);
+    }
     return scn_launch_status();
 }
 
 
-template <bool TRAIN, int PRODUCTS = 3>
+template <bool TRAIN, int PRODUCTS = 3, bool FOLD = false>
 inline int launch_coarse_h3(const CoarseStage& cs, const float* rays, int ray_stride, const float* wpacked, const short* stream_fwd,
                             const float* scales, float* raw, float* save, ChunkMaxima cm, hipStream_t st) {
     constexpr unsigned lds = fwd_lds_bytes<3>();
     const long P = (long)cs.n_rays * kCoarseSamples;
-    SCN_LDS_OPT_IN((mlp_fwd_h3_kernel<3, TRAIN, kCoarse, PRODUCTS>), lds);
-    hipLaunchKernelGGL((mlp_fwd_h3_kernel<3, TRAIN, kCoarse, PRODUCTS>), dim3(scn_ceil_div(P, kSamplesPerBlock)), dim3(kThreads), lds, st,
-                       (const float*)nullptr, rays + 8, ray_stride, kCoarseSamples, wpacked, stream_fwd, scales, raw, save, P, cs,
-                       FineStage{}, cm);
+    if constexpr (FOLD) {
+        static_assert(TRAIN && PRODUCTS == 3, "folded: the lean training pass of the standard network");
+        SCN_LDS_OPT_IN((mlp_fwd_h3_kernel_fold<kCoarse>), lds);
+        hipLaunchKernelGGL((mlp_fwd_h3_kernel_fold<kCoarse>), dim3(scn_ceil_div(P, kSamplesPerBlock)), dim3(kThreads), lds, st,
+                           (const float*)nullptr, rays + 8, ray_stride, kCoarseSamples, wpacked, stream_fwd, scales, raw, save, P, cs,
+                           FineStage{}, cm);
+    } else {
+        SCN_LDS_OPT_IN((mlp_fwd_h3_kernel<3, TRAIN, kCoarse, PRODUCTS>), lds);
+        hipLaunchKernelGGL((mlp_fwd_h3_kernel<3, TRAIN, kCoarse, PRODUCTS>), dim3(scn_ceil_div(P, kSamplesPerBlock)), dim3(kThreads), lds, st,
+                           (const float*)nullptr, rays + 8, ray_stride, kCoarseSamples, wpacked, stream_fwd, scales, raw, save, P, cs,
+                           FineStage{}, cm);
+    }
     return scn_launch_status();
 }
 
diff --git a/scnerf_amd/csrc/mlp_fwd_h3_pd3_fold.hip b/scnerf_amd/csrc/mlp_fwd_h3_pd3_fold.hip
--- /dev/null
+++ b/scnerf_amd/csrc/mlp_fwd_h3_pd3_fold.hip
@@ -0,0 +1,13 @@
+#include "mlp_fwd_h3_kernel.h"
+
+namespace scn {
+namespace h3f {
+
+int fwd_h3_pd3_fold(const float* pts, const float* viewdirs, int vd_stride, int samples_per_ray, const float* wpacked,
+                    const short* stream_fwd, const float* scales, float* raw, float* save, long long n_samples, ChunkMaxima cm,
+                    hipStream_t st) {
+    return launch_fwd_h3<3, true, 3, true>(pts, viewdirs, vd_stride, samples_per_ray, wpacked, stream_fwd, scales, raw, save, n_samples, cm, st);
+}
+
+}
+}
diff --git a/scnerf_amd/csrc/mlp_h3.h b/scnerf_amd/csrc/mlp_h3.h
--- a/scnerf_amd/csrc/mlp_h3.h
+++ b/scnerf_amd/csrc/mlp_h3.h
@@ -19,6 +19,10 @@
 constexpr int kScaleStride = 8;
 enum : int { kSw = 0, kSwInv = 1, kBoundA = 2, kBoundB = 3, kBoundAT = 4, kPoison = 7 };
 enum : int { kLayerFeat = 8, kLayerViews = 9, kLayerRgb = 10, kLayerAlpha = 11, kScaleLayers = 12 };
+constexpr int kScaleBlocks = 16, kScaleCols = 512;
+constexpr int kScalePartial = 4 + kScaleCols;
+constexpr int kScaleFoldBias = kScaleLayers * kScaleStride + kScaleLayers * kScaleBlocks * kScalePartial;
+constexpr int kScaleFloats = kScaleFoldBias + 128;
 
 typedef unsigned u32x4 __attribute__((ext_vector_type(4)));
 template <int N> using I = std::integral_constant<int, N>;
diff --git a/scnerf_amd/functional.py b/scnerf_amd/functional.py
--- a/scnerf_amd/functional.py
+++ b/scnerf_amd/functional.py
@@ -57,6 +57,9 @@
         resident = isinstance(pl_c, ops.ResidentWeights)
         mx_c = ops.ChunkMaxima(n * sc, dev) if (train and resident) else None
         lean = ops.lean_decision(("render", "all"), mx_c)
+        fold_c = ops.fold_decision(lean, n * sc)
+        if fold_c:
+            ops.pack_folded(flat_c, pl_c)
         fast = resident and pl_c.fast
         guards = ops.guard_records(dev, [("coarse", n * sc)] + ([("fine", n * (sc + sf))] if sf > 0 else []), fast=fast) \
             if (resident and n > 0) else {}
@@ -75,10 +78,11 @@
         elif sc == ops.COARSE_STAGE_SAMPLES and n > 0:
             z_c, pts_c, raw_c, rgb_c, disp_c, acc_c, w_c, depth_c = ops.coarse_stage_fwd(
                 rays, host_linspace(sc, dev), _c(t_rand), cfg.lindisp, wf_c, save_c, _c(noise_c), cfg.white_bkgd,
-                planes=pl_c, maxima=mx_c, guard=gd_c, lean=lean)
+                planes=pl_c, maxima=mx_c, guard=gd_c, lean=lean, fold=fold_c)
         else:
             z_c, pts_c = ops.coarse_sample(rays, host_linspace(sc, dev), _c(t_rand), cfg.lindisp)
-            raw_c = ops.mlp_fwd(pts_c, viewdirs, sc, wf_c, save_c, planes=pl_c, maxima=mx_c, guard=gd_c, lean=lean).view(n, sc, 4)
+            raw_c = ops.mlp_fwd(pts_c, viewdirs, sc, wf_c, save_c, planes=pl_c, maxima=mx_c, guard=gd_c, lean=lean,
+                                fold=fold_c).view(n, sc, 4)
             rgb_c, disp_c, acc_c, w_c, depth_c = ops.composite_fwd(raw_c, z_c, rays, _c(noise_c), cfg.white_bkgd)
 
         ctx.cfg, ctx.train, ctx.n = cfg, train, n
@@ -108,6 +112,9 @@
         wf_f, pl_f = (wf_c, pl_c) if fine_net is net_c else ops.network_packs(fine_net, flat_f, train, n)
         mx_f = ops.ChunkMaxima(n * tot, dev) if (train and resident) else None
         gd_f = guards.get("fine")
+        fold_f = ops.fold_decision(lean, n * tot) and not ops.fused_fine_stage()
+        if fold_f:
+            ops.pack_folded(flat_f, pl_f)
         if not train and sf > 0 and ops.inference_skip_empty() is not None and n > 0:
             out = RenderRaysFunction._fine_stage_on_live_rays(
                 ops.inference_skip_empty(), rays, z_c, w_c, u_dev, _c(noise_f), cfg.white_bkgd, wf_f, pl_f, gd_f,
@@ -124,7 +131,8 @@
                 rays, z_c, w_c, u_dev, wf_f, save_f, _c(noise_f), cfg.white_bkgd, pl_f, maxima=mx_f, lean=lean)
         else:
             z_f, pts_f, z_s, z_std, _, _ = ops.fine_sample(rays, z_c, w_c, u_dev)
-            raw_f = ops.mlp_fwd(pts_f, viewdirs, tot, wf_f, save_f, planes=pl_f, maxima=mx_f, guard=gd_f, lean=lean).view(n, tot, 4)
+            raw_f = ops.mlp_fwd(pts_f, viewdirs, tot, wf_f, save_f, planes=pl_f, maxima=mx_f, guard=gd_f, lean=lean,
+                                fold=fold_f).view(n, tot, 4)
             rgb_f, disp_f, acc_f, _, depth_f = ops.composite_fwd(raw_f, z_f, rays, _c(noise_f), cfg.white_bkgd,
                                                                  want_weights=False)
         ctx.fine = (z_f, pts_f, raw_f, _c(noise_f), save_f, mx_f)
diff --git a/scnerf_amd/mlp_layout.py b/scnerf_amd/mlp_layout.py
--- a/scnerf_amd/mlp_layout.py
+++ b/scnerf_amd/mlp_layout.py
@@ -382,8 +382,16 @@
         return idx.reshape(-1), meta, n
 
 
-def _h3_forward(lay: "Layout") -> H3Plan:
+def fold_offsets(pd: int = 3):
+    n = layout(pd).n_params
+    return n, n + (W // 2) * (W + IN_VIEWS), n + (W // 2) * (W + IN_VIEWS) + W // 2
+
+
+def _h3_forward(lay: "Layout", folded: bool = False) -> H3Plan:
     po, IN, pd = lay.param_offsets, lay.in_pts, lay.pd
+    if folded:
+        po = dict(po)
+        po["views_linears.0.weight"] = fold_offsets(pd)[0]
     plan = H3Plan()
     enc = [("e", u) for u in range(lay.e_slots // 8)]
     trunk = [("t", sl) for sl in range(16)]
@@ -409,7 +417,8 @@
             plan.pair_part("L5", 8, enc + trunk, dense("pts_linears.5.weight", W + IN, W, off_feat=IN), 5)
         else:
             plan.pair_part("L%d" % l, 8, trunk, dense("pts_linears.%d.weight" % l, W, W), l)
-    plan.pair_part("LF", 8, trunk, dense("feature_linear.weight", W, W), H3_LAYER_FEAT)
+    if not folded:
+        plan.pair_part("LF", 8, trunk, dense("feature_linear.weight", W, W), H3_LAYER_FEAT)
     venc = [("e", u) for u in range(E_VIEWS_SLOTS // 8)]
     plan.pair_part("V", 4, trunk + venc,
                    dense("views_linears.0.weight", W + IN_VIEWS, W // 2, L=L_VIEWS, pdim=3, off_enc=W), H3_LAYER_VIEWS)
@@ -470,18 +479,23 @@
 _h3_cache: Dict[Tuple[int, str], tuple] = {}
 
 
-def h3_plan(pd: int, kind: str):
-    key = (pd, kind)
+def h3_plan(pd: int, kind: str, folded: bool = False):
+    key = (pd, kind, folded)
+    if folded and kind != "fwd":
+        raise ValueError("only the forward stream has a folded plan")
     if key not in _h3_cache:
-        plan = _h3_forward(layout(pd)) if kind == "fwd" else _h3_backward(layout(pd))
+        plan = _h3_forward(layout(pd), folded) if kind == "fwd" else _h3_backward(layout(pd))
         idx, meta, n = plan.finish()
         _h3_cache[key] = (idx, meta, n, plan.part_units)
     return _h3_cache[key]
 
 
-def h3_scale_jobs(pd: int) -> np.ndarray:
+def h3_scale_jobs(pd: int, folded: bool = False) -> np.ndarray:
     lay = layout(pd)
     po = lay.param_offsets
+    if folded:
+        po = dict(po)
+        po["views_linears.0.weight"], po["views_linears.0.bias"] = fold_offsets(pd)[:2]
     names = ["pts_linears.%d" % l for l in range(8)] + ["feature_linear", "views_linears.0", "rgb_linear", "alpha_linear"]
     shapes = dict(lay.param_shapes)
     jobs = []
diff --git a/scnerf_amd/ops.py b/scnerf_amd/ops.py
--- a/scnerf_amd/ops.py
+++ b/scnerf_amd/ops.py
@@ -910,10 +910,11 @@
 
 
 class ResidentWeights:
-    __slots__ = ("fwd", "bwd", "scales", "pd", "fast")
+    __slots__ = ("fwd", "bwd", "scales", "pd", "fast", "fold")
 
     def __init__(self, fwd, bwd, scales, pd):
         self.fwd, self.bwd, self.scales, self.pd = fwd, bwd, scales, pd
+        self.fold = None
         self.fast = False
 
 
@@ -931,15 +932,63 @@
 _h3_tables = {}
 
 
-def _h3_device_tables(pd: int, device):
-    key = (pd, str(device))
+def _h3_device_tables(pd: int, device, folded: bool = False):
+    key = (pd, str(device), folded) if folded else (pd, str(device))
     if key not in _h3_tables:
-        t = {"jobs": torch.from_numpy(np.ascontiguousarray(ML.h3_scale_jobs(pd))).to(device)}
-        for kind in ("fwd", "bwd"):
-            idx, meta, _, _ = ML.h3_plan(pd, kind)
+        t = {"jobs": torch.from_numpy(np.ascontiguousarray(ML.h3_scale_jobs(pd, folded))).to(device)}
+        for kind in ("fwd",) if folded else ("fwd", "bwd"):
+            idx, meta, _, _ = ML.h3_plan(pd, kind, folded)
             t[kind] = (torch.from_numpy(idx).to(device), torch.from_numpy(meta).to(device), int(meta.shape[0]))
         _h3_tables[key] = t
     return _h3_tables[key]
+
+
+FOLD_MIN_SAMPLES = 131072
+_FOLD_FEATURE = _Switch((False, True), "SCNERF_FOLD_FEATURE", parse=lambda preset: preset not in (None, "", "0"))
+
+
+def fold_feature(on: Optional[bool] = None) -> bool:
+    if on is not None:
+        _FOLD_FEATURE.value = bool(on)
+    return _FOLD_FEATURE.value
+
+
+def fold_decision(lean: bool, P: int, pd: int = 3) -> bool:
+    return bool(lean and pd == 3 and _FOLD_FEATURE.value and P >= FOLD_MIN_SAMPLES)
+
+
+class FoldedWeights:
+    __slots__ = ("params", "fwd", "scales")
+
+    def __init__(self, params, fwd, scales):
+        self.params, self.fwd, self.scales = params, fwd, scales
+
+
+def pack_folded(flat_params: Tensor, rw: "ResidentWeights") -> "ResidentWeights":
+    _f(flat_params, "flat_params")
+    pd = rw.pd
+    if pd != 3:
+        raise ValueError("the folded pack exists for the standard network")
+    if rw.fold is not None:
+        return rw
+    lay = ML.layout(pd)
+    lib = _capi.load()
+    dev = flat_params.device
+    w_off, b_off, total = ML.fold_offsets(pd)
+    po = lay.param_offsets
+    t = _h3_device_tables(pd, dev, folded=True)
+    ext = torch.empty(total, dtype=torch.float32, device=dev)
+    ext[:lay.n_params].copy_(flat_params.detach().reshape(-1))
+    fw = FoldedWeights(ext, torch.empty(t["fwd"][2] * 512, dtype=torch.int16, device=dev),
+                       torch.empty(lib.scnerf_h3_scale_floats(), dtype=torch.float32, device=dev))
+    _capi.check(lib.scnerf_h3_fold(_p(ext), po["views_linears.0.weight"], po["views_linears.0.bias"],
+                                   po["feature_linear.weight"], po["feature_linear.bias"], w_off, b_off, _p(fw.scales),
+                                   _stream()), "scnerf_h3_fold")
+    st = lib.scnerf_h3_pack(_p(ext), _p(t["jobs"]), _p(t["fwd"][0]), _p(t["fwd"][1]), t["fwd"][2], None, None, 0,
+                            _p(fw.fwd), None, _p(fw.scales), _stream())
+    _capi.check(st, "scnerf_h3_pack")
+    rw.fold = fw
+    return rw
 
 
 def pack_resident(flat_params: Tensor, pd: int = 3, out: Optional[ResidentWeights] = None, remap=None) -> ResidentWeights:
@@ -1004,17 +1053,18 @@
 
 def mlp_fwd(pts: Tensor, viewdirs: Tensor, samples_per_ray: int, wpacked: Tensor,
             save: Optional[Tensor] = None, pd: int = 3, planes: Optional[Tensor] = None,
-            maxima: Optional["ChunkMaxima"] = None, guard: Optional[GuardRecord] = None, lean: bool = False) -> Tensor:
+            maxima: Optional["ChunkMaxima"] = None, guard: Optional[GuardRecord] = None, lean: bool = False,
+            fold: bool = False) -> Tensor:
     if isinstance(planes, ResidentWeights):
         if planes.pd != pd:
             raise ValueError("resident weights of another network variant")
-        return mlp_fwd_resident(pts, viewdirs, samples_per_ray, wpacked, planes, save, maxima, guard, lean=lean)
+        return mlp_fwd_resident(pts, viewdirs, samples_per_ray, wpacked, planes, save, maxima, guard, lean=lean, fold=fold)
     vptr, vstride, _, P = _network_args(pts, viewdirs, wpacked, "fwd", pd, save)
     raw = torch.empty((P, 4), dtype=torch.float32, device=pts.device)
     tag = "" if pd == 3 else "/pd4"
     if planes is not None:
         raise TypeError("planes must be a ResidentWeights or None")
-    if lean:
+    if lean or fold:
         raise ValueError("the lean workspace belongs to the resident arithmetic")
     with PROFILE.region("mlp_fwd_kernel%s/P=%d/%s" % (tag, P, "train" if save is not None else "infer"),
                         2 * _MAC_PER_SAMPLE[pd] * P):
@@ -1026,11 +1076,12 @@
 
 def mlp_fwd_resident(pts: Tensor, viewdirs: Tensor, samples_per_ray: int, wpacked: Tensor, rw: ResidentWeights,
                      save: Optional[Tensor] = None, maxima: Optional[ChunkMaxima] = None,
-                     guard: Optional[GuardRecord] = None, lean: bool = False) -> Tensor:
+                     guard: Optional[GuardRecord] = None, lean: bool = False, fold: bool = False) -> Tensor:
     pd = rw.pd
     vptr, vstride, _, P = _network_args(pts, viewdirs, wpacked, "fwd", pd, save)
     raw = torch.empty((P, 4), dtype=torch.float32, device=pts.device)
     _check_lean(lean, pd, save, maxima, rw)
+    stream_fwd, scales = _check_fold(fold, lean, rw)
     if rw.fast:
         if save is not None or guard is not None:
             raise ValueError("the one-product arithmetic is forward-only and takes no guard record")
@@ -1043,9 +1094,9 @@
                         2 * _MAC_PER_SAMPLE[pd] * P):
         mx = maxima if save is not None else None
         st = _capi.load().scnerf_mlp_fwd_h3_lean(
-            pd, _p(pts), vptr, vstride, int(samples_per_ray), _p(wpacked), _p(rw.fwd), _p(rw.scales), _p(raw), _p(save), P,
-            _p(mx.x) if mx else None, mx.chunks if mx else 0, mx.chunk_samples if mx else 0, *_guard_args(guard), int(lean),
-            _stream())
+            pd, _p(pts), vptr, vstride, int(samples_per_ray), _p(wpacked), _p(stream_fwd), _p(scales), _p(raw), _p(save), P,
+            _p(mx.x) if mx else None, mx.chunks if mx else 0, mx.chunk_samples if mx else 0, *_guard_args(guard),
+            int(lean) | (LEAN_FLAG_FOLD if fold else 0), _stream())
     _capi.check(st, "scnerf_mlp_fwd_h3")
 
     def rerun(flags, wgs):
@@ -1060,12 +1111,24 @@
         raise ValueError("the lean workspace needs a training pass on three-product packs with chunk maxima")
 
 
+LEAN_FLAG_FOLD = 2
+
+
+def _check_fold(fold, lean, rw):
+    if not fold:
+        return rw.fwd, rw.scales
+    if not lean or rw.pd != 3 or rw.fold is None:
+        raise ValueError("a folded pass is a lean pass of the standard network on weights with a folded pack")
+    return rw.fold.fwd, rw.fold.scales
+
+
 COARSE_STAGE_SAMPLES = 64
 
 
 def coarse_stage_fwd(rays: Tensor, t_vals: Tensor, t_rand: Optional[Tensor], lindisp: bool, wpacked: Tensor,
                      save: Optional[Tensor], noise: Optional[Tensor], white_bkgd: bool, planes: Optional[Tensor] = None,
-                     maxima: Optional["ChunkMaxima"] = None, guard: Optional[GuardRecord] = None, lean: bool = False):
+                     maxima: Optional["ChunkMaxima"] = None, guard: Optional[GuardRecord] = None, lean: bool = False,
+                     fold: bool = False):
     _f(rays, "rays"), _f(t_vals, "t_vals"), _f(wpacked, "wpacked")
     for name, t_ in (("t_rand", t_rand), ("noise", noise), ("save", save)):
         if t_ is not None:
@@ -1088,6 +1151,7 @@
         if planes.pd != 3:
             raise ValueError("the coarse stage samples 3-D points")
         _check_lean(lean, 3, save, maxima, planes)
+        stream_fwd, scales = _check_fold(fold, lean, planes)
         if planes.fast:
             if save is not None or guard is not None:
                 raise ValueError("the one-product arithmetic is forward-only and takes no guard record")
@@ -1101,11 +1165,11 @@
         with PROFILE.region("mlp_fwd_h3_kernel<coarse stage>/P=%d/%s" % (P, "train" if save is not None else "infer"),
                             2 * _MAC_PER_SAMPLE[3] * P):
             st = _capi.load().scnerf_coarse_stage_fwd_h3_lean(
-                _p(rays), rays.shape[1], _p(t_vals), _p(t_rand), int(bool(lindisp)), _p(wpacked), _p(planes.fwd),
-                _p(planes.scales), _p(save), _p(noise), int(bool(white_bkgd)), _p(z), _p(pts), _p(raw), _p(rgb), _p(disp),
+                _p(rays), rays.shape[1], _p(t_vals), _p(t_rand), int(bool(lindisp)), _p(wpacked), _p(stream_fwd),
+                _p(scales), _p(save), _p(noise), int(bool(white_bkgd)), _p(z), _p(pts), _p(raw), _p(rgb), _p(disp),
                 _p(acc), _p(depth), _p(w), n, s, _p(maxima.x) if (maxima and save is not None) else None,
-                maxima.chunks if maxima else 0, maxima.chunk_samples if maxima else 0, *_guard_args(guard), int(lean),
-                _stream())
+                maxima.chunks if maxima else 0, maxima.chunk_samples if maxima else 0, *_guard_args(guard),
+                int(lean) | (LEAN_FLAG_FOLD if fold else 0), _stream())
         _capi.check(st, "scnerf_coarse_stage_fwd_h3")
 
         def rerun(flags, wgs):
@@ -1117,7 +1181,7 @@
         return z, pts, raw, rgb, disp, acc, w, depth
     if planes is not None:
         raise TypeError("planes must be a ResidentWeights or None")
-    if lean:
+    if lean or fold:
         raise ValueError("the lean workspace belongs to the resident arithmetic")
     with PROFILE.region("mlp_fwd_kernel/P=%d/%s" % (P, "train" if save is not None else "infer"), 2 * _MAC_PER_SAMPLE[3] * P):
         st = _capi.load().scnerf_coarse_stage_fwd(_p(rays), rays.shape[1], _p(t_vals), _p(t_rand), int(bool(lindisp)),
```

New measurement: 342,800 rays/s. 15.1% lower.
